# MorphIQ-Labs/VectorWave

Hardware: AMD Instinct MI355X
Metric: Msamples/sec MODWT fwd+inv db4 L=6, batch 4096×4096 fp64 @ 1/2/4/8 GPU (higher is better)
Workload: dtype f64

## Files before the change

include/vectorwave_amd.h:

```cpp
#ifndef VECTORWAVE_AMD_H
#define VECTORWAVE_AMD_H

#include <stdint.h>

#ifdef __cplusplus
extern "C" {
#endif

#define VW_API __attribute__((visibility("default")))

typedef struct vw_ctx vw_ctx;
typedef struct vw_stream vw_stream;
typedef int vw_status;

enum {
    VW_OK = 0,
    VW_ERR_NULL = 1,
    VW_ERR_EMPTY = 2,
    VW_ERR_NONFINITE = 3,
    VW_ERR_LEVEL = 4,
    VW_ERR_TOO_LARGE = 5,
    VW_ERR_BOUNDARY = 6,
    VW_ERR_ARG = 7,
    VW_ERR_DEVICE = 8,
// ... 27 lines not shown
VW_API vw_status vw_ctx_set_stream(vw_ctx *ctx, void *hip_stream);
VW_API vw_status vw_ctx_use_null_stream(vw_ctx *ctx);
VW_API void *vw_ctx_get_stream(vw_ctx *ctx);
VW_API vw_status vw_ctx_set_option(vw_ctx *ctx, const char *key, int value);
VW_API vw_status vw_ctx_synchronize(vw_ctx *ctx);
VW_API int vw_ctx_device(vw_ctx *ctx);

VW_API const char *vw_last_error(void);
VW_API int64_t vw_last_error_index(void);
VW_API const char *vw_version(void);
VW_API void vw_set_signal_base(int64_t base);

VW_API int vw_max_levels(int64_t N, int L);
VW_API int64_t vw_upsampled_length(int L, int level);

VW_API vw_status vw_modwt_forward_f64(vw_ctx *ctx, const double *x, int64_t B, int64_t N, int64_t ldx,
                                      const double *lo, const double *hi, int L, int wavelet_id,
                                      int boundary, int J, unsigned flags,
                                      double *details, double *approx);
VW_API vw_status vw_modwt_forward_f32(vw_ctx *ctx, const float *x, int64_t B, int64_t N, int64_t ldx,
                                      const double *lo, const double *hi, int L, int wavelet_id,
                                      int boundary, int J, unsigned flags,
                                      float *details, float *approx);

VW_API vw_status vw_modwt_inverse_f64(vw_ctx *ctx, const double *details, const double *approx,
                                      int64_t B, int64_t N, const double *lo, const double *hi, int L,
                                      int wavelet_id, int boundary, int J, unsigned detail_mask,
                                      int approx_zero, unsigned flags, double *y);
VW_API vw_status vw_modwt_inverse_f32(vw_ctx *ctx, const float *details, const float *approx,
                                      int64_t B, int64_t N, const double *lo, const double *hi, int L,
                                      int wavelet_id, int boundary, int J, unsigned detail_mask,
                                      int approx_zero, unsigned flags, float *y);

VW_API vw_status vw_modwt_forward_bi_f64(vw_ctx *ctx, const double *x, int64_t B, int64_t N, int64_t ldx,
                                         const double *lo, int Llo, const double *hi, int Lhi, int wavelet_id,
                                         int boundary, int J, unsigned flags, double *details, double *approx);
VW_API vw_status vw_modwt_forward_bi_f32(vw_ctx *ctx, const float *x, int64_t B, int64_t N, int64_t ldx,
                                         const double *lo, int Llo, const double *hi, int Lhi, int wavelet_id,
                                         int boundary, int J, unsigned flags, float *details, float *approx);
VW_API vw_status vw_modwt_inverse_bi_f64(vw_ctx *ctx, const double *details, const double *approx, int64_t B,
                                         int64_t N, const double *lo, int Llo, const double *hi, int Lhi,
                                         int wavelet_id, int boundary, int J, unsigned detail_mask,
                                         int approx_zero, unsigned flags, double *y);
VW_API vw_status vw_modwt_inverse_bi_f32(vw_ctx *ctx, const float *details, const float *approx, int64_t B,
                                         int64_t N, const double *lo, int Llo, const double *hi, int Lhi,
                                         int wavelet_id, int boundary, int J, unsigned detail_mask,
                                         int approx_zero, unsigned flags, float *y);
VW_API vw_status vw_modwt1_forward_bi_f64(vw_ctx *ctx, const double *x, int64_t B, int64_t N, int64_t ldx,
                                          const double *lo, int Llo, const double *hi, int Lhi, int boundary,
                                          unsigned flags, double *approx, double *detail);
VW_API vw_status vw_modwt1_inverse_bi_f64(vw_ctx *ctx, const double *approx, const double *detail, int64_t B,
                                          int64_t N, const double *lo, int Llo, const double *hi, int Lhi,
                                          int boundary, unsigned flags, double *y);

VW_API vw_status vw_modwt_energy_f64(vw_ctx *ctx, const double *x, int64_t B, int64_t N, int64_t ldx,
                                     const double *lo, const double *hi, int L, int wavelet_id,
                                     int boundary, int J, unsigned flags, double *out);
VW_API vw_status vw_energy_planes_f64(vw_ctx *ctx, const double *details, const double *approx, int64_t B,
                                      int64_t N, int J, unsigned flags, double *out);

VW_API vw_status vw_mra_planes_f64(vw_ctx *ctx, const double *details, const double *approx, int64_t B, int64_t N,
                                   const double *lo, const double *hi, int L, int wavelet_id, int boundary, int J,
                                   unsigned flags, double *out);
VW_API vw_status vw_mra_planes_f32(vw_ctx *ctx, const float *details, const float *approx, int64_t B, int64_t N,
                                   const double *lo, const double *hi, int L, int wavelet_id, int boundary, int J,
                                   unsigned flags, float *out);
VW_API vw_status vw_modwt_mra_f64(vw_ctx *ctx, const double *x, int64_t B, int64_t N, int64_t ldx,
                                  const double *lo, const double *hi, int L, int wavelet_id, int boundary, int J,
                                  unsigned flags, double *out);
VW_API vw_status vw_modwt_mra_f32(vw_ctx *ctx, const float *x, int64_t B, int64_t N, int64_t ldx,
                                  const double *lo, const double *hi, int L, int wavelet_id, int boundary, int J,
                                  unsigned flags, float *out);

VW_API vw_status vw_modwt_forward_multi_f64(vw_ctx *const *ctxs, int nctx, const double *x, int64_t B, int64_t N,
                                            int64_t ldx, const double *lo, const double *hi, int L, int wavelet_id,
                                            int boundary, int J, unsigned flags, double *details, double *approx);
VW_API vw_status vw_modwt_inverse_multi_f64(vw_ctx *const *ctxs, int nctx, const double *details,
                                            const double *approx, int64_t B, int64_t N, const double *lo,
                                            const double *hi, int L, int wavelet_id, int boundary, int J,
                                            unsigned detail_mask, int approx_zero, unsigned flags, double *y);

VW_API vw_status vw_modwt_forward_multi_dev_f64(vw_ctx *const *ctxs, int nctx, const double *const *x,
                                                const int64_t *rows, int64_t N, int64_t ldx, const double *lo,
                                                const double *hi, int L, int wavelet_id, int boundary, int J,
                                                unsigned flags, double *const *details, double *const *approx);
VW_API vw_status vw_modwt_inverse_multi_dev_f64(vw_ctx *const *ctxs, int nctx, const double *const *details,
                                                const double *const *approx, const int64_t *rows, int64_t N,
                                                const double *lo, const double *hi, int L, int wavelet_id,
                                                int boundary, int J, unsigned detail_mask, int approx_zero,
                                                unsigned flags, double *const *y);

VW_API vw_status vw_modwt1_forward_f64(vw_ctx *ctx, const double *x, int64_t B, int64_t N, int64_t ldx,
                                       const double *lo, const double *hi, int L, int boundary,
                                       unsigned flags, double *approx, double *detail);
VW_API vw_status vw_modwt1_inverse_f64(vw_ctx *ctx, const double *approx, const double *detail,
                                       int64_t B, int64_t N, const double *lo, const double *hi, int L,
                                       int boundary, unsigned flags, double *y);


VW_API vw_status vw_fin_analyze_f64(vw_ctx *ctx, const double *prices, int64_t B, int64_t N, int64_t ld,
                                    const double *lo, const double *hi, int L, double anomaly_k,
                                    unsigned flags, double *out);
VW_API vw_status vw_fin_sharpe_f64(vw_ctx *ctx, const double *returns, int64_t B, int64_t N, int64_t ld,
                                   double risk_free, unsigned flags, double *out);
VW_API vw_status vw_fin_wavelet_sharpe_f64(vw_ctx *ctx, const double *returns, int64_t B, int64_t N, int64_t ld,
                                           const double *lo, const double *hi, int L, int boundary,
                                           double risk_free, unsigned flags, double *out);

VW_API vw_status vw_swt_denoise_f64(vw_ctx *ctx, const double *x, int64_t B, int64_t N, int64_t ldx,
                                    const double *lo, const double *hi, int L, int wavelet_id,
                                    int boundary, int J, double threshold, int soft, unsigned flags,
                                    double *y, double *thresholds_out);
VW_API vw_status vw_transpose_f64(vw_ctx *ctx, const double *in, int64_t rows, int64_t cols, unsigned flags,
                                  double *out);
VW_API vw_status vw_transpose_f32(vw_ctx *ctx, const float *in, int64_t rows, int64_t cols, unsigned flags,
                                  float *out);

#define VW_THR_UNIVERSAL 0
#define VW_THR_SURE 1
#define VW_THR_MINIMAX 2
#define VW_THR_BAYES 3
#define VW_THR_FIXED 4
VW_API vw_status vw_wavelet_denoise_f64(vw_ctx *ctx, const double *x, int64_t B, int64_t N, int64_t ldx,
                                        const double *lo, const double *hi, int L, int wavelet_id,
                                        int boundary, int levels, int method, double fixed_threshold, int soft,
                                        unsigned flags, double *y, double *thresholds_out);

VW_API vw_status vw_noise_sigma_f64(vw_ctx *ctx, const double *coeffs, int64_t B, int64_t N,
                                    unsigned flags, double *sigma);
VW_API vw_status vw_threshold_f64(vw_ctx *ctx, double *c, int64_t B, int64_t N, const double *thr,
                                  int soft, unsigned flags);

VW_API vw_status vw_median_f64(vw_ctx *ctx, const double *x, int64_t B, int64_t N, const double *center,
                               unsigned flags, double *median_out);
VW_API vw_status vw_stddev_f64(vw_ctx *ctx, const double *x, int64_t N, unsigned flags, double *out);
VW_API vw_status vw_window_gather_abs_f64(vw_ctx *ctx, const double *src, const int32_t *idx, int64_t count,
                                          double *window, int64_t wsize, int64_t start);

VW_API vw_status vw_stream_create(vw_ctx *ctx, const double *lo, const double *hi, int L,
                                  int boundary, int levels, vw_stream **out);
VW_API vw_status vw_stream_destroy(vw_stream *s);
VW_API vw_status vw_stream_process_f64(vw_stream *s, const double *block, int64_t B, int64_t n,
                                       unsigned flags, double *details, double *approx);
VW_API vw_status vw_stream_flush_f64(vw_stream *s, int64_t tail_len, unsigned flags,
                                     double *details, double *approx);
VW_API int64_t vw_stream_history_length(vw_stream *s, int level);
VW_API int64_t vw_stream_batch(vw_stream *s);

typedef struct vw_graph vw_graph;
VW_API vw_status vw_capture_begin(vw_ctx *ctx);
VW_API vw_status vw_capture_end(vw_ctx *ctx, vw_graph **out);
VW_API vw_status vw_graph_launch(vw_graph *graph, int64_t count);
VW_API vw_status vw_graph_destroy(vw_graph *graph);

typedef struct vw_pipeline vw_pipeline;
VW_API vw_status vw_pipeline_create(vw_ctx *fwd_ctx, vw_ctx *inv_ctx, int elem_bytes, int sets, void *const *x,
                                    void *const *details, void *const *approx, void *const *y, int64_t B,
                                    int64_t N, const double *lo, const double *hi, int L, int wavelet_id,
                                    int boundary, int J, unsigned flags, vw_pipeline **out);
VW_API vw_status vw_pipeline_run(vw_pipeline *p, int64_t steps);
VW_API vw_status vw_pipeline_join(vw_pipeline *p);
VW_API int64_t vw_pipeline_last_set(vw_pipeline *p);
VW_API vw_status vw_pipeline_destroy(vw_pipeline *p);

VW_API vw_status vw_fill_uniform_f64(vw_ctx *ctx, double *x, int64_t count, uint64_t seed, int64_t offset);
VW_API vw_status vw_fill_uniform_f32(vw_ctx *ctx, float *x, int64_t count, uint64_t seed, int64_t offset);
VW_API vw_status vw_device_alloc(vw_ctx *ctx, int64_t bytes, void **out);
VW_API vw_status vw_device_free(vw_ctx *ctx, void *p);
VW_API vw_status vw_memcpy(vw_ctx *ctx, void *dst, const void *src, int64_t bytes, int kind );

VW_API vw_status vw_ctx_enable_timing(vw_ctx *ctx, int enable);
VW_API vw_status vw_ctx_kernel_time(vw_ctx *ctx, const char *family, double *total_ms, int64_t *launches);
VW_API vw_status vw_ctx_reset_timing(vw_ctx *ctx);
VW_API vw_status vw_ctx_kernel_spans(vw_ctx *ctx, const char *family, void *ref_event, int64_t max,
                                     double *start_ms, double *end_ms, int64_t *count);

#ifdef __cplusplus
}
#endif
#endif
```

vectorwave_amd/_native.py:

```python
from __future__ import annotations

import ctypes
import os
from ctypes import POINTER, c_char_p, c_double, c_float, c_int, c_int64, c_uint, c_uint64, c_void_p

_HERE = os.path.dirname(os.path.abspath(__file__))
LIB_PATH = os.environ.get("VW_LIB_PATH", os.path.join(_HERE, "libvectorwave_amd.so"))

FLAG_CORE_LEVELS = 1 << 0
FLAG_VALIDATE = 1 << 1
FLAG_FFT_SWITCH = 1 << 2
FLAG_FMA = 1 << 3
FLAG_HOST_MEMORY = 1 << 4
FLAG_SYNC = 1 << 5
FLAG_BATCH_SYM_INVERSE = 1 << 6
FLAG_BATCH_HAAR = 1 << 7
FLAG_REF_NONFINITE = 1 << 8
FLAG_TREE_SUMS = 1 << 9

PERIODIC, SYMMETRIC, ZERO_PADDING = 0, 1, 2

_dp = POINTER(c_double)
_fp = POINTER(c_float)
SIGNATURES = {
    "vw_ctx_create": (c_int, [c_int, POINTER(c_void_p)]),
    "vw_ctx_destroy": (c_int, [c_void_p]),
    "vw_ctx_use_null_stream": (c_int, [c_void_p]),
    "vw_ctx_set_stream": (c_int, [c_void_p, c_void_p]),
    "vw_ctx_get_stream": (c_void_p, [c_void_p]),
    "vw_ctx_set_option": (c_int, [c_void_p, c_char_p, c_int]),
    "vw_ctx_synchronize": (c_int, [c_void_p]),
    "vw_ctx_device": (c_int, [c_void_p]),
    "vw_last_error": (c_char_p, []),
    "vw_last_error_index": (c_int64, []),
    "vw_version": (c_char_p, []),
    "vw_set_signal_base": (None, [c_int64]),
    "vw_max_levels": (c_int, [c_int64, c_int]),
    "vw_upsampled_length": (c_int64, [c_int, c_int]),
    "vw_modwt_forward_f64": (c_int, [c_void_p, c_void_p, c_int64, c_int64, c_int64, _dp, _dp, c_int, c_int, c_int,
                                     c_int, c_uint, c_void_p, c_void_p]),
    "vw_modwt_forward_f32": (c_int, [c_void_p, c_void_p, c_int64, c_int64, c_int64, _dp, _dp, c_int, c_int, c_int,
                                     c_int, c_uint, c_void_p, c_void_p]),
    "vw_modwt_inverse_f64": (c_int, [c_void_p, c_void_p, c_void_p, c_int64, c_int64, _dp, _dp, c_int, c_int, c_int,
                                     c_int, c_uint, c_int, c_uint, c_void_p]),
    "vw_modwt_inverse_f32": (c_int, [c_void_p, c_void_p, c_void_p, c_int64, c_int64, _dp, _dp, c_int, c_int, c_int,
                                     c_int, c_uint, c_int, c_uint, c_void_p]),
    "vw_modwt_forward_multi_f64": (c_int, [c_void_p, c_int, c_void_p, c_int64, c_int64, c_int64, _dp, _dp, c_int,
                                           c_int, c_int, c_int, c_uint, c_void_p, c_void_p]),
    "vw_modwt_inverse_multi_f64": (c_int, [c_void_p, c_int, c_void_p, c_void_p, c_int64, c_int64, _dp, _dp, c_int,
                                           c_int, c_int, c_int, c_uint, c_int, c_uint, c_void_p]),
    "vw_modwt_forward_multi_dev_f64": (c_int, [c_void_p, c_int, c_void_p, c_void_p, c_int64, c_int64, _dp, _dp,
                                               c_int, c_int, c_int, c_int, c_uint, c_void_p, c_void_p]),
    "vw_modwt_inverse_multi_dev_f64": (c_int, [c_void_p, c_int, c_void_p, c_void_p, c_void_p, c_int64, _dp, _dp,
                                               c_int, c_int, c_int, c_int, c_uint, c_int, c_uint, c_void_p]),
    "vw_modwt1_forward_f64": (c_int, [c_void_p, c_void_p, c_int64, c_int64, c_int64, _dp, _dp, c_int, c_int, c_uint,
                                      c_void_p, c_void_p]),
    "vw_modwt1_inverse_f64": (c_int, [c_void_p, c_void_p, c_void_p, c_int64, c_int64, _dp, _dp, c_int, c_int, c_uint,
                                      c_void_p]),
    "vw_modwt_forward_bi_f64": (c_int, [c_void_p, c_void_p, c_int64, c_int64, c_int64, _dp, c_int, _dp, c_int, c_int,
                                        c_int, c_int, c_uint, c_void_p, c_void_p]),
    "vw_modwt_forward_bi_f32": (c_int, [c_void_p, c_void_p, c_int64, c_int64, c_int64, _dp, c_int, _dp, c_int, c_int,
                                        c_int, c_int, c_uint, c_void_p, c_void_p]),
    "vw_modwt_inverse_bi_f64": (c_int, [c_void_p, c_void_p, c_void_p, c_int64, c_int64, _dp, c_int, _dp, c_int, c_int,
                                        c_int, c_int, c_uint, c_int, c_uint, c_void_p]),
    "vw_modwt_inverse_bi_f32": (c_int, [c_void_p, c_void_p, c_void_p, c_int64, c_int64, _dp, c_int, _dp, c_int, c_int,
                                        c_int, c_int, c_uint, c_int, c_uint, c_void_p]),
    "vw_modwt1_forward_bi_f64": (c_int, [c_void_p, c_void_p, c_int64, c_int64, c_int64, _dp, c_int, _dp, c_int, c_int,
                                         c_uint, c_void_p, c_void_p]),
    "vw_modwt1_inverse_bi_f64": (c_int, [c_void_p, c_void_p, c_void_p, c_int64, c_int64, _dp, c_int, _dp, c_int, c_int,
                                         c_uint, c_void_p]),
    "vw_modwt_energy_f64": (c_int, [c_void_p, c_void_p, c_int64, c_int64, c_int64, _dp, _dp, c_int, c_int, c_int,
                                    c_int, c_uint, c_void_p]),
    "vw_energy_planes_f64": (c_int, [c_void_p, c_void_p, c_void_p, c_int64, c_int64, c_int, c_uint, c_void_p]),
    "vw_mra_planes_f64": (c_int, [c_void_p, c_void_p, c_void_p, c_int64, c_int64, _dp, _dp, c_int, c_int, c_int,
                                  c_int, c_uint, c_void_p]),
    "vw_mra_planes_f32": (c_int, [c_void_p, c_void_p, c_void_p, c_int64, c_int64, _dp, _dp, c_int, c_int, c_int,
                                  c_int, c_uint, c_void_p]),
    "vw_modwt_mra_f64": (c_int, [c_void_p, c_void_p, c_int64, c_int64, c_int64, _dp, _dp, c_int, c_int, c_int,
                                 c_int, c_uint, c_void_p]),
    "vw_modwt_mra_f32": (c_int, [c_void_p, c_void_p, c_int64, c_int64, c_int64, _dp, _dp, c_int, c_int, c_int,
                                 c_int, c_uint, c_void_p]),
    "vw_fin_analyze_f64": (c_int, [c_void_p, c_void_p, c_int64, c_int64, c_int64, _dp, _dp, c_int, c_double, c_uint,
                                   c_void_p]),
    "vw_fin_sharpe_f64": (c_int, [c_void_p, c_void_p, c_int64, c_int64, c_int64, c_double, c_uint, c_void_p]),
    "vw_fin_wavelet_sharpe_f64": (c_int, [c_void_p, c_void_p, c_int64, c_int64, c_int64, _dp, _dp, c_int, c_int,
                                          c_double, c_uint, c_void_p]),
    "vw_swt_denoise_f64": (c_int, [c_void_p, c_void_p, c_int64, c_int64, c_int64, _dp, _dp, c_int, c_int, c_int,
                                   c_int, c_double, c_int, c_uint, c_void_p, c_void_p]),
    "vw_wavelet_denoise_f64": (c_int, [c_void_p, c_void_p, c_int64, c_int64, c_int64, _dp, _dp, c_int, c_int, c_int,
                                       c_int, c_int, c_double, c_int, c_uint, c_void_p, c_void_p]),
    "vw_transpose_f64": (c_int, [c_void_p, c_void_p, c_int64, c_int64, c_uint, c_void_p]),
    "vw_transpose_f32": (c_int, [c_void_p, c_void_p, c_int64, c_int64, c_uint, c_void_p]),
    "vw_noise_sigma_f64": (c_int, [c_void_p, c_void_p, c_int64, c_int64, c_uint, c_void_p]),
    "vw_threshold_f64": (c_int, [c_void_p, c_void_p, c_int64, c_int64, c_void_p, c_int, c_uint]),
    "vw_stream_create": (c_int, [c_void_p, _dp, _dp, c_int, c_int, c_int, POINTER(c_void_p)]),
    "vw_stream_destroy": (c_int, [c_void_p]),
    "vw_stream_process_f64": (c_int, [c_void_p, c_void_p, c_int64, c_int64, c_uint, c_void_p, c_void_p]),
    "vw_stream_flush_f64": (c_int, [c_void_p, c_int64, c_uint, c_void_p, c_void_p]),
    "vw_stream_history_length": (c_int64, [c_void_p, c_int]),
    "vw_stream_batch": (c_int64, [c_void_p]),
    "vw_fill_uniform_f64": (c_int, [c_void_p, c_void_p, c_int64, c_uint64, c_int64]),
    "vw_fill_uniform_f32": (c_int, [c_void_p, c_void_p, c_int64, c_uint64, c_int64]),
    "vw_device_alloc": (c_int, [c_void_p, c_int64, POINTER(c_void_p)]),
    "vw_device_free": (c_int, [c_void_p, c_void_p]),
    "vw_memcpy": (c_int, [c_void_p, c_void_p, c_void_p, c_int64, c_int]),
    "vw_ctx_enable_timing": (c_int, [c_void_p, c_int]),
    "vw_ctx_kernel_time": (c_int, [c_void_p, c_char_p, POINTER(c_double), POINTER(c_int64)]),
    "vw_ctx_reset_timing": (c_int, [c_void_p]),
    "vw_ctx_kernel_spans": (c_int, [c_void_p, c_char_p, c_void_p, c_int64, POINTER(c_double), POINTER(c_double),
                                    POINTER(c_int64)]),
    "vw_median_f64": (c_int, [c_void_p, c_void_p, c_int64, c_int64, c_void_p, c_uint, c_void_p]),
    "vw_stddev_f64": (c_int, [c_void_p, c_void_p, c_int64, c_uint, c_void_p]),
    "vw_window_gather_abs_f64": (c_int, [c_void_p, c_void_p, c_void_p, c_int64, c_void_p, c_int64, c_int64]),
    "vw_capture_begin": (c_int, [c_void_p]),
    "vw_capture_end": (c_int, [c_void_p, POINTER(c_void_p)]),
    "vw_graph_launch": (c_int, [c_void_p, c_int64]),
    "vw_graph_destroy": (c_int, [c_void_p]),
    "vw_pipeline_create": (c_int, [c_void_p, c_void_p, c_int, c_int, c_void_p, c_void_p, c_void_p, c_void_p, c_int64,
                                   c_int64, _dp, _dp, c_int, c_int, c_int, c_int, c_uint, POINTER(c_void_p)]),
    "vw_pipeline_run": (c_int, [c_void_p, c_int64]),
    "vw_pipeline_join": (c_int, [c_void_p]),
    "vw_pipeline_last_set": (c_int64, [c_void_p]),
    "vw_pipeline_destroy": (c_int, [c_void_p]),
}

_lib = None


def load() -> ctypes.CDLL:
    global _lib
    if _lib is not None:
        return _lib
    if not os.path.exists(LIB_PATH):
        raise ImportError(
            f"vectorwave_amd native library not found at {LIB_PATH}; build it with "
            f"`python -c 'import __graft_entry__ as g; g.build()'` (make -C vectorwave_amd/csrc)")
    lib = ctypes.CDLL(LIB_PATH)
    for name, (res, args) in SIGNATURES.items():
        fn = getattr(lib, name)
        fn.restype = res
        fn.argtypes = args
    _lib = lib
    return lib


def last_error() -> str:
    msg = load().vw_last_error()
    return msg.decode() if msg else ""


def last_error_index() -> int:
    return int(load().vw_last_error_index())


def taps_array(values) -> ctypes.Array:
    arr = (c_double * len(values))(*[float(v) for v in values])
    return arr
```

vectorwave_amd/csrc/vw_capi.cpp:

```cpp
#include "../../include/vectorwave_amd.h"
#include "vw_internal.h"
#include "vw_deep.h"
#include "vw_plan.h"

#include <algorithm>
#include <cmath>
#include <cstdarg>
#include <cstdio>
#include <cstring>
#include <map>
#include <mutex>
#include <set>
#include <string>
#include <thread>
#include <vector>

using namespace vw;

static thread_local std::string t_err;
static thread_local int64_t t_err_index = -1;
static thread_local int64_t t_signal_base = 0;

static vw_status fail(vw_status code, const char* fmt, ...) {
  char buf[512];
  va_list ap;
  va_start(ap, fmt);
  vsnprintf(buf, sizeof(buf), fmt, ap);
  va_end(ap);
  t_err = buf;
  if (code != VW_ERR_NONFINITE) t_err_index = -1;
  return code;
}

static vw_status ok() {
  t_err.clear();
  t_err_index = -1;
  return VW_OK;
}

#define VW_HIP(call)                                                                         \
  do {                                                                                       \
    hipError_t e_ = (call);                                                                  \
    if (e_ != hipSuccess) return fail(VW_ERR_DEVICE, "%s: %s", #call, hipGetErrorString(e_)); \
  } while (0)

#define VW_TRY(expr)                      \
  do {                                    \
    vw_status s_ = (expr);                \
    if (s_ != VW_OK) return s_;           \
  } while (0)

struct TimedLaunch {
  std::string family;
  hipEvent_t start, stop;
  bool graph_owned = false;
};

struct vw_graph;
struct vw_ctx;
static void kill_pipelines_of(vw_ctx* c);

struct vw_ctx {
  int device = 0;
  hipStream_t stream = nullptr;
  bool own_stream = false;
  bool capturing = false;
  unsigned ws_gen = 0;
  Tuning tune;
  int cus = 256;
  std::recursive_mutex mu;
  void* ws = nullptr;
  size_t ws_bytes = 0;
  void* ws2 = nullptr;
  size_t ws2_bytes = 0;
  unsigned long long* bad = nullptr;
  bool timing = false;
  std::vector<TimedLaunch> pending;
  std::vector<TimedLaunch> captured;
  std::vector<hipEvent_t> event_pool;
  std::map<std::string, std::pair<double, int64_t>> totals;
  std::set<vw_graph*> graphs;
  std::vector<std::pair<void*, size_t>> stage;
  void* med = nullptr;
  size_t med_bytes = 0;
  int* nf = nullptr;
  int64_t nf_rows = 0;
};

struct vw_graph {
  vw_ctx* ctx = nullptr;
  int device = 0;
  unsigned ws_gen = 0;
  std::vector<TimedLaunch> timed;
  hipGraph_t graph = nullptr;
  hipGraphExec_t exec = nullptr;
};

static void release_graph(vw_graph* gr) {
  for (auto& t : gr->timed) { hipEventDestroy(t.start); hipEventDestroy(t.stop); }
  gr->timed.clear();
  if (gr->exec) hipGraphExecDestroy(gr->exec);
  if (gr->graph) hipGraphDestroy(gr->graph);
  gr->exec = nullptr;
  gr->graph = nullptr;
}

struct vw_stream {
  vw_ctx* ctx = nullptr;
  std::vector<double> lo, hi;
  int L = 0;
  int boundary = 0;
  int levels = 0;
  int64_t last_batch = -1;
  bool hist_init = false;
  std::vector<double*> hist;
  std::vector<double*> snap;
  std::vector<int> hist_len;
};

static hipEvent_t pool_event(vw_ctx* c) {
  if (!c->event_pool.empty()) {
    hipEvent_t e = c->event_pool.back();
    c->event_pool.pop_back();
    return e;
  }
  hipEvent_t e = nullptr;
  if (hipEventCreate(&e) != hipSuccess) return nullptr;
  return e;
}

static bool capture_event(hipStream_t st, hipEvent_t ev) {
  hipStreamCaptureStatus status;
  unsigned long long id = 0;
  hipGraph_t g = nullptr;
  const hipGraphNode_t* deps = nullptr;
  size_t ndeps = 0;
  if (hipStreamGetCaptureInfo_v2(st, &status, &id, &g, &deps, &ndeps) == hipSuccess &&
      status == hipStreamCaptureStatusActive && g) {
    hipGraphNode_t node = nullptr;
    if (hipGraphAddEventRecordNode(&node, g, deps, ndeps, ev) == hipSuccess &&
        hipStreamUpdateCaptureDependencies(st, &node, 1, hipStreamSetCaptureDependencies) == hipSuccess)
      return true;
  }
  (void)hipGetLastError();
  if (hipEventRecordWithFlags(ev, st, hipEventRecordExternal) == hipSuccess) return true;
  (void)hipGetLastError();
  return false;
}

struct LaunchTimer {
  vw_ctx* c;
  TimedLaunch tl;
  bool on;
  LaunchTimer(vw_ctx* ctx, const char* family) : c(ctx), on(ctx->timing) {
    if (!on) return;
    tl.family = family;
    if (c->capturing) {
      tl.graph_owned = true;
      tl.start = tl.stop = nullptr;
      if (hipEventCreate(&tl.start) != hipSuccess || hipEventCreate(&tl.stop) != hipSuccess ||
          !capture_event(c->stream, tl.start)) {
        if (tl.start) hipEventDestroy(tl.start);
        if (tl.stop) hipEventDestroy(tl.stop);
        on = false;
      }
      return;
    }
    tl.start = pool_event(c);
    tl.stop = pool_event(c);
    if (!tl.start || !tl.stop) { on = false; return; }
    hipEventRecord(tl.start, c->stream);
  }
  ~LaunchTimer() {
    if (!on) return;
    if (tl.graph_owned) {
      if (capture_event(c->stream, tl.stop)) {
        c->captured.push_back(tl);
      } else {
        hipEventDestroy(tl.start);
        hipEventDestroy(tl.stop);
      }
      return;
    }
    hipEventRecord(tl.stop, c->stream);
    c->pending.push_back(tl);
  }
};

static void collect_timing(vw_ctx* c) {
  for (auto& tl : c->pending) {
    float ms = 0.f;
    if (hipEventSynchronize(tl.stop) == hipSuccess && hipEventElapsedTime(&ms, tl.start, tl.stop) == hipSuccess) {
      auto& t = c->totals[tl.family];
      t.first += ms;
      t.second += 1;
    }
    if (!tl.graph_owned) {
      c->event_pool.push_back(tl.start);
      c->event_pool.push_back(tl.stop);
    }
  }
  c->pending.clear();
}

static vw_status ensure_ws(vw_ctx* c, size_t bytes) {
  if (bytes <= c->ws_bytes) return VW_OK;
  if (c->capturing) return fail(VW_ERR_STATE, "workspace growth during capture: run the call once before capturing it");
  if (c->ws) {
    hipDeviceSynchronize();
    ++c->ws_gen;
    hipFree(c->ws);
    c->ws = nullptr;
    c->ws_bytes = 0;
  }
  size_t want = std::max(bytes, (size_t)1 << 20);
  VW_HIP(hipMalloc(&c->ws, want));
  c->ws_bytes = want;
  return VW_OK;
}

static vw_status ensure_nf(vw_ctx* c, int64_t B) {
  if (B <= c->nf_rows) return VW_OK;
  if (c->capturing) return fail(VW_ERR_STATE, "row-flag growth during capture: run the call once before capturing it");
  if (c->nf) {
    hipDeviceSynchronize();
    ++c->ws_gen;
    hipFree(c->nf);
    c->nf = nullptr;
    c->nf_rows = 0;
  }
  const int64_t rows = std::max<int64_t>(B, 4096);
  VW_HIP(hipMalloc(&c->nf, (size_t)rows * sizeof(int)));
  VW_HIP(hipMemset(c->nf, 0, (size_t)rows * sizeof(int)));
  VW_HIP(hipDeviceSynchronize());
  c->nf_rows = rows;
  return VW_OK;
}

static inline size_t align_up(size_t v, size_t a) { return (v + a - 1) / a * a; }

extern "C" int vw_max_levels(int64_t N, int L) { return max_levels(N, L); }
extern "C" int64_t vw_upsampled_length(int L, int level) { return upsampled_length(L, level); }

extern "C" vw_status vw_ctx_create(int device, vw_ctx** out) {
  if (!out) return fail(VW_ERR_NULL, "out is null");
  int n = 0;
  VW_HIP(hipGetDeviceCount(&n));
  if (device < 0 || device >= n) return fail(VW_ERR_ARG, "device %d out of range (%d devices)", device, n);
  VW_HIP(hipSetDevice(device));
  vw_ctx* c = new vw_ctx();
  c->device = device;
  c->tune = read_tuning();
  { int n = 0; if (hipDeviceGetAttribute(&n, hipDeviceAttributeMultiprocessorCount, device) == hipSuccess && n > 0) c->cus = n; }
  if (hipStreamCreateWithFlags(&c->stream, hipStreamNonBlocking) != hipSuccess) {
    delete c;
    return fail(VW_ERR_DEVICE, "hipStreamCreate failed");
  }
  c->own_stream = true;
  if (hipMalloc(&c->bad, sizeof(unsigned long long)) != hipSuccess) {
    hipStreamDestroy(c->stream);
    delete c;
    return fail(VW_ERR_DEVICE, "hipMalloc failed");
  }
  *out = c;
  return ok();
}

extern "C" vw_status vw_ctx_destroy(vw_ctx* c) {
  if (!c) return fail(VW_ERR_NULL, "ctx is null");
  hipSetDevice(c->device);
  if (c->capturing) {
    hipGraph_t gph = nullptr;
    if (hipStreamEndCapture(c->stream, &gph) == hipSuccess && gph) hipGraphDestroy(gph);
    (void)hipGetLastError();
    for (auto& t : c->captured) { hipEventDestroy(t.start); hipEventDestroy(t.stop); }
    c->captured.clear();
    c->capturing = false;
  }
  hipStreamSynchronize(c->stream);
  kill_pipelines_of(c);
  hipSetDevice(c->device);
  collect_timing(c);
  for (vw_graph* gr : c->graphs) {
    release_graph(gr);
    gr->ctx = nullptr;
  }
  c->graphs.clear();
  for (auto e : c->event_pool) hipEventDestroy(e);
  if (c->ws) hipFree(c->ws);
  if (c->ws2) hipFree(c->ws2);
  if (c->med) hipFree(c->med);
  if (c->nf) hipFree(c->nf);
  for (auto& b : c->stage) hipFree(b.first);
  if (c->bad) hipFree(c->bad);
  if (c->own_stream) hipStreamDestroy(c->stream);
  delete c;
  return ok();
}

static vw_status rebind_stream(vw_ctx* c, hipStream_t next, bool own_next) {
  if (c->capturing) return fail(VW_ERR_STATE, "stream change during capture");
  hipStream_t prev = c->stream;
  if (c->own_stream) {
    VW_HIP(hipStreamSynchronize(prev));
    VW_HIP(hipStreamDestroy(prev));
    c->own_stream = false;
  } else if (prev != next) {
    hipEvent_t ev = nullptr;
    VW_HIP(hipEventCreateWithFlags(&ev, hipEventDisableTiming));
    hipError_t e = hipEventRecord(ev, prev);
    if (e == hipSuccess && next) e = hipStreamWaitEvent(next, ev, 0);
    if (e == hipSuccess && !next) e = hipEventSynchronize(ev);
    hipEventDestroy(ev);
    if (e != hipSuccess) return fail(VW_ERR_DEVICE, "stream ordering failed: %s", hipGetErrorString(e));
  }
  c->stream = next;
  c->own_stream = own_next;
  return VW_OK;
}

extern "C" vw_status vw_ctx_use_null_stream(vw_ctx* c) {
  if (!c) return fail(VW_ERR_NULL, "ctx is null");
  std::lock_guard<std::recursive_mutex> g(c->mu);
  hipSetDevice(c->device);
  VW_TRY(rebind_stream(c, nullptr, false));
  return ok();
}

extern "C" vw_status vw_ctx_set_stream(vw_ctx* c, void* s) {
  if (!c) return fail(VW_ERR_NULL, "ctx is null");
  std::lock_guard<std::recursive_mutex> g(c->mu);
  hipSetDevice(c->device);
  if (s) {
    VW_TRY(rebind_stream(c, (hipStream_t)s, false));
  } else {
    hipStream_t ns = nullptr;
    VW_HIP(hipStreamCreateWithFlags(&ns, hipStreamNonBlocking));
    VW_TRY(rebind_stream(c, ns, true));
  }
  return ok();
}


extern "C" vw_status vw_capture_begin(vw_ctx* c) {
  if (!c) return fail(VW_ERR_NULL, "ctx is null");
  std::lock_guard<std::recursive_mutex> g(c->mu);
  if (c->capturing) return fail(VW_ERR_STATE, "already capturing");
  if (!c->stream) return fail(VW_ERR_STATE, "the null stream cannot be captured; bind a stream first");
  hipSetDevice(c->device);
  VW_HIP(hipStreamBeginCapture(c->stream, hipStreamCaptureModeThreadLocal));
  c->capturing = true;
  c->captured.clear();
  return ok();
}

extern "C" vw_status vw_capture_end(vw_ctx* c, vw_graph** out) {
  if (!c || !out) return fail(VW_ERR_NULL, "null argument");
  std::lock_guard<std::recursive_mutex> g(c->mu);
  if (!c->capturing) return fail(VW_ERR_STATE, "not capturing");
  hipSetDevice(c->device);
  c->capturing = false;
  std::vector<TimedLaunch> timed;
  timed.swap(c->captured);
  auto drop = [&] { for (auto& t : timed) { hipEventDestroy(t.start); hipEventDestroy(t.stop); } };
  hipGraph_t graph = nullptr;
  hipError_t ec = hipStreamEndCapture(c->stream, &graph);
  if (ec != hipSuccess) {
    drop();
    return fail(VW_ERR_DEVICE, "hipStreamEndCapture: %s", hipGetErrorString(ec));
  }
  hipGraphExec_t exec = nullptr;
  hipError_t e = hipGraphInstantiate(&exec, graph, nullptr, nullptr, 0);
  if (e != hipSuccess) {
    hipGraphDestroy(graph);
    drop();
    return fail(VW_ERR_DEVICE, "graph instantiate failed: %s", hipGetErrorString(e));
  }
  vw_graph* gr = new vw_graph();
  gr->timed.swap(timed);
  gr->ctx = c;
  gr->device = c->device;
  gr->ws_gen = c->ws_gen;
  gr->graph = graph;
  gr->exec = exec;
  c->graphs.insert(gr);
  *out = gr;
  return ok();
}


extern "C" vw_status vw_graph_launch(vw_graph* gr, int64_t count) {
  if (!gr) return fail(VW_ERR_NULL, "graph is null");
  vw_ctx* c = gr->ctx;
  if (!c) return fail(VW_ERR_STATE, "the context of this graph was destroyed");
  std::lock_guard<std::recursive_mutex> g(c->mu);
  if (gr->ws_gen != c->ws_gen)
    return fail(VW_ERR_STATE, "the context workspace moved since this graph was recorded; record it again");
  hipSetDevice(c->device);
  for (int64_t i = 0; i < count; ++i) VW_HIP(hipGraphLaunch(gr->exec, c->stream));
  if (c->timing && count > 0 && !gr->timed.empty()) {
    std::set<hipEvent_t> mine;
    for (const auto& t : gr->timed) mine.insert(t.start);
    c->pending.erase(std::remove_if(c->pending.begin(), c->pending.end(),
                                    [&](const TimedLaunch& t) { return t.graph_owned && mine.count(t.start); }),
                     c->pending.end());
    for (const auto& t : gr->timed) c->pending.push_back(t);
  }
  return ok();
}

extern "C" vw_status vw_graph_destroy(vw_graph* gr) {
  if (!gr) return fail(VW_ERR_NULL, "graph is null");
  vw_ctx* c = gr->ctx;
  if (!c) {
    delete gr;
    return ok();
  }
  std::lock_guard<std::recursive_mutex> g(c->mu);
  hipSetDevice(c->device);
  hipStreamSynchronize(c->stream);
  collect_timing(c);
  release_graph(gr);
  c->graphs.erase(gr);
  delete gr;
  return ok();
}

struct vw_pipeline {
  vw_ctx* cf = nullptr;
  vw_ctx* ci = nullptr;
  int device = 0;
  int esz = 8;
  int R = 0;
  std::vector<void*> x, det, app, y;
  int64_t B = 0, N = 0;
  std::vector<double> lo, hi;
  int L = 0, wavelet_id = 0, boundary = 0, J = 0;
  unsigned flags = 0;
  std::vector<hipEvent_t> ev_f, ev_i;
  std::vector<char> live;
  hipEvent_t join_ev = nullptr;
  int64_t next = 0;
  bool dead = false;
  std::mutex mu;
};

static std::mutex g_pipe_mu;
static std::set<vw_pipeline*> g_pipes;

static void release_pipeline(vw_pipeline* p) {
  for (auto e : p->ev_f) if (e) hipEventDestroy(e);
  for (auto e : p->ev_i) if (e) hipEventDestroy(e);
  if (p->join_ev) hipEventDestroy(p->join_ev);
  p->ev_f.clear();
  p->ev_i.clear();
  p->join_ev = nullptr;
}

static void kill_pipelines_of(vw_ctx* c) {
  std::lock_guard<std::mutex> g(g_pipe_mu);
  for (vw_pipeline* p : g_pipes)
    if (!p->dead && (p->cf == c || p->ci == c)) {
      std::lock_guard<std::mutex> pg(p->mu);
      hipSetDevice(p->device);
      hipStreamSynchronize(p->cf->stream);
      hipStreamSynchronize(p->ci->stream);
      release_pipeline(p);
      p->dead = true;
    }
}

extern "C" vw_status vw_pipeline_create(vw_ctx* cf, vw_ctx* ci, int elem_bytes, int sets, void* const* x,
                                        void* const* details, void* const* approx, void* const* y, int64_t B,
                                        int64_t N, const double* lo, const double* hi, int L, int wavelet_id,
                                        int boundary, int J, unsigned flags, vw_pipeline** out) {
  if (!cf || !ci || !x || !details || !approx || !y || !lo || !hi || !out) return fail(VW_ERR_NULL, "null argument");
  if (elem_bytes != 8 && elem_bytes != 4) return fail(VW_ERR_ARG, "elem_bytes must be 8 (f64) or 4 (f32)");
  if (sets < 1 || sets > 1024) return fail(VW_ERR_ARG, "sets must be in [1, 1024]");
  if (B <= 0 || N <= 0) return fail(VW_ERR_EMPTY, "Signals cannot be null or empty");
  if (L <= 0 || L > kMaxTaps) return fail(VW_ERR_ARG, "filter length %d out of range", L);
  if (J < 1) return fail(VW_ERR_ARG, "levels must be >= 1");
  if (cf->device != ci->device) return fail(VW_ERR_ARG, "both contexts must be on one device");
  if (flags & (VW_FLAG_HOST_MEMORY | VW_FLAG_SYNC | VW_FLAG_VALIDATE))
    return fail(VW_ERR_ARG, "pipeline steps take device buffers, no SYNC / VALIDATE / HOST_MEMORY");
  for (int r = 0; r < sets; ++r)
    if (!x[r] || !details[r] || !approx[r] || !y[r]) return fail(VW_ERR_NULL, "buffer set %d has a null pointer", r);
  if (cf->capturing || ci->capturing) return fail(VW_ERR_STATE, "a context is capturing");
  vw_pipeline* p = new vw_pipeline();
  p->cf = cf;
  p->ci = ci;
  p->device = cf->device;
  p->esz = elem_bytes;
  p->R = sets;
  p->x.assign(x, x + sets);
  p->det.assign(details, details + sets);
  p->app.assign(approx, approx + sets);
  p->y.assign(y, y + sets);
  p->B = B;
  p->N = N;
  p->lo.assign(lo, lo + L);
  p->hi.assign(hi, hi + L);
  p->L = L;
  p->wavelet_id = wavelet_id;
  p->boundary = boundary;
  p->J = J;
  p->flags = flags;
  hipSetDevice(p->device);
  p->ev_f.assign(sets, nullptr);
  p->ev_i.assign(sets, nullptr);
  p->live.assign(sets, 0);
  hipError_t e = hipEventCreateWithFlags(&p->join_ev, hipEventDisableTiming);
  for (int r = 0; r < sets && e == hipSuccess; ++r) {
    e = hipEventCreateWithFlags(&p->ev_f[r], hipEventDisableTiming);
    if (e == hipSuccess) e = hipEventCreateWithFlags(&p->ev_i[r], hipEventDisableTiming);
  }
  if (e != hipSuccess) {
    release_pipeline(p);
    delete p;
    return fail(VW_ERR_DEVICE, "event creation failed: %s", hipGetErrorString(e));
  }
  {
    std::lock_guard<std::mutex> g(g_pipe_mu);
    g_pipes.insert(p);
  }
  *out = p;
  return ok();
}

extern "C" vw_status vw_pipeline_run(vw_pipeline* p, int64_t steps) {
  if (!p) return fail(VW_ERR_NULL, "pipeline is null");
  std::lock_guard<std::mutex> pg(p->mu);
  if (p->dead) return fail(VW_ERR_STATE, "a context of this pipeline was destroyed");
  if (steps < 0) return fail(VW_ERR_ARG, "steps must be >= 0");
  if (p->cf->capturing || p->ci->capturing) return fail(VW_ERR_STATE, "a context of this pipeline is capturing");
  hipSetDevice(p->device);
  const bool f32 = p->esz == 4;
  for (int64_t k = 0; k < steps; ++k) {
    const int r = (int)(p->next % p->R);
    hipStream_t sf = p->cf->stream, si = p->ci->stream;
    if (p->live[r]) VW_HIP(hipStreamWaitEvent(sf, p->ev_i[r], 0));
    vw_status st = f32 ? vw_modwt_forward_f32(p->cf, (const float*)p->x[r], p->B, p->N, p->N, p->lo.data(),
                                              p->hi.data(), p->L, p->wavelet_id, p->boundary, p->J, p->flags,
                                              (float*)p->det[r], (float*)p->app[r])
                       : vw_modwt_forward_f64(p->cf, (const double*)p->x[r], p->B, p->N, p->N, p->lo.data(),
                                              p->hi.data(), p->L, p->wavelet_id, p->boundary, p->J, p->flags,
                                              (double*)p->det[r], (double*)p->app[r]);
    if (st != VW_OK) return st;
    VW_HIP(hipEventRecord(p->ev_f[r], sf));
    VW_HIP(hipStreamWaitEvent(si, p->ev_f[r], 0));
    st = f32 ? vw_modwt_inverse_f32(p->ci, (const float*)p->det[r], (const float*)p->app[r], p->B, p->N,
                                    p->lo.data(), p->hi.data(), p->L, p->wavelet_id, p->boundary, p->J, 0xFFFFFFFFu,
                                    0, p->flags, (float*)p->y[r])
             : vw_modwt_inverse_f64(p->ci, (const double*)p->det[r], (const double*)p->app[r], p->B, p->N,
                                    p->lo.data(), p->hi.data(), p->L, p->wavelet_id, p->boundary, p->J, 0xFFFFFFFFu,
                                    0, p->flags, (double*)p->y[r]);
    if (st != VW_OK) return st;
    VW_HIP(hipEventRecord(p->ev_i[r], si));
    p->live[r] = 1;
    ++p->next;
  }
// ... 123 lines not shown
    if (J < 1 || J > maxl)
      return fail(VW_ERR_LEVEL, "Invalid number of decomposition levels: %d (valid 1..%d for N=%lld, L=%d)", J, maxl,
                  (long long)N, L);
  } else {
    if (J < 1) return fail(VW_ERR_LEVEL, "levels must be >= 1");
    if (J > kMaxLevels) return fail(VW_ERR_LEVEL, "levels %d exceeds engine limit %d", J, kMaxLevels);
    if (vw_upsampled_length(L, J) > (int64_t)1 << 30) return fail(VW_ERR_TOO_LARGE, "upsampled filter too long");
  }
  return VW_OK;
}

static vw_status check_bank(int64_t N, int L, int Lhi, int J, unsigned flags, bool forward) {
  if (Lhi == 0) return VW_OK;
  if (Lhi < 1 || Lhi > kMaxTaps) return fail(VW_ERR_ARG, "filter length %d unsupported (1..%d)", Lhi, kMaxTaps);
  if (flags & VW_FLAG_CORE_LEVELS) {
    if (vw_upsampled_length(std::max(L, Lhi), J) > N)
      return fail(VW_ERR_TOO_LARGE, "Upsampled %s filter length exceeds signal length", forward ? "analysis" : "reconstruction");
  } else if (forward && Lhi > L) {
    if (vw_upsampled_length(Lhi, J) > (int64_t)1 << 30) return fail(VW_ERR_TOO_LARGE, "upsampled filter too long");
  }
  return VW_OK;
}

template <typename T>
static void copy_taps(T* dst, const double* src, int L) {
  const double s = 1.0 / std::sqrt(2.0);
  for (int i = 0; i < L; ++i) dst[i] = (T)(src[i] * s);
  for (int i = L; i < kMaxTaps; ++i) dst[i] = T(0);
}

template <typename T, typename Call>
static void copy_bank(T* lo, T* hi, const Call& k, int taps, int taps_hi = 0) {
  copy_taps(lo, k.lo, std::min(k.L, taps));
  copy_taps(hi, k.hi, std::min(k.Lhi > 0 ? k.Lhi : k.L, taps_hi > 0 ? taps_hi : taps));
}

static vw_status capture_guard(vw_ctx* c, unsigned flags) {
  if (c->capturing && (flags & (VW_FLAG_VALIDATE | VW_FLAG_HOST_MEMORY | VW_FLAG_SYNC)))
    return fail(VW_ERR_STATE, "validation, host memory and SYNC cannot be captured");
  return VW_OK;
}

static vw_status read_bad(vw_ctx* c, unsigned long long* out) {
  VW_HIP(hipMemcpyAsync(out, c->bad, sizeof(unsigned long long), hipMemcpyDeviceToHost, c->stream));
  VW_HIP(hipStreamSynchronize(c->stream));
  return VW_OK;
}

static vw_status report_bad(unsigned long long bad, int64_t N) {
  if (bad == ~0ull) return VW_OK;
  const bool out = (bad >> 62) & 1ull;
  const unsigned long long flat = bad & ((1ull << 62) - 1);
  t_err_index = (int64_t)(flat % (unsigned long long)N);
  return fail(VW_ERR_NONFINITE, "%s contains non-finite value at index %lld (signal %lld)",
              out ? "coefficients" : "signal", (long long)(flat % (unsigned long long)N),
              (long long)(flat / (unsigned long long)N) + (long long)t_signal_base);
}

template <typename T>
struct ScanPlane {
  const T* p;
  int64_t ld;
  int len;
};

template <typename T>
static vw_status ref_nonfinite(vw_ctx* c, const std::vector<ScanPlane<T>>& planes, RefArgs<T>& r,
                               bool inverse, bool flagged, int grid) {
  const int64_t B = r.B, N = r.N;
  if ((int)planes.size() > kRefPlanes) return fail(VW_ERR_ARG, "too many planes for the non-finite scan");
  LaunchTimer lt(c, flagged ? "ref_nonfinite" : "ref_nonfinite_scan");
  hipError_t e;
  if (!flagged) {
    RefScan<T> s;
    memset(&s, 0, sizeof(s));
    for (const auto& p : planes) {
      s.p[s.np] = p.p;
      s.ld[s.np] = p.ld;
      s.len[s.np] = p.len;
      ++s.np;
    }
    s.B = B; s.N = (int)N; s.chunks = ref_scan_chunks((int)N); s.flag = c->nf;
    e = launch_flag_nonfinite<T>(s, c->stream);
    if (e != hipSuccess) return fail(VW_ERR_DEVICE, "non-finite scan launch failed: %s", hipGetErrorString(e));
  }
  r.flag = c->nf;
  r.scratch = reinterpret_cast<T*>(c->ws);
  e = launch_ref_cascade<T>(r, (int)grid, inverse, c->stream);
  if (e != hipSuccess) return fail(VW_ERR_DEVICE, "reference-arithmetic launch failed: %s", hipGetErrorString(e));
  return VW_OK;
}

static hipError_t mfma_forward(const FwdArgs<float>& a, int lds, hipStream_t st) { return launch_forward_mfma(a, lds, st); }
static hipError_t mfma_forward(const FwdArgs<double>&, int, hipStream_t) { return hipErrorNotSupported; }
static hipError_t mfma_inverse(const InvArgs<float>& a, int lds, hipStream_t st) { return launch_inverse_mfma(a, lds, st); }
static hipError_t mfma_inverse(const InvArgs<double>&, int, hipStream_t) { return hipErrorNotSupported; }


static vw_status reserve(vw_ctx* c, const PlanReserve& r) {
  if (r.ws_bytes) VW_TRY(ensure_ws(c, r.ws_bytes));
  if (r.nf_rows) VW_TRY(ensure_nf(c, r.nf_rows));
  return VW_OK;
}

static const char* const kStepNames[] = {"deep", "multi-level", "level-group", "level", "level"};
static vw_status step_failed(const char* dir, int kind, hipError_t e) {
  return fail(VW_ERR_DEVICE, "%s %s launch failed: %s", dir, kStepNames[kind - kStepDeep], hipGetErrorString(e));
}

template <typename T>
static vw_status forward_steps(vw_ctx* c, const FwdCall<T>& k, const FwdPlan<T>& p) {
  const size_t plane = (size_t)k.B * (size_t)k.N;
  T* const ws[2] = {reinterpret_cast<T*>(c->ws), reinterpret_cast<T*>(c->ws) + plane};
  for (const PlanStep<T>& s : p.steps) {
    const T* const src = s.src == kBufIn ? k.x : ws[s.src - kBufWs0];
    T* const dst = s.dst == kBufOut ? k.approx : ws[s.dst - kBufWs0];
    T* const det = k.details + (size_t)(s.jlo - 1) * plane;
    hipError_t e;
    if (s.kind == kStepDeep) {
      DeepArgs<T> d = s.deep;
      d.src = src; d.out = dst;
      d.nf_flag = s.probe ? c->nf : nullptr;
      for (int g = 0; g < d.g; ++g) d.out_d[g] = det + (size_t)g * plane;
      copy_bank(d.lo, d.hi, k, d.taps);
      LaunchTimer lt(c, "forward_level");
      e = launch_deep<T>(d, s.lds, p.fma, false, c->stream);
    } else if (s.kind == kStepMulti) {
      MultiArgs<T> m = s.multi;
      m.src_a = src; m.out_a = dst;
      for (int g = 0; g < m.nlev; ++g) m.out_d[g] = det + (size_t)g * plane;
      copy_bank(m.lo, m.hi, k, m.taps);
      LaunchTimer lt(c, "forward_level");
      e = launch_forward_multi<T>(m, s.lds, p.fma, c->stream);
    } else {
      LevelArgs<T> a = s.lvl;
      a.src_a = src; a.out_a = dst; a.out_d = det;
      a.hist = k.hist ? k.hist[s.jlo - 1] : nullptr;
      a.bad = c->bad;
      copy_bank(a.lo, a.hi, k, a.taps);
      LaunchTimer lt(c, "forward_level");
      e = s.kind == kStepSweep ? launch_forward_sweep<T>(a, p.fma, c->stream)
                               : launch_forward_level<T>(a, s.lds, p.fma, c->stream);
    }
    if (e != hipSuccess) return step_failed("forward", s.kind, e);
    if (s.hist_update) {
      e = launch_history_update<T>(src, s.lvl.lda, k.hist[s.jlo - 1], k.hist[s.jlo - 1], k.B, (int)k.N,
                                   s.lvl.lv.hist_len, c->stream);
      if (e != hipSuccess) return fail(VW_ERR_DEVICE, "history update failed: %s", hipGetErrorString(e));
    }
  }
  return VW_OK;
}

template <typename T>
static vw_status forward_impl(vw_ctx* c, FwdCall<T> k) {
  VW_TRY(capture_guard(c, k.flags));
  k.cus = c->cus;
  FwdPlan<T> p;
  plan_forward(c->tune, k, &p);
  if (p.error != VW_OK) return fail((vw_status)p.error, "%s", p.msg);
  VW_TRY(reserve(c, p.res));
  const LevelDesc* const lv = p.args.lv;
  if (p.snapshot)
    for (int j = 0; j < k.J; ++j)
      if (lv[j].hist_len > 0)
        VW_HIP(hipMemcpyAsync(k.hist_snap[j], k.hist[j], (size_t)k.B * lv[j].hist_len * sizeof(T),
                              hipMemcpyDeviceToDevice, c->stream));
  if (p.validate) VW_HIP(hipMemsetAsync(c->bad, 0xFF, sizeof(unsigned long long), c->stream));
  if (p.fused) {
    FwdArgs<T> a = p.args;
    a.x = k.x; a.details = k.details; a.approx = k.approx;
    a.bad = c->bad;
    a.nf_flag = p.nf_probed ? c->nf : nullptr;
    for (int j = 0; j < k.J; ++j) a.hist[j] = k.hist ? k.hist[j] : nullptr;
    copy_bank(a.lo, a.hi, k, a.taps, a.taps_hi);
    LaunchTimer lt(c, "forward");
    hipError_t e = p.kernel == kFwdMfma    ? mfma_forward(a, p.lds, c->stream)
                 : p.kernel == kFwdBlk     ? launch_forward_blk<T>(a, p.threads, p.lds, p.fma, p.nv, c->stream)
                 : p.kernel == kFwdPersist ? launch_forward_persist<T>(a, p.threads, p.lds, p.fma, p.nv, c->stream)
                                           : launch_forward_fused<T>(a, p.threads, p.lds, p.fma, p.nv, c->stream);
    if (e != hipSuccess) return fail(VW_ERR_DEVICE, "forward launch failed: %s", hipGetErrorString(e));
  } else {
    VW_TRY(forward_steps(c, k, p));
  }
  if (p.ref_nf) {
    std::vector<ScanPlane<T>> planes{{k.approx, k.N, 0}};
    RefArgs<T> r;
    memset(&r, 0, sizeof(r));
    r.x = k.x; r.ldx = k.ldx; r.details = k.details; r.approx = k.approx;
    r.B = k.B; r.N = (int)k.N; r.J = k.J; r.L = k.L; r.mode = ref_mode(k.boundary);
    if (k.hist) {
      r.hist_mode = 1;
      r.hist_first = k.hist_first ? 1 : 0;
      for (int j = 0; j < k.J; ++j) {
        r.hist_len[j] = lv[j].hist_len;
        r.hist_old[j] = k.hist_first ? nullptr : (k.hist_update ? k.hist_snap[j] : k.hist[j]);
        r.hist_new[j] = k.hist_update ? k.hist[j] : nullptr;
      }
    }
    r.Lhi = k.Lhi;
    copy_bank(r.lo, r.hi, k, p.args.taps, p.args.taps_hi);
    VW_TRY(ref_nonfinite<T>(c, planes, r, false, p.nf_probed, p.res.ref_grid));
  }
  if (p.validate) {
    unsigned long long bad = 0;
    VW_TRY(read_bad(c, &bad));
    VW_TRY(report_bad(bad, k.N));
  }
  if (k.flags & VW_FLAG_SYNC) VW_HIP(hipStreamSynchronize(c->stream));
  return VW_OK;
}

template <typename T>
static vw_status inverse_steps(vw_ctx* c, const InvCall<T>& k, const InvPlan<T>& p) {
  const size_t plane = (size_t)k.B * (size_t)k.N;
  T* const ws[2] = {reinterpret_cast<T*>(c->ws), reinterpret_cast<T*>(c->ws) + plane};
  auto det = [&](int j, int use_d) { return use_d ? k.details + (size_t)(j - 1) * plane : nullptr; };
  auto thr = [&](int j) { return k.thr ? k.thr + (size_t)(j - 1) * (size_t)k.thr_ld : nullptr; };
  for (const PlanStep<T>& s : p.steps) {
    const T* const src = s.src == kBufNone ? nullptr : s.src == kBufIn ? k.approx : ws[s.src - kBufWs0];
    T* const dst = s.dst == kBufOut ? k.y : ws[s.dst - kBufWs0];
    hipError_t e;
    if (s.kind == kStepDeep) {
      DeepArgs<T> d = s.deep;
      d.src = src; d.out = dst;
      for (int g = 0; g < d.g; ++g) {
        d.src_d[g] = det(s.jlo + g, p.args.lv[s.jlo - 1 + g].use_d);
        d.thr[g] = thr(s.jlo + g);
      }
      copy_bank(d.lo, d.hi, k, d.taps);
      LaunchTimer lt(c, "inverse_level");
      e = launch_deep<T>(d, s.lds, p.fma, true, c->stream);
    } else if (s.kind == kStepMulti) {
      MultiArgs<T> m = s.multi;
      m.src_a = src; m.out_a = dst;
      m.nf_flag = s.probe ? c->nf : nullptr;
      for (int g = 0; g < m.nlev; ++g) {
        m.src_d[g] = det(s.jlo + g, p.args.lv[s.jlo - 1 + g].use_d);
        m.thr[g] = thr(s.jlo + g);
      }
      copy_bank(m.lo, m.hi, k, m.taps);
      LaunchTimer lt(c, "inverse_level");
      e = launch_inverse_multi<T>(m, s.lds, p.fma, c->stream);
    } else {
      LevelArgs<T> a = s.lvl;
      a.src_a = src; a.out_a = dst;
      a.src_d = det(s.jhi, a.use_d);
      a.thr = thr(s.jhi);
      if (s.kind == kStepSweepG) {
        a.src_d2 = det(s.jhi - 1, a.use_d2);
        a.thr2 = thr(s.jhi - 1);
        if (s.jhi - s.jlo == 2) {
          a.src_d3 = det(s.jhi - 2, a.use_d3);
          a.thr3 = thr(s.jhi - 2);
        }
      }
      copy_bank(a.lo, a.hi, k, a.taps);
      LaunchTimer lt(c, "inverse_level");
      e = s.kind == kStepSweepG ? launch_inverse_sweepg<T>(a, s.G, s.ka, s.R, p.fma, c->stream)
        : s.kind == kStepSweep  ? launch_inverse_sweep<T>(a, p.fma, c->stream)
                                : launch_inverse_level<T>(a, s.lds, p.fma, c->stream);
    }
    if (e != hipSuccess) return step_failed("inverse", s.kind, e);
  }
  return VW_OK;
}

template <typename T>
static vw_status inverse_impl(vw_ctx* c, InvCall<T> k) {
  VW_TRY(capture_guard(c, k.flags));
  k.cus = c->cus;
  InvPlan<T> p;
  plan_inverse(c->tune, k, &p);
  if (p.error != VW_OK) return fail((vw_status)p.error, "%s", p.msg);
  VW_TRY(reserve(c, p.res));
  if (p.fused) {
    InvArgs<T> a = p.args;
    a.details = k.details; a.approx = k.approx; a.y = k.y; a.thr = k.thr;
    a.nf_flag = p.nf_probed ? c->nf : nullptr;
    copy_bank(a.lo, a.hi, k, a.taps, a.taps_hi);
    LaunchTimer lt(c, "inverse");
    hipError_t e = p.kernel == kInvMfma ? mfma_inverse(a, p.lds, c->stream)
                                        : launch_inverse_fused<T>(a, p.threads, p.lds, p.fma, p.nv, c->stream);
    if (e != hipSuccess) return fail(VW_ERR_DEVICE, "inverse launch failed: %s", hipGetErrorString(e));
  } else {
    VW_TRY(inverse_steps(c, k, p));
  }
  if (p.ref_nf) {
    std::vector<ScanPlane<T>> planes{{k.y, k.N, 0}};
    RefArgs<T> r;
    memset(&r, 0, sizeof(r));
    r.x = k.approx_zero ? nullptr : k.approx; r.det_in = k.details; r.y = k.y;
    r.thr = k.thr; r.thr_ld = k.thr_ld; r.soft = k.soft;
    r.B = k.B; r.N = (int)k.N; r.J = k.J; r.L = k.L; r.mode = ref_mode(k.boundary);
    r.Lhi = k.Lhi;
    copy_bank(r.lo, r.hi, k, p.args.taps, p.args.taps_hi);
    for (int j = 0; j < k.J; ++j) r.lv[j] = p.args.lv[j];
    VW_TRY(ref_nonfinite<T>(c, planes, r, true, p.nf_probed, p.res.ref_grid));
  }
  if (k.flags & VW_FLAG_SYNC) VW_HIP(hipStreamSynchronize(c->stream));
  return VW_OK;
}

struct Staging {
  vw_ctx* c;
  size_t used_block = 0, used_off = 0;
  explicit Staging(vw_ctx* ctx) : c(ctx) {}
  ~Staging() {
    hipStreamSynchronize(c->stream);
    if (c->stage.size() > 1) {
      auto big = std::max_element(c->stage.begin(), c->stage.end(),
                                  [](const std::pair<void*, size_t>& a, const std::pair<void*, size_t>& b) {
                                    return a.second < b.second;
                                  });
      const auto keep = *big;
      for (auto& blk : c->stage)
        if (blk.first != keep.first) hipFree(blk.first);
      c->stage.assign(1, keep);
    }
  }
  vw_status carve(size_t bytes, void** out) {
    bytes = align_up(std::max<size_t>(bytes, 16), 256);
    for (; used_block < c->stage.size(); ++used_block, used_off = 0) {
      auto& blk = c->stage[used_block];
      if (used_off + bytes <= blk.second) {
        *out = static_cast<char*>(blk.first) + used_off;
        used_off += bytes;
        return VW_OK;
      }
    }
    size_t carved = bytes;
    for (size_t k = 0; k < used_block && k < c->stage.size(); ++k) carved += c->stage[k].second;
    if (used_block < c->stage.size()) carved += used_off;
    const size_t want = std::max({carved, (size_t)4 << 20});
    void* p = nullptr;
    VW_HIP(hipMalloc(&p, want));
    c->stage.push_back({p, want});
    used_block = c->stage.size() - 1;
    used_off = bytes;
    *out = p;
    return VW_OK;
  }
  template <typename T>
  vw_status in(const T* host, size_t count, T** dev) {
    void* p = nullptr;
    VW_TRY(carve(count * sizeof(T), &p));
    if (host && count) VW_HIP(hipMemcpyAsync(p, host, count * sizeof(T), hipMemcpyHostToDevice, c->stream));
    *dev = reinterpret_cast<T*>(p);
    return VW_OK;
  }
  template <typename T>
  vw_status in_planes(const T* host, size_t planes, size_t count, size_t host_stride, T** dev) {
    void* p = nullptr;
    VW_TRY(carve(planes * count * sizeof(T), &p));
    if (host && count && planes)
      VW_HIP(hipMemcpy2DAsync(p, count * sizeof(T), host, host_stride * sizeof(T), count * sizeof(T), planes,
                              hipMemcpyHostToDevice, c->stream));
    *dev = reinterpret_cast<T*>(p);
    return VW_OK;
  }
  template <typename T>
  vw_status out(T* host, const T* dev, size_t count) {
    if (host && count) VW_HIP(hipMemcpyAsync(host, dev, count * sizeof(T), hipMemcpyDeviceToHost, c->stream));
    return VW_OK;
  }
  template <typename T>
  vw_status out_planes(T* host, const T* dev, size_t planes, size_t count, size_t host_stride) {
    if (host && count && planes)
      VW_HIP(hipMemcpy2DAsync(host, host_stride * sizeof(T), dev, count * sizeof(T), count * sizeof(T), planes,
                              hipMemcpyDeviceToHost, c->stream));
    return VW_OK;
  }
};


template <typename T>
static vw_status forward_host(vw_ctx* c, const T* x, int64_t B, int64_t N, int64_t ldx, const double* lo,
                              const double* hi, int L, int boundary, int J, unsigned flags, T* details,
                              int64_t det_stride, T* approx, int Lhi = 0) {
  if (c->capturing) return fail(VW_ERR_STATE, "host-memory calls cannot be captured (they synchronize)");
  Staging s(c);
  T *dx, *dd, *da;
  VW_TRY(s.in(x, (size_t)(B - 1) * ldx + N, &dx));
  VW_TRY(s.in<T>(nullptr, (size_t)J * B * N, &dd));
  VW_TRY(s.in<T>(nullptr, (size_t)B * N, &da));
  FwdCall<T> fk;
  fk.x = dx; fk.B = B; fk.N = N; fk.ldx = ldx; fk.lo = lo; fk.hi = hi; fk.L = L; fk.boundary = boundary; fk.J = J;
  fk.flags = flags & ~(VW_FLAG_SYNC | VW_FLAG_HOST_MEMORY); fk.details = dd; fk.approx = da; fk.Lhi = Lhi;
  VW_TRY(forward_impl<T>(c, fk));
  VW_TRY(s.out_planes(details, dd, (size_t)J, (size_t)(B * N), (size_t)det_stride));
  VW_TRY(s.out(approx, da, (size_t)B * N));
  VW_HIP(hipStreamSynchronize(c->stream));
  return VW_OK;
}

template <typename T>
static vw_status inverse_host(vw_ctx* c, const T* details, int64_t det_stride, const T* approx, int64_t B, int64_t N,
                              const double* lo, const double* hi, int L, int wid, int boundary, int J,
                              unsigned detail_mask, int approx_zero, unsigned flags, T* y, int Lhi = 0) {
  if (c->capturing) return fail(VW_ERR_STATE, "host-memory calls cannot be captured (they synchronize)");
  Staging s(c);
  T *dd = nullptr, *da = nullptr, *dy;
  if (detail_mask) VW_TRY(s.in_planes(details, (size_t)J, (size_t)(B * N), (size_t)det_stride, &dd));
  if (!approx_zero) VW_TRY(s.in(approx, (size_t)B * N, &da));
  VW_TRY(s.in<T>(nullptr, (size_t)B * N, &dy));
  InvCall<T> ik;
  ik.details = dd; ik.approx = da; ik.B = B; ik.N = N; ik.lo = lo; ik.hi = hi; ik.L = L; ik.wid = wid;
  ik.boundary = boundary; ik.J = J; ik.detail_mask = detail_mask; ik.approx_zero = approx_zero;
  ik.flags = flags & ~(VW_FLAG_SYNC | VW_FLAG_HOST_MEMORY); ik.y = dy; ik.Lhi = Lhi;
  VW_TRY(inverse_impl<T>(c, ik));
  VW_TRY(s.out(y, dy, (size_t)B * N));
  VW_HIP(hipStreamSynchronize(c->stream));
  return VW_OK;
}

template <typename T>
static vw_status modwt_forward(vw_ctx* c, const T* x, int64_t B, int64_t N, int64_t ldx, const double* lo,
                               const double* hi, int L, int wid, int boundary, int J, unsigned flags, T* details,
                               T* approx, int Lhi = 0) {
  (void)wid;
  VW_TRY(check_common(c, x, details, lo, hi, B, N, L, boundary));
  if (!approx) return fail(VW_ERR_NULL, "approx is null");
  if (ldx < N) return fail(VW_ERR_ARG, "ldx (%lld) < N (%lld)", (long long)ldx, (long long)N);
  VW_TRY(check_levels(N, L, J, flags));
  VW_TRY(check_bank(N, L, Lhi, J, flags, true));
  std::lock_guard<std::recursive_mutex> g(c->mu);
  hipSetDevice(c->device);
  if (flags & VW_FLAG_HOST_MEMORY) {
    VW_TRY(forward_host<T>(c, x, B, N, ldx, lo, hi, L, boundary, J, flags, details, B * N, approx, Lhi));
    return ok();
  }
  FwdCall<T> fk;
  fk.x = x; fk.B = B; fk.N = N; fk.ldx = ldx; fk.lo = lo; fk.hi = hi; fk.L = L; fk.boundary = boundary; fk.J = J;
  fk.flags = flags; fk.details = details; fk.approx = approx; fk.Lhi = Lhi;
  VW_TRY(forward_impl<T>(c, fk));
  return ok();
}

static vw_status check_inverse(vw_ctx* c, const void* details, const void* approx, const void* y, const double* lo,
                               const double* hi, int64_t B, int64_t N, int L, int boundary, int J, unsigned detail_mask,
                               int approx_zero, unsigned flags) {
  if (!c) return fail(VW_ERR_NULL, "ctx is null");
  if (!y || !lo || !hi) return fail(VW_ERR_NULL, "null argument");
  if (!details && detail_mask) return fail(VW_ERR_NULL, "details is null");
  if (!approx && !approx_zero) return fail(VW_ERR_NULL, "approx is null");
  VW_TRY(check_common(c, y, y, lo, hi, B, N, L, boundary));
  if (J < 1 || J > kMaxLevels) return fail(VW_ERR_LEVEL, "levels must be in 1..%d", kMaxLevels);
  if ((flags & VW_FLAG_CORE_LEVELS) && vw_upsampled_length(L, J) > N)
    return fail(VW_ERR_TOO_LARGE, "Upsampled reconstruction filter length exceeds signal length");
  return VW_OK;
}

template <typename T>
static vw_status modwt_inverse(vw_ctx* c, const T* details, const T* approx, int64_t B, int64_t N, const double* lo,
                               const double* hi, int L, int wid, int boundary, int J, unsigned detail_mask,
                               int approx_zero, unsigned flags, T* y, int Lhi = 0) {
  VW_TRY(check_inverse(c, details, approx, y, lo, hi, B, N, L, boundary, J, detail_mask, approx_zero, flags));
  VW_TRY(check_bank(N, L, Lhi, J, flags, false));
  std::lock_guard<std::recursive_mutex> g(c->mu);
  hipSetDevice(c->device);
  if (flags & VW_FLAG_HOST_MEMORY) {
    VW_TRY(inverse_host<T>(c, details, B * N, approx, B, N, lo, hi, L, wid, boundary, J, detail_mask, approx_zero,
                           flags, y, Lhi));
    return ok();
  }
  InvCall<T> ik;
  ik.details = details; ik.approx = approx; ik.B = B; ik.N = N; ik.lo = lo; ik.hi = hi; ik.L = L; ik.wid = wid;
  ik.boundary = boundary; ik.J = J; ik.detail_mask = detail_mask; ik.approx_zero = approx_zero; ik.flags = flags;
  ik.y = y; ik.Lhi = Lhi;
  VW_TRY(inverse_impl<T>(c, ik));
  return ok();
}

extern "C" vw_status vw_modwt_forward_f64(vw_ctx* c, const double* x, int64_t B, int64_t N, int64_t ldx,
                                          const double* lo, const double* hi, int L, int wid, int boundary, int J,
                                          unsigned flags, double* details, double* approx) {
  return modwt_forward<double>(c, x, B, N, ldx, lo, hi, L, wid, boundary, J, flags, details, approx);
}
extern "C" vw_status vw_modwt_forward_f32(vw_ctx* c, const float* x, int64_t B, int64_t N, int64_t ldx,
                                          const double* lo, const double* hi, int L, int wid, int boundary, int J,
                                          unsigned flags, float* details, float* approx) {
  return modwt_forward<float>(c, x, B, N, ldx, lo, hi, L, wid, boundary, J, flags, details, approx);
}
extern "C" vw_status vw_modwt_inverse_f64(vw_ctx* c, const double* details, const double* approx, int64_t B,
                                          int64_t N, const double* lo, const double* hi, int L, int wid, int boundary,
                                          int J, unsigned detail_mask, int approx_zero, unsigned flags, double* y) {
  return modwt_inverse<double>(c, details, approx, B, N, lo, hi, L, wid, boundary, J, detail_mask, approx_zero,
                               flags, y);
}
extern "C" vw_status vw_modwt_inverse_f32(vw_ctx* c, const float* details, const float* approx, int64_t B,
                                          int64_t N, const double* lo, const double* hi, int L, int wid, int boundary,
                                          int J, unsigned detail_mask, int approx_zero, unsigned flags, float* y) {
  return modwt_inverse<float>(c, details, approx, B, N, lo, hi, L, wid, boundary, J, detail_mask, approx_zero, flags,
                              y);
}

static int bank_hi(int Llo, int Lhi) { return Lhi == Llo ? 0 : Lhi; }
static vw_status bank_arg(int Lhi) {
  if (Lhi < 1 || Lhi > kMaxTaps) return fail(VW_ERR_ARG, "filter length %d unsupported (1..%d)", Lhi, kMaxTaps);
  return VW_OK;
}
extern "C" vw_status vw_modwt_forward_bi_f64(vw_ctx* c, const double* x, int64_t B, int64_t N, int64_t ldx,
                                             const double* lo, int Llo, const double* hi, int Lhi, int wid,
                                             int boundary, int J, unsigned flags, double* details, double* approx) {
  VW_TRY(bank_arg(Lhi));
  return modwt_forward<double>(c, x, B, N, ldx, lo, hi, Llo, wid, boundary, J, flags, details, approx, bank_hi(Llo, Lhi));
}
extern "C" vw_status vw_modwt_forward_bi_f32(vw_ctx* c, const float* x, int64_t B, int64_t N, int64_t ldx,
                                             const double* lo, int Llo, const double* hi, int Lhi, int wid,
                                             int boundary, int J, unsigned flags, float* details, float* approx) {
  VW_TRY(bank_arg(Lhi));
  return modwt_forward<float>(c, x, B, N, ldx, lo, hi, Llo, wid, boundary, J, flags, details, approx, bank_hi(Llo, Lhi));
}
extern "C" vw_status vw_modwt_inverse_bi_f64(vw_ctx* c, const double* details, const double* approx, int64_t B,
                                             int64_t N, const double* lo, int Llo, const double* hi, int Lhi, int wid,
                                             int boundary, int J, unsigned detail_mask, int approx_zero,
                                             unsigned flags, double* y) {
  VW_TRY(bank_arg(Lhi));
  return modwt_inverse<double>(c, details, approx, B, N, lo, hi, Llo, wid, boundary, J, detail_mask, approx_zero,
                               flags, y, bank_hi(Llo, Lhi));
}
extern "C" vw_status vw_modwt_inverse_bi_f32(vw_ctx* c, const float* details, const float* approx, int64_t B,
                                             int64_t N, const double* lo, int Llo, const double* hi, int Lhi, int wid,
                                             int boundary, int J, unsigned detail_mask, int approx_zero,
                                             unsigned flags, float* y) {
  VW_TRY(bank_arg(Lhi));
  return modwt_inverse<float>(c, details, approx, B, N, lo, hi, Llo, wid, boundary, J, detail_mask, approx_zero,
                              flags, y, bank_hi(Llo, Lhi));
}

static void shard_block(int64_t B, int n, int k, int64_t* start, int64_t* rows) {
  const int64_t base = B / n, extra = B % n;
  *start = k * base + std::min<int64_t>(k, extra);
  *rows = base + (k < extra ? 1 : 0);
}

template <typename F>
static vw_status run_per_ctx(vw_ctx* const* ctxs, int nctx, const char* what, F&& fn) {
  if (!ctxs) return fail(VW_ERR_NULL, "ctxs is null");
  if (nctx < 1) return fail(VW_ERR_ARG, "need at least one context (got %d)", nctx);
  for (int k = 0; k < nctx; ++k)
    if (!ctxs[k]) return fail(VW_ERR_NULL, "ctxs[%d] is null", k);
  struct Res { vw_status st = VW_OK; std::string msg; int64_t idx = -1; };
  std::vector<Res> res(nctx);
  auto work = [&](int k) {
    const vw_status st = fn(k);
    res[k].st = st;
    if (st != VW_OK) { res[k].msg = t_err; res[k].idx = t_err_index; }
  };
  std::vector<std::thread> th;
  th.reserve(nctx);
  for (int k = 1; k < nctx; ++k) th.emplace_back(work, k);
  work(0);
  for (auto& t : th) t.join();
  for (int k = 0; k < nctx; ++k)
    if (res[k].st != VW_OK) {
      t_err = std::string(what) + " " + std::to_string(k) + ": " + res[k].msg;
      t_err_index = res[k].idx;
      return res[k].st;
    }
  return ok();
}

template <typename F>
static vw_status run_sharded(vw_ctx* const* ctxs, int nctx, int64_t B, F&& fn) {
  if (!ctxs) return fail(VW_ERR_NULL, "ctxs is null");
  if (nctx < 1) return fail(VW_ERR_ARG, "need at least one context (got %d)", nctx);
  for (int k = 0; k < nctx; ++k)
    if (!ctxs[k]) return fail(VW_ERR_NULL, "ctxs[%d] is null", k);
  if (B <= 0) return fail(VW_ERR_EMPTY, "batch must be non-empty (B=%lld)", (long long)B);
  const int used = (int)std::min<int64_t>(nctx, B);
  struct Res { vw_status st = VW_OK; std::string msg; int64_t idx = -1; };
  std::vector<Res> res(used);
  auto work = [&](int k) {
    int64_t start, rows;
    shard_block(B, used, k, &start, &rows);
    t_signal_base = start;
    const vw_status st = fn(ctxs[k], start, rows);
    t_signal_base = 0;
    res[k].st = st;
    if (st != VW_OK) { res[k].msg = t_err; res[k].idx = t_err_index; }
  };
  std::vector<std::thread> th;
  th.reserve(used);
  for (int k = 1; k < used; ++k) th.emplace_back(work, k);
  work(0);
  for (auto& t : th) t.join();
  for (int k = 0; k < used; ++k)
    if (res[k].st != VW_OK) {
      int64_t start, rows;
      shard_block(B, used, k, &start, &rows);
      t_err = "block " + std::to_string(k) + " (rows " + std::to_string(start) + ".." +
              std::to_string(start + rows - 1) + "): " + res[k].msg;
      t_err_index = res[k].idx;
      return res[k].st;
    }
  return ok();
}

extern "C" vw_status vw_modwt_forward_multi_f64(vw_ctx* const* ctxs, int nctx, const double* x, int64_t B, int64_t N,
                                                int64_t ldx, const double* lo, const double* hi, int L, int wid,
                                                int boundary, int J, unsigned flags, double* details,
                                                double* approx) {
  if (!(flags & VW_FLAG_HOST_MEMORY)) return fail(VW_ERR_ARG, "multi-context calls take host memory (VW_FLAG_HOST_MEMORY)");
  if (!x || !details || !approx || !lo || !hi) return fail(VW_ERR_NULL, "null array argument");
  if (ldx < N) return fail(VW_ERR_ARG, "ldx (%lld) < N (%lld)", (long long)ldx, (long long)N);
  return run_sharded(ctxs, nctx, B, [&](vw_ctx* c, int64_t start, int64_t rows) -> vw_status {
    (void)wid;
    VW_TRY(check_common(c, x, details, lo, hi, rows, N, L, boundary));
    VW_TRY(check_levels(N, L, J, flags));
    std::lock_guard<std::recursive_mutex> g(c->mu);
    hipSetDevice(c->device);
    return forward_host<double>(c, x + start * ldx, rows, N, ldx, lo, hi, L, boundary, J, flags,
                                details + start * N, B * N, approx + start * N);
  });
}

extern "C" vw_status vw_modwt_inverse_multi_f64(vw_ctx* const* ctxs, int nctx, const double* details,
                                                const double* approx, int64_t B, int64_t N, const double* lo,
                                                const double* hi, int L, int wid, int boundary, int J,
                                                unsigned detail_mask, int approx_zero, unsigned flags, double* y) {
  if (!(flags & VW_FLAG_HOST_MEMORY)) return fail(VW_ERR_ARG, "multi-context calls take host memory (VW_FLAG_HOST_MEMORY)");
  if (!y || !lo || !hi) return fail(VW_ERR_NULL, "null argument");
  if (!details && detail_mask) return fail(VW_ERR_NULL, "details is null");
  if (!approx && !approx_zero) return fail(VW_ERR_NULL, "approx is null");
  if (J < 1 || J > kMaxLevels) return fail(VW_ERR_LEVEL, "levels must be in 1..%d", kMaxLevels);
  if ((flags & VW_FLAG_CORE_LEVELS) && vw_upsampled_length(L, J) > N)
    return fail(VW_ERR_TOO_LARGE, "Upsampled reconstruction filter length exceeds signal length");
  return run_sharded(ctxs, nctx, B, [&](vw_ctx* c, int64_t start, int64_t rows) -> vw_status {
    VW_TRY(check_common(c, y, y, lo, hi, rows, N, L, boundary));
    std::lock_guard<std::recursive_mutex> g(c->mu);
    hipSetDevice(c->device);
    return inverse_host<double>(c, details ? details + start * N : nullptr, B * N,
                                approx ? approx + start * N : nullptr, rows, N, lo, hi, L, wid, boundary, J,
                                detail_mask, approx_zero, flags, y + start * N);
  });
}

extern "C" vw_status vw_modwt_forward_multi_dev_f64(vw_ctx* const* ctxs, int nctx, const double* const* x,
                                                    const int64_t* rows, int64_t N, int64_t ldx, const double* lo,
                                                    const double* hi, int L, int wid, int boundary, int J,
                                                    unsigned flags, double* const* details,
                                                    double* const* approx) {
  if (flags & VW_FLAG_HOST_MEMORY)
    return fail(VW_ERR_ARG, "device-resident multi-context calls take device memory (no VW_FLAG_HOST_MEMORY)");
  if (!x || !rows || !details || !approx) return fail(VW_ERR_NULL, "null array argument");
  return run_per_ctx(ctxs, nctx, "context", [&](int k) -> vw_status {
// ... 1089 lines not shown
```

vectorwave_amd/csrc/vw_device.h:

```cpp
#pragma once
#include <hip/hip_runtime.h>
#include <cstdint>
#include <type_traits>
#include "vw_internal.h"

#pragma clang fp contract(off)

namespace vw {

template <typename T> struct VT;
template <> struct VT<double> { typedef double v __attribute__((ext_vector_type(2))); static constexpr int V = 2; };
template <> struct VT<float>  { typedef float  v __attribute__((ext_vector_type(4))); static constexpr int V = 4; };

__device__ __forceinline__ double fma_t(double a, double b, double c) { return __builtin_fma(a, b, c); }
__device__ __forceinline__ float fma_t(float a, float b, float c) { return __builtin_fmaf(a, b, c); }

template <bool FMA, typename T>
__device__ __forceinline__ T madd(T acc, T x, T f) {
  if constexpr (FMA) return fma_t(x, f, acc);
  else return acc + x * f;
}

#ifndef VW_PK_F32
#define VW_PK_F32 0
// ... 523 lines not shown
      const vec v = lds_vec_at<vec>(a0 + (unsigned)((LM - 1 - i) * S * (int)sizeof(T)));
      if (i < L) vmadd<FMA, kPkFwd>(al, v, lo[i]);
      if (i < LH) vmadd<FMA, kPkFwd>(ah, v, hi[i]);
      if ((i & 3) == 3) __builtin_amdgcn_sched_barrier(0);
    }
    emit(k, w, al, ah);
  });
}

template <typename T, int L, bool FMA, int NV, bool FULL = false, int LH = L, typename Emit>
__device__ __forceinline__ void fwd_row(const T* buf, int nvec, int s, const T* lo, const T* hi, int taps, int ct,
                                        Emit&& emit, int taps_hi = -1) {
  constexpr int V = VT<T>::V;
  if constexpr (L > 0) {
    if (s == 1) return fwd_row_t<T, L, FMA, NV, 1, FULL, LH>(buf, nvec, s, lo, hi, taps, emit);
    if constexpr (V == 4) {
      if (s == 2) return fwd_row_t<T, L, FMA, NV, 2, FULL, LH>(buf, nvec, s, lo, hi, taps, emit);
    }
  }
  if constexpr (L > 0 && L <= 8 && LH <= 8) {
    if (ct) {
      switch (s) {
#define VW_CASE(n) \
        case n:    \
          if constexpr (n % V == 0) return fwd_row_ct<T, L, FMA, NV, n, FULL, LH>(buf, nvec, lo, hi, emit); \
          break;
        VW_CT_SPACINGS(VW_CASE)
#undef VW_CASE
        default: break;
      }
    }
  }
  fwd_row_t<T, L, FMA, NV, 0, FULL, LH>(buf, nvec, s, lo, hi, taps, emit, taps_hi);
}

template <typename T, int L, bool FMA, int NV, int SC, int DIR, bool FULL = false>
__device__ __forceinline__ void inv_row_t(const T* buf, int nvec, int s, int dir, int off, const T* f, int taps,
                                          T (&acc)[NV][VT<T>::V]) {
  constexpr int V = VT<T>::V;
  using vec = typename VT<T>::v;
  for_vecs<L, NV, FULL>(nvec, [&](int k, int w) {
    const int t0 = w * V;
    if constexpr (L > 0 && SC > 0) {
      inv_window<T, L, FMA, SC, DIR>(buf, t0 + off, f, acc[k]);
    } else if constexpr (L > 0 && SC == 0) {
#pragma unroll
      for (int i = 0; i < L; ++i) {
        const vec v = *reinterpret_cast<const vec*>(buf + t0 + off + DIR * i * s);
        vmadd<FMA>(acc[k], v, f[i]);
        if ((i & 3) == 3) __builtin_amdgcn_sched_barrier(0);
      }
    } else {
      inv_branch<T, L, FMA>(buf, t0, s, dir, off, f, taps, acc[k]);
    }
#pragma unroll
    for (int e = 0; e < V; ++e) asm volatile("" : "+v"(acc[k][e]));
  });
}

template <typename T, int L, bool FMA, int NV, int S, int DIR, bool FULL>
__device__ __forceinline__ void inv_row_ct(const T* buf, int nvec, int off, const T* f, T (&acc)[NV][VT<T>::V]) {
  constexpr int V = VT<T>::V;
  using vec = typename VT<T>::v;
  static_assert(S % V == 0 && (L - 1) * S * (int)sizeof(T) < 65536, "aligned reads, 16-bit offsets");
  const T* const low = buf + off - (DIR > 0 ? 0 : (L - 1) * S);
  for_vecs<L, NV, FULL>(nvec, [&](int k, int w) {
    const int t0 = w * V;
    const unsigned a0 = lds_base(low + t0);
#pragma unroll
    for (int i = 0; i < L; ++i) {
      const vec v = lds_vec_at<vec>(a0 + (unsigned)((DIR > 0 ? i : L - 1 - i) * S * (int)sizeof(T)));
      vmadd<FMA>(acc[k], v, f[i]);
      if ((i & 3) == 3) __builtin_amdgcn_sched_barrier(0);
    }
#pragma unroll
    for (int e = 0; e < V; ++e) asm volatile("" : "+v"(acc[k][e]));
  });
}

template <typename T, int L, bool FMA, int NV, bool FULL = false>
__device__ __forceinline__ void inv_row(const T* buf, int nvec, int s, int dir, int off, const T* f, int taps, int ct,
                                        T (&acc)[NV][VT<T>::V]) {
  constexpr int V = VT<T>::V;
  if constexpr (L > 0) {
    if ((off & (V - 1)) == 0) {
      if (s == 1) {
        if (dir > 0) return inv_row_t<T, L, FMA, NV, 1, 1, FULL>(buf, nvec, s, dir, off, f, taps, acc);
        return inv_row_t<T, L, FMA, NV, 1, -1, FULL>(buf, nvec, s, dir, off, f, taps, acc);
      }
      if constexpr (V == 4) {
        if (s == 2) {
          if (dir > 0) return inv_row_t<T, L, FMA, NV, 2, 1, FULL>(buf, nvec, s, dir, off, f, taps, acc);
          return inv_row_t<T, L, FMA, NV, 2, -1, FULL>(buf, nvec, s, dir, off, f, taps, acc);
        }
      }
      if constexpr (L <= 8) {
        if (ct) {
          switch (s) {
#define VW_CASE(n)                                                                                  \
            case n:                                                                                 \
              if constexpr (n % V == 0) {                                                           \
                if (dir > 0) return inv_row_ct<T, L, FMA, NV, n, 1, FULL>(buf, nvec, off, f, acc);  \
                return inv_row_ct<T, L, FMA, NV, n, -1, FULL>(buf, nvec, off, f, acc);              \
              }                                                                                     \
              break;
            VW_CT_SPACINGS(VW_CASE)
#undef VW_CASE
            default: break;
          }
        }
      }
      if (dir > 0) return inv_row_t<T, L, FMA, NV, 0, 1, FULL>(buf, nvec, s, dir, off, f, taps, acc);
      return inv_row_t<T, L, FMA, NV, 0, -1, FULL>(buf, nvec, s, dir, off, f, taps, acc);
    }
  }
  inv_row_t<T, L, FMA, NV, -1, 1, FULL>(buf, nvec, s, dir, off, f, taps, acc);
}

template <typename T, int NV>
__device__ __forceinline__ void zero_regs(T (&r)[NV][VT<T>::V]) {
#pragma unroll
  for (int k = 0; k < NV; ++k)
#pragma unroll
    for (int e = 0; e < VT<T>::V; ++e) r[k][e] = T(0);
}

#ifndef VW_LONG_WAVES
#define VW_LONG_WAVES 4
#endif
#define VW_FUSED_W(L, W) ((L) <= 8 ? (W) : VW_LONG_WAVES)
#define VW_FUSED_BOUNDS(NV, W)                                                        \
  __attribute__((amdgpu_flat_work_group_size(1, ((NV) <= 4 && (NV) != 2) ? 512 : 1024), \
                 amdgpu_waves_per_eu((NV) == 2 ? 8 : (NV) <= 4 ? (W) : 4)))

template <typename T>
__device__ __forceinline__ T nf_step(T v, T z) {
  if constexpr (sizeof(T) == 8) return __builtin_fma(v, T(0), z);
  else return __builtin_fmaf(v, T(0), z);
}
template <typename T, int V>
__device__ __forceinline__ void nf_probe(T& z, const T (&v)[V]) {
#pragma unroll
  for (int e = 0; e < V; ++e) z = nf_step<T>(v[e], z);
}
template <typename T, int L, int NV, int V, bool FULL = false>
__device__ __forceinline__ void nf_probe_rows(T& z, const T (&v)[NV][V], int nvec) {
  for_vecs<L, NV, FULL>(nvec, [&](int k, int) { nf_probe<T, V>(z, v[k]); });
}
template <typename T>
__device__ __forceinline__ void nf_flag_row(int* flag, long long b, T z) {
  if (__any(z != z) && (threadIdx.x & 63) == 0) flag[b] = 1;
}

template <typename T, int L, bool FMA, int NV, bool VALIDATE, bool NFP = false, bool FULL = false, int LH = L>
__device__ __forceinline__ void fwd_level(const FwdArgs<T>& p, const T* X, int nvec, const LevelDesc& lv, T* dout,
                                          T* aout, bool vec_ok, unsigned long long flat0, T (&areg)[NV][VT<T>::V],
                                          T* nf = nullptr) {
  constexpr int V = VT<T>::V;
  const int N = p.N;
  const int ct = VALIDATE ? 0 : p.level_ct;
  fwd_row<T, L, FMA, NV, FULL, LH>(X, nvec, lv.s, p.lo, p.hi, p.taps, ct, [&](int k, int w, const T (&al)[V], const T (&ah)[V]) {
    const int t0 = w * V;
    store_vec<VW_FWD_STORE_AUX, FULL>(dout, t0, N, vec_ok, ah);
    if (aout) store_vec<VW_FWD_STORE_AUX, FULL>(aout, t0, N, vec_ok, al);
    if constexpr (VALIDATE) {
      check_out<T>(1, p.bad, flat0, t0, N, ah);
      check_out<T>(1, p.bad, flat0, t0, N, al);
    }
    if constexpr (NFP) {
      if (aout) nf_probe<T, V>(*nf, al);
    }
#pragma unroll
    for (int e = 0; e < V; ++e) areg[k][e] = al[e];
  }, p.taps_hi);
}

template <typename T, int L, bool FMA, int NV, bool HIST, int LH = L>
__global__ void VW_FUSED_BOUNDS(NV, VW_FUSED_W((L > LH ? L : LH), 8)) k_forward_fused(const FwdArgs<T> p) {
  constexpr int V = VT<T>::V;
  extern __shared__ __attribute__((aligned(16))) unsigned char smem[];
  T* X = reinterpret_cast<T*>(smem) + p.hlpad;
  T* Y = p.region1 ? reinterpret_cast<T*>(smem) + p.region1 + p.hlpad : X;
  const bool dbl = p.region1 != 0;
  const long long b = p.rev ? p.B - 1 - (long long)blockIdx.x : (long long)blockIdx.x;
  const int N = p.N;
  const int nvec = (N + V - 1) / V;
  const int NT = blockDim.x;
  const int tid = threadIdx.x;
  const bool vec_ok = (L > 0) || p.vec_io != 0;
  const unsigned long long flat0 = (unsigned long long)b * (unsigned long long)N;
  auto hist_of = [&](int j) -> const T* {
    if constexpr (!HIST) return nullptr;
    const LevelDesc& d = p.lv[j - 1];
    return d.mode == kHaloHistory ? p.hist[j - 1] + b * d.hist_len : nullptr;
  };

  T areg[NV][V];
  load_row_regs<T, NV>(areg, p.x + b * p.ldx, N, nvec, vec_ok, false);
  wait_vmem();
  if (p.validate) {
    for_vecs<L, NV>(nvec, [&](int k, int w) {
#pragma unroll
      for (int e = 0; e < V; ++e)
        if (w * V + e < N && !finite_t(areg[k][e])) atomicMin(p.bad, flat0 + (unsigned long long)(w * V + e));
    });
  }
  regs_to_level<T, L, NV>(X, areg, nvec, N, p.lv[0], p.npow2, hist_of(1));

  for (int j = 1; j <= p.J; ++j) {
    const LevelDesc lv = p.lv[j - 1];
    lds_barrier();
    T* dout = p.details + ((size_t)(j - 1) * (size_t)p.B + (size_t)b) * (size_t)N;
    T* aout = (j == p.J) ? p.approx + b * (size_t)N : nullptr;
    if (p.validate) fwd_level<T, L, FMA, NV, true, false, false, LH>(p, X, nvec, lv, dout, aout, vec_ok, flat0, areg);
    else fwd_level<T, L, FMA, NV, false, false, false, LH>(p, X, nvec, lv, dout, aout, vec_ok, flat0, areg);
    if (HIST && p.hist_update && lv.hist_len > 0) {
      T* hnew = p.hist[j - 1] + b * lv.hist_len;
      for (int q = tid; q < lv.hist_len; q += NT) hnew[q] = X[q + N - lv.hist_len];
    }
    if (j < p.J) {
      if (!dbl) lds_barrier();
      regs_to_level<T, L, NV>(Y, areg, nvec, N, p.lv[j], p.npow2, hist_of(j + 1));
      T* t = X; X = Y; Y = t;
    }
  }
}

__device__ __forceinline__ void lds_dma16(unsigned lds, const void* g, bool nt) {
  unsigned keep;
  if (nt) {
    asm volatile(
        "s_mov_b32 %0, m0\n\t"
        "s_mov_b32 m0, %2\n\t"
        "s_nop 0\n\t"
        "global_load_lds_dwordx4 %1, off nt\n\t"
        "s_mov_b32 m0, %0"
        : "=&s"(keep)
        : "v"(g), "s"(__builtin_amdgcn_readfirstlane(lds))
        : "memory");
  } else {
    asm volatile(
        "s_mov_b32 %0, m0\n\t"
        "s_mov_b32 m0, %2\n\t"
        "s_nop 0\n\t"
        "global_load_lds_dwordx4 %1, off\n\t"
        "s_mov_b32 m0, %0"
        : "=&s"(keep)
        : "v"(g), "s"(__builtin_amdgcn_readfirstlane(lds))
        : "memory");
  }
}

template <typename T>
__device__ __forceinline__ void dma_row(T* buf, const T* __restrict__ src, int nvec, bool nt) {
  constexpr int V = VT<T>::V;
  const int lane = threadIdx.x & 63, wv = __builtin_amdgcn_readfirstlane(threadIdx.x >> 6), nw = blockDim.x >> 6;
  for (int c = wv; c * 64 < nvec; c += nw)
    lds_dma16((unsigned)(uintptr_t)(buf + c * 64 * V), src + (size_t)(c * 64 + lane) * V, nt);
}

template <int N>
__device__ __forceinline__ void wait_vmcnt() {
  static_assert(N >= 0 && N < 64, "vmcnt range");
  __builtin_amdgcn_s_waitcnt((N & 0xF) | ((N >> 4) << 14) | (0x7 << 4) | (0xF << 8));
}

__device__ __forceinline__ void wait_vmcnt_rt(int n) {
  switch (__builtin_amdgcn_readfirstlane(n)) {
    case 0: wait_vmcnt<0>(); break;
    case 1: wait_vmcnt<1>(); break;
    case 2: wait_vmcnt<2>(); break;
    case 3: wait_vmcnt<3>(); break;
    case 4: wait_vmcnt<4>(); break;
    case 5: wait_vmcnt<5>(); break;
    case 6: wait_vmcnt<6>(); break;
    case 7: wait_vmcnt<7>(); break;
    case 8: wait_vmcnt<8>(); break;
    case 9: wait_vmcnt<9>(); break;
    case 10: wait_vmcnt<10>(); break;
    case 11: wait_vmcnt<11>(); break;
    case 12: wait_vmcnt<12>(); break;
    case 13: wait_vmcnt<13>(); break;
    case 14: wait_vmcnt<14>(); break;
    case 15: wait_vmcnt<15>(); break;
    case 16: wait_vmcnt<16>(); break;
    case 17: wait_vmcnt<17>(); break;
    case 18: wait_vmcnt<18>(); break;
    case 19: wait_vmcnt<19>(); break;
    case 20: wait_vmcnt<20>(); break;
    case 21: wait_vmcnt<21>(); break;
    case 22: wait_vmcnt<22>(); break;
    case 23: wait_vmcnt<23>(); break;
    case 24: wait_vmcnt<24>(); break;
    case 25: wait_vmcnt<25>(); break;
    case 26: wait_vmcnt<26>(); break;
    case 27: wait_vmcnt<27>(); break;
    case 28: wait_vmcnt<28>(); break;
    case 29: wait_vmcnt<29>(); break;
    case 30: wait_vmcnt<30>(); break;
    case 31: wait_vmcnt<31>(); break;
    case 32: wait_vmcnt<32>(); break;
    case 33: wait_vmcnt<33>(); break;
    case 34: wait_vmcnt<34>(); break;
    case 35: wait_vmcnt<35>(); break;
    case 36: wait_vmcnt<36>(); break;
    case 37: wait_vmcnt<37>(); break;
    case 38: wait_vmcnt<38>(); break;
    case 39: wait_vmcnt<39>(); break;
    case 40: wait_vmcnt<40>(); break;
    case 41: wait_vmcnt<41>(); break;
    case 42: wait_vmcnt<42>(); break;
    case 43: wait_vmcnt<43>(); break;
    case 44: wait_vmcnt<44>(); break;
    case 45: wait_vmcnt<45>(); break;
    case 46: wait_vmcnt<46>(); break;
    case 47: wait_vmcnt<47>(); break;
    case 48: wait_vmcnt<48>(); break;
    case 49: wait_vmcnt<49>(); break;
    case 50: wait_vmcnt<50>(); break;
    case 51: wait_vmcnt<51>(); break;
    case 52: wait_vmcnt<52>(); break;
    case 53: wait_vmcnt<53>(); break;
    case 54: wait_vmcnt<54>(); break;
    case 55: wait_vmcnt<55>(); break;
    case 56: wait_vmcnt<56>(); break;
    case 57: wait_vmcnt<57>(); break;
// ... 1150 lines not shown
```

vectorwave_amd/csrc/vw_internal.h:

```cpp
#pragma once
#include <hip/hip_runtime.h>
#include <atomic>
#include <cstdint>
#include "vw_taps.h"

namespace vw {

constexpr int kMaxTaps = 64;
constexpr int kMaxLevels = 24;
constexpr int kNV = 8;
constexpr int kMaxThreads = 1024;
constexpr int kLdsBytes = 160 * 1024;
constexpr int kSweepMinS = 16;
constexpr int kSweepChunk = 128;

enum HaloMode : int {
  kHaloPeriodic = 0,
  kHaloZero = 1,
  kHaloSymmetric = 2,
  kHaloFftPad = 3,
  kHaloHistory = 4
};

struct LevelDesc {
  int s;
  int hl, hr;
  int mode;
  int dir_a;
  int off_a;
  int dir_d;
  int off_d;
  int use_d;
  int hist_len;
  int own;
  int il_a, il_b;
  int ir_a, ir_b;
  int vs, ve;
};

template <typename T>
struct FwdArgs {
  const T* x;
  long long ldx;
  T* details;
  T* approx;
  long long B;
  int N;
  int J;
  int npow2;
  int hlpad;
  int region1;
  int vec_io;
  int unrolled;
  int dma_nt;
  int level_ct;
  int validate;
  int rev;
  unsigned long long* bad;
  T* hist[kMaxLevels];
  int hist_update;
  int taps;
  int taps_hi;
  int tap_lds;
  int blk_tight;
  int* nf_flag;
  T lo[kMaxTaps];
  T hi[kMaxTaps];
  LevelDesc lv[kMaxLevels];
};

template <typename T>
struct InvArgs {
  const T* details;
  const T* approx;
  T* y;
  long long B;
  int N;
  int J;
  int hlpad_a, hlpad_d;
  int region_d;
  int vec_io;
  int pair;
  int unrolled;
  int level_ct;
  int full;
  int plain;
  int waves;
  int db;
  int blk;
  int approx_zero;
  int rev;
  const T* thr;
  long long thr_ld;
  int soft;
  int taps;
  int taps_hi;
  int tap_lds;
  int blk_tight;
  int* nf_flag;
  T lo[kMaxTaps];
  T hi[kMaxTaps];
  LevelDesc lv[kMaxLevels];
};

template <typename T>
struct LevelArgs {
  const T* src_a;
  long long lda;
  const T* src_d;
  const T* src_d2;
  const T* thr2;
  int use_d2;
  const T* src_d3;
  const T* thr3;
  int use_d3;
  T* out_a;
  T* out_d;
  const T* hist;
  long long B;
  int N;
  int tile;
  int hlpad;
  int region_d, hlpad_d;
  int pair;
  const T* thr;
  int soft;
  int use_d;
  int vec_io;
  int validate;
  unsigned long long* bad;
  int npow2;
  int taps;
  T lo[kMaxTaps];
  T hi[kMaxTaps];
  LevelDesc lv;
};

constexpr int kMaxGroup = 8;
constexpr int kMultiInvNI = 8;
constexpr int kMultiPF = 6;
template <typename T>
struct MultiArgs {
  const T* src_a;
  long long lda;
  const T* src_d[kMaxGroup];
  T* out_d[kMaxGroup];
  T* out_a;
  const T* thr[kMaxGroup];
  long long B;
  int N;
  int tile;
  int nlev;
  int s0;
  int ext[kMaxGroup + 1];
  int region;
  int vec_io;
  int soft;
  int taps;
  int rblk;
  int pf;
  int pad;
  int* nf_flag;
  int slack;
  int ni;
  T lo[kMaxTaps];
  T hi[kMaxTaps];
};

enum ThrMethod { kThrUniversal = 0, kThrSure = 1, kThrMinimax = 2, kThrBayes = 3, kThrFixed = 4 };
constexpr int kSigmaRegN = 16384;
constexpr int kSureMaxN = 16384;
struct DenoiseConsts {
  double level_scale[kMaxLevels];
  double univ_c;
  double log_n;
  int method;
  int n;
};

constexpr int kRefPlanes = 2 * kMaxLevels + 3;
template <typename T>
struct RefScan {
  const T* p[kRefPlanes];
  long long ld[kRefPlanes];
  int len[kRefPlanes];
  int np;
  long long B;
  int N;
  int chunks;
  int* flag;
};
template <typename T>
struct RefArgs {
  const T* x;
  long long ldx;
  const T* det_in;
  T* details;
  T* approx;
  T* y;
  const T* thr;
  long long thr_ld;
  int soft;
  long long B;
  int N;
  int J;
  int L;
  int Lhi;
  int mode;
  int hist_mode;
  int hist_first;
  const T* hist_old[kMaxLevels];
  T* hist_new[kMaxLevels];
  int hist_len[kMaxLevels];
  int* flag;
  T* scratch;
  T lo[kMaxTaps];
  T hi[kMaxTaps];
  LevelDesc lv[kMaxLevels];
};
template <typename T>
hipError_t launch_flag_nonfinite(const RefScan<T>& a, hipStream_t st);
template <typename T>
hipError_t launch_ref_cascade(const RefArgs<T>& a, int grid, bool inverse, hipStream_t st);
int ref_scan_chunks(int N);

hipError_t launch_forward_mfma(const FwdArgs<float>& a, int lds, hipStream_t st);
hipError_t launch_inverse_mfma(const InvArgs<float>& a, int lds, hipStream_t st);

constexpr int kFinMaxN = 16384;
constexpr int kFinMaxTaps = 30;
constexpr int kFinPerThread = 16;
struct FinArgs {
  const double* x;
  long long ld;
  long long B;
  int N;
  int L;
  int tree;
  int validate;
  int wavelet;
  double k;
  double* out;
  unsigned long long* bad;
  double lo[kFinMaxTaps];
  double hi[kFinMaxTaps];
};
hipError_t launch_fin_analyze(const FinArgs& a, hipStream_t st);
hipError_t launch_fin_sharpe(const FinArgs& a, hipStream_t st);

constexpr int kEnergyWaves = kMaxThreads / 64;
constexpr int kEnergyRed = (kMaxLevels + 1) * kEnergyWaves;
constexpr int kEnergyUnrollMax = 8;
struct EnergyArgs {
  const double* x;
  long long ldx;
  double* out;
  long long B;
  int N;
  int J;
  int npow2;
  int hlpad;
  int region1;
  int red_off;
  int vec_io;
  int unrolled;
  int level_ct;
  int taps;
  double lo[kMaxTaps];
  double hi[kMaxTaps];
  LevelDesc lv[kMaxLevels];
};
struct EnergyPlanesArgs {
  const double* approx;
  const double* details;
  long long B;
  int N;
  int J;
  int vec_io;
  double* out;
};
hipError_t launch_energy_fused(const EnergyArgs& a, int threads, int lds_bytes, bool fma, int nv, int grid,
                               hipStream_t st);
hipError_t launch_energy_planes(const EnergyPlanesArgs& a, bool tree, int cus, hipStream_t st);

constexpr int kMraUnrollMax = 14;
template <typename T>
struct MraArgs {
  const T* details;
  const T* approx;
  T* out;
  long long B;
  int N;
  int J;
  int hlpad;
  int region1;
  int vec_io;
  int unrolled;
  int level_ct;
  int taps;
  T lo[kMaxTaps];
  T hi[kMaxTaps];
  LevelDesc lv[kMaxLevels];
};
template <typename T>
hipError_t launch_mra(const MraArgs<T>& a, int threads, int lds_bytes, bool fma, int nv, int grid, hipStream_t st);

constexpr int kMaxDevices = 64;
struct LdsOnce {
  std::atomic<int> limit[kMaxDevices];
};
template <typename Kern>
static hipError_t set_lds(Kern k, int lds_bytes, LdsOnce* once, int want = kLdsBytes) {
  if (lds_bytes <= 64 * 1024) return hipSuccess;
  int dev = 0;
  if (hipGetDevice(&dev) != hipSuccess || dev < 0) dev = 0;
  std::atomic<int>* f = dev < kMaxDevices ? &once->limit[dev] : nullptr;
  if (f && f->load(std::memory_order_acquire) >= lds_bytes) return hipSuccess;
  if (want < lds_bytes) want = lds_bytes;
  hipError_t e = hipFuncSetAttribute(reinterpret_cast<const void*>(k), hipFuncAttributeMaxDynamicSharedMemorySize, want);
  if (e != hipSuccess) return e;
  if (f) f->store(want, std::memory_order_release);
  return hipSuccess;
}

template <typename T>
hipError_t launch_forward_fused(const FwdArgs<T>& a, int threads, int lds_bytes, bool fma, int nv, hipStream_t st);
template <typename T>
hipError_t launch_forward_persist(const FwdArgs<T>& a, int threads, int lds_bytes, bool fma, int nv, hipStream_t st);
template <typename T>
hipError_t launch_forward_blk(const FwdArgs<T>& a, int threads, int lds_bytes, bool fma, int nv, hipStream_t st);
template <typename T>
hipError_t launch_inverse_fused(const InvArgs<T>& a, int threads, int lds_bytes, bool fma, int nv, hipStream_t st);
template <typename T>
hipError_t launch_forward_level(const LevelArgs<T>& a, int lds_bytes, bool fma, hipStream_t st);
template <typename T>
hipError_t launch_inverse_level(const LevelArgs<T>& a, int lds_bytes, bool fma, hipStream_t st);
template <typename T>
hipError_t launch_forward_sweep(const LevelArgs<T>& a, bool fma, hipStream_t st);
template <typename T>
hipError_t launch_inverse_sweep(const LevelArgs<T>& a, bool fma, hipStream_t st);
template <typename T>
hipError_t launch_inverse_sweepg(const LevelArgs<T>& a, int levels, int ka, int R, bool fma, hipStream_t st);
template <typename T>
hipError_t launch_forward_multi(const MultiArgs<T>& a, int lds_bytes, bool fma, hipStream_t st);

template <typename T>
hipError_t launch_inverse_multi(const MultiArgs<T>& a, int lds_bytes, bool fma, hipStream_t st);
template <typename T>
hipError_t launch_history_update(const T* level_in, long long ld_in, const T* old_hist, T* new_hist,
                                 long long B, int n, int hist_len, hipStream_t st);

hipError_t launch_level_threshold(const double* coeffs, long long level_stride, const double* sigma,
                                  const DenoiseConsts& k, long long B, int levels, double* thr, hipStream_t st);
hipError_t launch_noise_sigma(const double* coeffs, long long ld, long long B, int N, double scale_c,
                              double* sigma_out, double* thr_out, hipStream_t st);
hipError_t launch_median(const double* x, long long ld, long long B, int N, const double* center, double* median_out,
                         hipStream_t st);
hipError_t launch_abs_center(const double* x, long long ld, long long B, int N, const double* center, double* out,
                             hipStream_t st);
hipError_t launch_seq_std(const double* x, int n, double* out, hipStream_t st);
hipError_t launch_gather_abs(const double* src, const int* idx, int count, double* window, int wsize, int start,
                             hipStream_t st);
template <typename T>
hipError_t launch_transpose(const T* in, long long rows, long long cols, T* out, hipStream_t st);
template <typename T>
hipError_t launch_threshold(T* c, long long B, long long N, const T* thr, int soft, hipStream_t st);
template <typename T>
hipError_t launch_fill_uniform(T* x, long long count, unsigned long long seed, long long offset, hipStream_t st);
template <typename T>
hipError_t launch_single_haar_batch(const T* x, long long ldx, long long B, int N, T* approx, T* detail,
                                    hipStream_t st);

struct BlkLayout {
  int sh, pad;
};
constexpr BlkLayout blk_pad(int m, int nv, int tight = 0) {
  if (m <= 0 || m >= 16) return BlkLayout{30, 0};
  if (nv >= 8) return tight ? BlkLayout{4, 1} : BlkLayout{3, 1};
  if (m == 8) return BlkLayout{3, 2};
  return BlkLayout{2, 1};
}

int fused_max_threads();

}
```

vectorwave_amd/csrc/vw_plan.cpp:

```cpp
#include "vw_plan.h"

#include <algorithm>
#include <cstdio>
#include <cstdlib>
#include <cstring>
#include <type_traits>

namespace vw {

struct TuningKey {
  const char* name;
  void (*set)(Tuning& t, const Tuning& d, int v);
};
#define VW_KEY(name, stmt) {name, [](Tuning& t, const Tuning& d, int v) { (void)d; stmt; }}
static const TuningKey kTuningTable[] = {
    VW_KEY("VW_NV", t.nv = v < 0 ? d.nv : v <= 4 ? 4 : 8),
    VW_KEY("VW_FWD_PERSIST", t.fwd_persist = v < 0 ? d.fwd_persist : v != 0),
    VW_KEY("VW_FWD_BUF", t.fwd_buf = v < 0 ? d.fwd_buf : v),
    VW_KEY("VW_FORCE_TILED", t.force_tiled = v > 0),
    VW_KEY("VW_FWD_REV", t.fwd_rev = v < 0 ? 0 : v),
    VW_KEY("VW_INV_REV", t.inv_rev = v < 0 ? 0 : v),
    VW_KEY("VW_FWD_TILE", t.fwd_tile = v < 0 ? 0 : v),
    VW_KEY("VW_MULTI", t.multi = v < 0 ? d.multi : v != 0),
    VW_KEY("VW_MULTI_DIV", t.multi_div = v <= 0 ? d.multi_div : v),
    VW_KEY("VW_MULTI_TILE", t.multi_tile = v < 0 ? 0 : v),
    VW_KEY("VW_INV_BUF", t.inv_buf = v < 0 ? 0 : v),
    VW_KEY("VW_INV_TILE", t.inv_tile = v < 0 ? 0 : v),
    VW_KEY("VW_MULTI_RBLK", t.multi_rblk = v < 0 ? d.multi_rblk : v),
    VW_KEY("VW_MULTI_PF", t.multi_pf = v < 0 ? d.multi_pf : v),
    VW_KEY("VW_MULTI_PAD", t.multi_pad = v < 0 ? d.multi_pad : v),
    VW_KEY("VW_MULTI_INV_TILE", t.multi_inv_tile = v < 0 ? 0 : v),
    VW_KEY("VW_NO_SWEEP", t.no_sweep = v > 0),
    VW_KEY("VW_SWEEP_QC", t.sweep_qc = v >= 16 ? v : d.sweep_qc),
    VW_KEY("VW_UNROLL_MAX", t.unroll_max = v < 0 ? d.unroll_max : v),
    VW_KEY("VW_BLK", t.blk = v < 0 ? d.blk : v),
    VW_KEY("VW_FWD_NV", t.fwd_nv = v < 0 ? d.fwd_nv : v),
    VW_KEY("VW_INV_NV", t.inv_nv = v < 0 ? d.inv_nv : v),
    VW_KEY("VW_DEEP", t.deep = v < 0 ? d.deep : v != 0; t.deep_inv = v < 0 ? d.deep_inv : v != 0),
    VW_KEY("VW_DEEP_INV", t.deep_inv = v < 0 ? d.deep_inv : v != 0),
    VW_KEY("VW_DEEP_LDS", t.deep_lds = v <= 0 ? d.deep_lds : v),
    VW_KEY("VW_DEEP_WAVES", t.deep_waves = v <= 0 ? d.deep_waves : v),
    VW_KEY("VW_DEEP_PF_FWD", t.deep_pf_fwd = v <= 0 ? d.deep_pf_fwd : std::min(v, 16)),
    VW_KEY("VW_DEEP_PF_INV", t.deep_pf_inv = v <= 0 ? d.deep_pf_inv : std::min(v, 16)),
    VW_KEY("VW_SWEEP2", t.sweep2 = v < 0 ? d.sweep2 : v),
    VW_KEY("VW_SWEEP2_KA", t.sweep2_ka = v == 16 ? 16 : v == 8 ? 8 : d.sweep2_ka),
    VW_KEY("VW_SWEEP2_UC", t.sweep2_uc = v >= 32 ? v : d.sweep2_uc),
    VW_KEY("VW_SWEEP2_R", t.sweep2_r = v == 32 ? 32 : 0),
    VW_KEY("VW_SWEEP2_MINB", t.sweep2_minb = v < 0 ? d.sweep2_minb : v),
    VW_KEY("VW_BLK_FWD8", t.blk_fwd8 = v < 0 ? d.blk_fwd8 : v),
    VW_KEY("VW_DMA_NT", t.dma_nt = v < 0 ? d.dma_nt : v),
    VW_KEY("VW_MULTI_NI", t.multi_ni = v < 0 ? d.multi_ni : v == 4 ? 4 : 8),
    VW_KEY("VW_MFMA", t.mfma = v < 0 ? d.mfma : v),
    VW_KEY("VW_REF_GRID", t.ref_grid = v < 0 ? d.ref_grid : v),
    VW_KEY("VW_LEVEL_CT", t.level_ct = v < 0 ? d.level_ct : v != 0),
    VW_KEY("VW_ENERGY_FUSED", t.energy_fused = v < 0 ? d.energy_fused : v),
    VW_KEY("VW_MRA_FUSED", t.mra_fused = v < 0 ? d.mra_fused : v >= 2 ? 2 : v),
    VW_KEY("VW_BI", t.bi = v < 0 ? d.bi : v & 7),
    VW_KEY("VW_BI_LISTED", t.bi_listed = v < 0 ? d.bi_listed : v != 0),
    VW_KEY("VW_INV_WAVES", t.inv_waves = v == 6 || v == 8 ? v : d.inv_waves),
};
#undef VW_KEY

bool set_tuning(Tuning& t, const char* key, int v) {
  const Tuning d;
  for (const TuningKey& k : kTuningTable)
    if (!strcmp(k.name, key)) { k.set(t, d, v); return true; }
  return false;
}

Tuning read_tuning() {
  Tuning t;
  const Tuning d;
  for (const TuningKey& k : kTuningTable) {
    const char* e = getenv(k.name);
    if (e) k.set(t, d, *e == '\0' ? 1 : atoi(e));
  }
  return t;
}


int max_levels(int64_t N, int L) {
  if (L <= 0 || N <= L) return 0;
  int max_level = 1;
  const long long lm1 = L - 1;
  while (max_level < 10) {
    const long long scaled = lm1 * (1LL << (max_level - 1)) + 1LL;
    if (scaled > N) break;
    max_level++;
  }
  return max_level - 1;
}

int64_t upsampled_length(int L, int level) {
  const int64_t up = (level <= 1) ? 1 : ((int64_t)1 << (level - 1));
  return (int64_t)(L - 1) * up + 1;
}

int ref_mode(int boundary) {
  return boundary == VW_PERIODIC ? kHaloPeriodic : boundary == VW_ZERO_PADDING ? kHaloZero : kHaloSymmetric;
}

static void sym_decide(int wid, int L, int level, int* ap, int* dh, int* dp, int* dg) {
  int detailPlus = 1, deltaG = 0, deltaH = 0;
  const bool isHaar = L <= 2;
  int approxPlus = isHaar ? 1 : 0;
  if (isHaar) {
    deltaG = 0;
    deltaH = (level <= 1) ? 0 : -1;
  } else if (wid == VW_WID_DB6) {
    deltaH = (level <= 1) ? 0 : -1;
    deltaG = (level >= 3) ? 1 : 0;
  } else if (wid == VW_WID_DB8) {
    deltaH = (level <= 1) ? 0 : 1;
    deltaG = (level >= 2) ? 1 : 0;
  } else if (wid == VW_WID_SYM4) {
    approxPlus = 1; detailPlus = 0; deltaH = 0; deltaG = 0;
  } else if (wid == VW_WID_SYM8) {
    if (level <= 1) { deltaH = 0; deltaG = 0; }
    else if (level == 2) { deltaH = 1; deltaG = 0; }
    else { deltaH = 1; deltaG = 1; }
  } else if (wid == VW_WID_COIF2) {
    approxPlus = 1; deltaH = (level <= 1) ? 0 : 1; detailPlus = 0; deltaG = 0;
  } else if (wid == VW_WID_COIF3) {
    detailPlus = 0;
    if (level <= 1) { deltaH = 0; deltaG = 0; } else { deltaH = -1; deltaG = 1; }
  } else if (L >= 12) {
    if (level <= 1) { deltaH = 0; deltaG = 0; }
    else { const bool even = level % 2 == 0; deltaH = even ? 0 : -1; deltaG = even ? 0 : -1; }
  } else {
    if (level <= 1) { deltaH = 0; deltaG = 0; } else { deltaH = -1; deltaG = 0; }
  }
  *ap = approxPlus; *dh = deltaH; *dp = detailPlus; *dg = deltaG;
}

static int compute_tau(int base_len, int level) {
  const int lm1 = base_len - 1;
  if (level <= 1) return std::max(0, lm1 / 2);
  const long long up = 1LL << (level - 1);
  const long long Lj = (long long)lm1 * up + 1LL;
  const long long tau = (Lj - 1LL) / 2LL;
  if (tau < 0) return 0;
  if (tau > 2147483647LL) return 2147483647;
  return (int)tau;
}

static int next_pow2(int64_t n) {
  int64_t p = 1;
  while (p < n) p <<= 1;
  return (int)p;
}

static bool is_pow2(int64_t n) { return n > 0 && (n & (n - 1)) == 0; }

static void branch_extent(int N, int tmax, int L, int s, int dir, int off, int* hl, int* hr) {
  const long long reach = (long long)(L - 1) * s;
  long long mn, mx;
  if (dir > 0) { mn = off; mx = (long long)tmax + reach + off; }
  else { mn = (long long)off - reach; mx = (long long)tmax + off; }
  *hl = (int)std::max<long long>(*hl, -mn);
  *hr = (int)std::max<long long>(*hr, mx - (N - 1));
}

static inline int64_t round_up(int64_t v, int64_t a) { return (v + a - 1) / a * a; }
template <typename T> static constexpr int vec_width() { return 16 / (int)sizeof(T); }
static bool aligned16(const void* p) { return ((uintptr_t)p & 15u) == 0; }
static bool plus_zero(const LevelDesc& d) { return d.dir_a == 1 && d.dir_d == 1 && d.off_a == 0 && d.off_d == 0; }

struct StepAlign {
  const void* in;
  const void* out;
  const void* planes;
  size_t plane_bytes;
  bool buf(int b) const {
    return b == kBufIn ? aligned16(in) : b == kBufOut ? aligned16(out) : b == kBufWs1 ? plane_bytes % 16 == 0 : true;
  }
  bool plane(int k) const { return (((uintptr_t)planes + (uintptr_t)k * plane_bytes) & 15u) == 0; }
};

template <typename P>
static void plan_error(P* p, int code, const char* fmt, int a = 0, int b = 0) {
  p->error = code;
  snprintf(p->msg, sizeof(p->msg), fmt, a, b);
}

static bool fused_plan(const Tuning& tu, int64_t N, int V, int elem, int64_t lds_elems_extra, int* threads, int* nv,
                       int* lds, bool* fit, int nv_req = 0) {
  const int64_t nvec = (N + V - 1) / V;
  int want = tu.nv;
  if ((nvec + want - 1) / want > 512) want = 8;
  if (nv_req == 2 && nvec % 2 == 0 && nvec / 2 <= kMaxThreads) want = 2;
  const int64_t th = (nvec + want - 1) / want;
  if (th > kMaxThreads) return false;
  const int64_t bytes = lds_elems_extra * elem;
  if (bytes > kLdsBytes) return false;
  *nv = want;
  *threads = (int)th;
  *lds = (int)bytes;
  *fit = (int64_t)(want - 1) * th <= nvec;
  return true;
}

static void set_halo_images(LevelDesc& d, int64_t N, int64_t npow2, int V, int threads, int nv) {
  int64_t s_el = 0, e_el = N;
  d.il_a = 0; d.il_b = 1; d.ir_a = 0; d.ir_b = -1;
  switch (d.mode) {
    case kHaloPeriodic:
      d.il_a = 1; d.il_b = (int)-N; d.ir_a = 1; d.ir_b = (int)N;
      s_el = d.hr; e_el = N - d.hl;
      break;
    case kHaloSymmetric:
      d.il_a = -1; d.il_b = -1; d.ir_a = -1; d.ir_b = (int)(2 * N - 1);
      s_el = d.hl; e_el = N - d.hr;
// ... 321 lines not shown
      MultiArgs<T>& m = s.multi;
      m.lda = lda;
      bool io = al.buf(src) && al.buf(s.dst);
      for (int k = 0; k < g; ++k) io = io && al.plane(j - 1 + k);
      m.ext[g] = 0;
      for (int k = g - 1; k >= 0; --k)
        m.ext[k] = m.ext[k + 1] + (int)round_up((int64_t)(L - 1) * lv[j - 1 + k].s, V);
      m.B = c.B; m.N = (int)N; m.tile = mtile; m.nlev = g; m.s0 = lv[j - 1].s;
      m.region = (int)round_up(m.ext[0] + mtile + V, V);
      m.vec_io = (N % V == 0) && (lda % V == 0) && io;
      m.taps = L;
      s.lds = (int)(2 * m.region * sizeof(T));
      src = s.dst;
      lda = N;
      j = je;
      continue;
    }
    const bool sweep = lv[j - 1].s >= kSweepMinS && has_unrolled_taps(L) && !tu.no_sweep;
    PlanStep<T>& s = add_step(p->steps, sweep ? kStepSweep : kStepTile, j, j, src, j == J ? kBufOut : nxt);
    LevelArgs<T>& a = s.lvl;
    a.lv = lv[j - 1];
    const int hp = (int)round_up(a.lv.hl, V);
    const int64_t fit = ((int64_t)kLdsBytes / (int64_t)sizeof(T) - hp - 2 * V) / V * V;
    const int tile = (int)std::min<int64_t>(tile_max, fit);
    if (tile < 64 * V) return plan_error(p, VW_ERR_UNSUPPORTED, "level %d halo (%d samples) exceeds LDS", j, a.lv.hl);
    a.lda = lda;
    a.B = c.B; a.N = (int)N; a.tile = sweep ? tu.sweep_qc : tile; a.hlpad = hp;
    a.vec_io = (N % V == 0) && (lda % V == 0) && al.buf(src) && al.buf(s.dst) && al.plane(j - 1);
    a.validate = validate; a.npow2 = p->args.npow2; a.taps = L;
    s.lds = sweep ? 0 : (int)((hp + tile + V) * sizeof(T));
    s.hist_update = hist && c.hist_update;
    src = s.dst;
    lda = N;
  }
  p->nf_probed = !p->steps.empty() && p->steps.back().probe;
}

template <typename C>
static int hi_taps(const C& c) { return c.Lhi > 0 ? c.Lhi : c.L; }

static int listed_taps(const Tuning& tu, int L, bool two_lengths) {
  return (two_lengths && tu.bi_listed && !has_unrolled_taps(L) && L < kMaxTaps && has_unrolled_taps(L + 1)) ? L + 1 : L;
}

template <typename T>
static void plan_forward_taps(const Tuning& tu, const FwdCall<T>& call, int taps, FwdPlan<T>* p, bool bi = false) {
  FwdCall<T> c = call;
  const int Llo = call.L, Lhi = hi_taps(call);
  c.L = taps;
  c.Lhi = 0;
  const bool hist = c.hist != nullptr;
  p->fma = c.flags & VW_FLAG_FMA;
  p->validate = c.flags & VW_FLAG_VALIDATE;
  FwdArgs<T>& a = p->args;
  a.B = c.B; a.N = (int)c.N; a.J = c.J; a.ldx = c.ldx;
  a.npow2 = next_pow2(c.N);
  a.validate = p->validate;
  a.hist_update = c.hist_update ? 1 : 0;
  a.taps = c.L; a.taps_hi = c.L;
  int mixed = 0;
  const int max_hl = forward_levels(c, a.lv, Llo, Lhi, &mixed);
  if (mixed)
    return plan_error(p, VW_ERR_UNSUPPORTED, "FFT switch: one filter of level %d is in the FFT region, one is not (mixed level)",
                      mixed);
  p->snapshot = (c.flags & VW_FLAG_REF_NONFINITE) && hist && c.hist_update && c.hist_snap && !c.hist_first && c.J >= 2;
  const bool padded = taps != Llo || taps != Lhi;
  p->ref_nf = (c.flags & VW_FLAG_REF_NONFINITE) && !p->validate && (padded || (!c.single_level && c.J >= 2)) &&
              !(c.flags & VW_FLAG_FFT_SWITCH) && (!hist || !c.hist_update || c.hist_first || c.hist_snap);
  p->fused = plan_forward_fused(tu, c, max_hl, p, bi);
  if (bi && p->fused && !hist && p->nv != 2 && p->kernel == kFwdFused &&
      ((tu.bi & 4) || (a.unrolled && has_unrolled_pair(Llo, Lhi)))) {
    a.taps = Llo; a.taps_hi = Lhi;
    a.unrolled = a.unrolled && has_unrolled_pair(Llo, Lhi);
  }
  if (!p->fused) plan_forward_levels(tu, c, p);
  reserve_ref<T>(tu, c.cus, c.B, c.N, p);
}

void plan_energy(const Tuning& tu, const FwdCall<double>& c, EnergyPlan* p) {
  constexpr int V = vec_width<double>();
  const int64_t N = c.N, nvec = (N + V - 1) / V;
  const int L = c.L, J = c.J;
  EnergyArgs& a = p->args;
  p->fma = c.flags & VW_FLAG_FMA;
  p->fused = false;
  if (!(c.flags & VW_FLAG_TREE_SUMS) || tu.energy_fused == 0 || tu.force_tiled || J < 1 || J > kMaxLevels ||
      (c.flags & (VW_FLAG_VALIDATE | VW_FLAG_REF_NONFINITE)) || c.hist || c.single_level)
    return;
  const int max_hl = forward_levels(c, a.lv);
  for (int j = 0; j < J; ++j)
    if (a.lv[j].mode == kHaloFftPad) return;
  const int hlpad = (int)round_up(max_hl, V);
  const int64_t region = round_up(hlpad + nvec * V + V, V);
  int threads = 0, lds = 0, nv = 4;
  bool fit = false;
  bool dbl = p->fma && (2 * region + kEnergyRed) * (int64_t)sizeof(double) <= kLdsBytes / 2 &&
             fused_plan(tu, N, V, sizeof(double), 2 * region + kEnergyRed, &threads, &nv, &lds, &fit);
  if (!dbl && !fused_plan(tu, N, V, sizeof(double), region + kEnergyRed, &threads, &nv, &lds, &fit)) return;
  threads = (int)round_up(threads, 64);
  fit = (int64_t)(nv - 1) * threads <= nvec;
  const bool io_aligned = (c.ldx % V == 0) && (N % V == 0) && aligned16(c.x);
  a.B = c.B; a.N = (int)N; a.J = J; a.ldx = c.ldx;
  a.npow2 = next_pow2(N);
  a.taps = L;
  for (int j = 0; j < J; ++j) set_halo_images(a.lv[j], N, a.npow2, V, threads, nv);
  a.hlpad = hlpad;
  a.region1 = dbl ? (int)region : 0;
  a.red_off = (int)((dbl ? 2 : 1) * region);
  a.vec_io = io_aligned;
  a.unrolled = io_aligned && fit && L <= tu.unroll_max && L <= kEnergyUnrollMax && has_unrolled_taps(L);
  a.level_ct = tu.level_ct;
  const int wpe = (nv <= 4 && L <= 8) ? 6 : 4;
  const int by_waves = std::max(1, wpe * 4 / (threads / 64));
  const int by_lds = std::max(1, kLdsBytes / std::max(lds, 1));
  p->grid = (int)std::min<int64_t>(c.B, (int64_t)std::max(c.cus, 1) * std::min(by_waves, by_lds));
  p->threads = threads; p->nv = nv; p->lds = lds;
  p->fused = true;
}


template <typename T>
static void inverse_levels(const InvCall<T>& c, int Llo, int Lhi, LevelDesc* lv, int* max_hl, int* max_hr) {
  constexpr int V = vec_width<T>();
  const int tmax = (int)((c.N + V - 1) / V * V - 1);
  for (int j = 1; j <= c.J; ++j) {
    LevelDesc& d = lv[j - 1];
    memset(&d, 0, sizeof(d));
    d.s = 1 << (j - 1);
    d.use_d = (c.detail_mask >> (j - 1)) & 1u;
    d.mode = ref_mode(c.boundary);
    if (c.boundary == VW_SYMMETRIC && !c.single_level) {
      int ap, dh, dp, dg;
      sym_decide(c.wid, Llo, j, &ap, &dh, &dp, &dg);
      const int tauH = compute_tau(Llo, j) + dh;
      const int tauG = compute_tau(Lhi, j) + dg;
      d.dir_a = ap ? 1 : -1; d.off_a = ap ? -tauH : tauH;
      d.dir_d = dp ? 1 : -1; d.off_d = dp ? -tauG : tauG;
    } else if (c.boundary == VW_SYMMETRIC) {
      const int dir = (c.flags & VW_FLAG_BATCH_SYM_INVERSE) ? 1 : -1;
      d.dir_a = d.dir_d = dir; d.off_a = d.off_d = 0;
    } else {
      d.dir_a = d.dir_d = 1; d.off_a = d.off_d = 0;
    }
    int hl = 0, hr = 0;
    branch_extent((int)c.N, tmax, c.L, d.s, d.dir_a, d.off_a, &hl, &hr);
    branch_extent((int)c.N, tmax, c.L, d.s, d.dir_d, d.off_d, &hl, &hr);
    d.hl = hl; d.hr = hr;
    *max_hl = std::max(*max_hl, hl);
    *max_hr = std::max(*max_hr, hr);
  }
}

template <typename T>
static bool plan_inverse_fused(const Tuning& tu, const InvCall<T>& c, bool pair, int max_hl, int max_hr,
                               InvPlan<T>* p, bool bi = false) {
  constexpr int V = vec_width<T>();
  const int64_t N = c.N, nvec = (N + V - 1) / V;
  const int L = c.L, J = c.J;
  const bool periodic = c.boundary == VW_PERIODIC;
  InvArgs<T>& a = p->args;
  const int hlpad = (int)round_up(max_hl, V);
  const int64_t region = round_up(hlpad + nvec * V + max_hr + V, V);
  int threads = 0, lds = 0, nv = 4;
  const bool blk_pref = !bi && tu.blk > 0 && L >= tu.blk && has_unrolled_taps(L) && periodic;
  bool db = !pair && (tu.inv_buf ? tu.inv_buf == 2 : (c.B <= 2LL * c.cus && !blk_pref));
  bool fused = false, fit = false;
  const bool inv_io = (N % V == 0) && aligned16(c.details) && aligned16(c.approx) && aligned16(c.y);
  const int inv_nv2 = (tu.inv_nv == 2 && inv_io && L <= 8 && L <= tu.unroll_max && has_unrolled_taps(L)) ? 2 : 0;
  if (!tu.force_tiled) {
    if (pair || db) fused = fused_plan(tu, N, V, sizeof(T), 2 * region, &threads, &nv, &lds, &fit, inv_nv2);
    if (!fused && !pair) {
      db = false;
      fused = fused_plan(tu, N, V, sizeof(T), region, &threads, &nv, &lds, &fit, inv_nv2);
    }
  }
  if (!fused) return false;
  for (int j = 0; j < J; ++j) set_halo_images(a.lv[j], N, 0, V, threads, nv);
  a.db = db ? 1 : 0;
  a.hlpad_a = hlpad; a.hlpad_d = hlpad; a.region_d = (int)region;
  a.vec_io = inv_io;
  a.unrolled = a.vec_io && fit && L <= tu.unroll_max;
  a.pair = pair;
  a.rev = tu.inv_rev;
  a.level_ct = tu.level_ct;
  a.full = tu.level_ct && a.unrolled && (int64_t)threads * nv == nvec;
  p->kernel = pair ? kInvPair : db ? kInvDb : kInvSeq;
  if (!bi && tu.blk > 0 && L >= tu.blk && has_unrolled_taps(L) && nv != 2 && !pair && !db && periodic && a.unrolled &&
      (int64_t)threads * nv == nvec) {
    const BlkPlan b = blk_plan<T>(a.lv, J, L, nvec, nv, true);
    a.blk_tight = b.tight;
    if (b.ok) {
      a.blk = 1;
      a.tap_lds = (int)(b.buf * V);
      lds = (int)(b.buf * 16) + 2 * L * (int)sizeof(T);
      p->kernel = kInvBlk;
    }
  }
  if (std::is_same<T, float>::value) {
    bool ok = !bi && (tu.mfma & 2) && p->fma && !pair && periodic && a.vec_io;
    for (int j = 0; ok && j < J; ++j) ok = plus_zero(a.lv[j]);
    if (const int mfma_lds = mfma_layout(ok, L, J, N, 0, &a.hlpad_a, &a.tap_lds)) {
      lds = mfma_lds;
      p->kernel = kInvMfma;
    }
  }
  p->nf_probed = p->ref_nf && (p->kernel == kInvSeq || p->kernel == kInvBlk);
  bool plain = a.full && p->kernel == kInvSeq && sizeof(T) == 8 && nv == 4 && L <= 8 && periodic && !c.thr &&
               !c.approx_zero && !a.rev && !p->ref_nf;
  for (int j = 0; plain && j < J; ++j)
    plain = a.lv[j].use_d && plus_zero(a.lv[j]) && a.lv[j].hl == 0 && a.lv[j].hr <= N;
  a.plain = plain ? 1 : 0;
  a.waves = tu.inv_waves;
  p->threads = threads; p->nv = nv; p->lds = lds;
  return true;
}

template <typename T>
static void inverse_multi_layout(const Tuning& tu, const LevelDesc* lv, int j0, int g, int L, int mtile,
                                 MultiArgs<T>& m) {
  constexpr int V = vec_width<T>();
  m.region = (int)round_up(mtile + m.ext[g - 1] + V, V);
  m.rblk = tu.multi_rblk;
  m.pf = tu.multi_pf && m.vec_io && (int64_t)(mtile + m.ext[g - 1]) / V <= (int64_t)kMultiPF * 256;
  m.pad = tu.multi_pad && m.pf && m.rblk && has_unrolled_taps(L);
  if (m.pad) {
    const int nvmax = (mtile + m.ext[g - 1]) / V + 1;
    m.region = (nvmax + nvmax / 8 + 1) * V;
  }
  m.slack = 160;
  m.ni = kMultiInvNI;
  if (tu.multi_ni == 4 && sizeof(T) == 8 && m.pad) {
    auto fits = [&](int64_t t) {
      if ((t + m.ext[g - 1]) / V > (int64_t)kMultiPF * 256) return false;
      for (int k = 0; k < g; ++k) {
        const int64_t s = lv[j0 - 1 + k].s, M = s % V == 0 ? s / V : 0;
        const int64_t nv = (t + (k > 0 ? m.ext[k - 1] : 0)) / V;
        const bool blk = M == 1 || M == 2 || M == 4 || M == 8;
        if (blk ? (nv + 4 * M - 1) / (4 * M) * M > 256 : nv > 4 * 256) return false;
      }
      return true;
    };
    int64_t t = mtile;
    while (t >= 512 && !fits(t)) t -= 64 * V;
    if (t >= 512) {
      m.ni = 4;
      m.tile = (int)t;
      const int nvmax = (int)((t + m.ext[g - 1]) / V) + 1;
      m.region = (nvmax + nvmax / 4 + 1) * V;
    }
  }
}

template <typename T>
static void plan_inverse_levels(const Tuning& tu, const InvCall<T>& c, bool pair, InvPlan<T>* p) {
  constexpr int V = vec_width<T>();
  const int64_t N = c.N;
  const int L = c.L, J = c.J;
  const bool periodic = c.boundary == VW_PERIODIC;
  const LevelDesc* lv = p->args.lv;
  const int tile_max = tu.inv_tile ? tu.inv_tile / V * V : 1024;
  const size_t plane = (size_t)c.B * (size_t)N;
  p->res.ws_bytes = 2 * plane * sizeof(T) + 256;
  const StepAlign al{c.approx, c.y, c.details, plane * sizeof(T)};
  auto plane_al = [&](int j) { return !lv[j - 1].use_d || al.plane(j - 1); };
  const int mtile = tu.multi_inv_tile >= 64 * V ? tu.multi_inv_tile / V * V : multi_tile<T>(tu);
  int groups[kMaxLevels], start_of[kMaxLevels + 1] = {};
  level_groups(tu, lv, J, L, V, mtile, !pair && periodic, groups);
  for (int j = 1; j <= J; ++j) {
    if (groups[j - 1] < 2) continue;
    int64_t ext = 0;
    for (int k = 0; k < groups[j - 1]; ++k) ext += round_up((int64_t)(L - 1) * lv[j - 1 + k].s, V);
    if ((mtile + ext) / V <= (int64_t)kMultiInvNI * 256) start_of[j + groups[j - 1] - 1] = j;
  }
  char in_group[kMaxLevels + 1] = {};
  for (int e = 1; e <= J; ++e)
    for (int k = start_of[e]; start_of[e] > 0 && k <= e; ++k) in_group[k] = 1;
  int cur = c.approx_zero ? kBufNone : kBufIn;
  for (int j = J; j >= 1; --j) {
    const int nxt = cur == kBufWs0 ? kBufWs1 : kBufWs0;
    if (!pair && periodic && !in_group[j] && al.buf(cur) && aligned16(c.details) && aligned16(c.y) &&
        deep_plan<T>(tu, lv, j, j, L, N, true, nullptr)) {
      int jl = j;
      while (jl > 1 && !in_group[jl - 1] && deep_plan<T>(tu, lv, jl - 1, j, L, N, true, nullptr)) --jl;
      PlanStep<T>& s = add_step(p->steps, kStepDeep, jl, j, cur, jl == 1 ? kBufOut : nxt);
      s.lds = deep_plan<T>(tu, lv, jl, j, L, N, true, &s.deep);
      deep_segments<T>(tu, c.cus, c.B, &s.deep);
      s.deep.lda = N; s.deep.B = c.B; s.deep.taps = L; s.deep.soft = c.soft;
      cur = s.dst;
      j = jl;
      continue;
    }
    if (start_of[j] > 0) {
      const int j0 = start_of[j], g = j - j0 + 1;
      PlanStep<T>& s = add_step(p->steps, kStepMulti, j0, j, cur, j0 == 1 ? kBufOut : nxt);
      MultiArgs<T>& m = s.multi;
      s.probe = p->ref_nf && j0 == 1;
      bool io = al.buf(cur) && al.buf(s.dst);
      for (int k = 0; k < g; ++k) {
        io = io && plane_al(j0 + k);
        m.ext[k] = (k > 0 ? m.ext[k - 1] : 0) + (int)round_up((int64_t)(L - 1) * lv[j0 - 1 + k].s, V);
      }
      m.B = c.B; m.N = (int)N; m.tile = mtile; m.nlev = g; m.s0 = lv[j0 - 1].s;
      m.vec_io = (N % V == 0) && io;
      m.soft = c.soft; m.taps = L;
      inverse_multi_layout<T>(tu, lv, j0, g, L, mtile, m);
      s.lds = (int)((2 * m.region + m.slack * V) * sizeof(T));
      cur = s.dst;
      j = j0;
      continue;
    }
    if (tu.sweep2 && !tu.deep_inv && !tu.no_sweep && !pair && j >= 2 && has_unrolled_taps(L)) {
      int G = 0, ka = 0, R = 0;
      for (int levels = std::min(tu.sweep2 >= 3 ? 3 : 2, j); levels >= 2 && !G; --levels)
        if (sweepg_plan<T>(tu, lv, j, levels, L, N, in_group, start_of, &ka, &R)) G = levels;
      if (G) {
        PlanStep<T>& s = add_step(p->steps, kStepSweepG, j - G + 1, j, cur, j == G ? kBufOut : nxt);
        LevelArgs<T>& a = s.lvl;
        a.lv = lv[j - 1];
        a.use_d = lv[j - 1].use_d;
        a.use_d2 = lv[j - 2].use_d;
        if (G == 3) a.use_d3 = lv[j - 3].use_d;
        a.soft = c.soft;
        a.B = c.B; a.N = (int)N; a.taps = L;
        s.G = G == 2 ? 2 : 4; s.ka = ka; s.R = R;
        a.tile = (int)round_up(tu.sweep2_uc, s.G * ka);
        cur = s.dst;
        j -= G - 1;
        continue;
      }
    }
    const bool sweep = lv[j - 1].s >= kSweepMinS && has_unrolled_taps(L) && !tu.no_sweep;
    PlanStep<T>& s = add_step(p->steps, sweep ? kStepSweep : kStepTile, j, j, cur, j == 1 ? kBufOut : nxt);
    LevelArgs<T>& a = s.lvl;
    a.lv = lv[j - 1];
    const int hp = (int)round_up(a.lv.hl, V);
    const int64_t fit = ((int64_t)kLdsBytes / (int64_t)sizeof(T) / 2 - hp - a.lv.hr - 2 * V) / V * V;
    const int tile = (int)std::min<int64_t>(tile_max, fit);
    if (tile < 64 * V) return plan_error(p, VW_ERR_UNSUPPORTED, "level %d halo exceeds LDS", j);
    const int64_t reg = round_up(hp + tile + a.lv.hr + V, V);
    a.use_d = a.lv.use_d;
    a.B = c.B; a.N = (int)N; a.tile = sweep ? tu.sweep_qc : tile; a.hlpad = hp; a.hlpad_d = hp; a.region_d = (int)reg;
    a.pair = pair; a.soft = c.soft; a.taps = L;
    a.vec_io = (N % V == 0) && al.buf(s.dst) && al.buf(cur) && plane_al(j);
    s.lds = sweep ? 0 : (int)(2 * reg * sizeof(T));
    cur = s.dst;
  }
  p->nf_probed = !p->steps.empty() && p->steps.back().probe;
}

template <typename T>
static void plan_inverse_taps(const Tuning& tu, const InvCall<T>& call, int taps, InvPlan<T>* p, bool bi = false) {
  InvCall<T> c = call;
  const int Llo = call.L, Lhi = hi_taps(call);
  const bool pair = c.single_level || c.boundary == VW_ZERO_PADDING;
  if (pair && Lhi < Llo)
    return plan_error(p, VW_ERR_UNSUPPORTED, "pairwise inverse: the reference indexes past its high-pass array (%d < %d taps)",
                      Lhi, Llo);
  c.L = pair ? Llo : taps;
  c.Lhi = 0;
  p->fma = c.flags & VW_FLAG_FMA;
  const bool padded = !pair && (c.L != Llo || c.L != Lhi);
  p->ref_nf = (c.flags & VW_FLAG_REF_NONFINITE) && (padded || (!c.single_level && c.J >= 2));
  InvArgs<T>& a = p->args;
  a.B = c.B; a.N = (int)c.N; a.J = c.J;
  a.approx_zero = c.approx_zero; a.thr_ld = c.thr_ld; a.soft = c.soft; a.taps = c.L; a.taps_hi = c.L;
  int max_hl = 0, max_hr = 0;
  inverse_levels(c, Llo, Lhi, a.lv, &max_hl, &max_hr);
  p->fused = plan_inverse_fused(tu, c, pair, max_hl, max_hr, p, bi);
  if (bi && p->fused && !pair && p->nv != 2 && (p->kernel == kInvSeq || p->kernel == kInvDb) &&
      ((tu.bi & 4) || (a.unrolled && has_unrolled_pair(Llo, Lhi)))) {
    a.taps = Llo; a.taps_hi = Lhi;
    a.unrolled = a.unrolled && has_unrolled_pair(Llo, Lhi);
    a.full = 0;
    a.plain = 0;
  }
  if (!p->fused) plan_inverse_levels(tu, c, pair, p);
  reserve_ref<T>(tu, c.cus, c.B, c.N, p);
}

template <typename T>
void plan_mra(const Tuning& tu, const InvCall<T>& c, MraPlan<T>* p) {
  constexpr int V = vec_width<T>();
  const int64_t N = c.N, nvec = (N + V - 1) / V;
  const int L = c.L, J = c.J;
  MraArgs<T>& a = p->args;
  p->fma = c.flags & VW_FLAG_FMA;
  p->fused = false;
  if (tu.mra_fused == 0 || tu.force_tiled || c.single_level || J < 1 || J > kMaxLevels || L < 1 || L > kMaxTaps ||
      (c.flags & (VW_FLAG_VALIDATE | VW_FLAG_REF_NONFINITE)) || (c.Lhi != 0 && c.Lhi != L) || c.thr)
    return;
  InvCall<T> k = c;
  k.detail_mask = ~0u;
  k.approx_zero = 0;
  int max_hl = 0, max_hr = 0;
  inverse_levels(k, L, L, a.lv, &max_hl, &max_hr);
  const int64_t hlpad = round_up(max_hl, V);
  const int64_t region = round_up(hlpad + nvec * V + max_hr + V, V);
  int threads = 0, lds = 0, nv = 4;
  bool fit = false;
  if (!fused_plan(tu, N, V, sizeof(T), 2 * region, &threads, &nv, &lds, &fit)) return;
  threads = (int)round_up(threads, 64);
  fit = (int64_t)(nv - 1) * threads <= nvec;
  const bool io_aligned = (N % V == 0) && aligned16(c.details) && aligned16(c.approx) && aligned16(c.y);
  a.B = c.B; a.N = (int)N; a.J = J;
  a.taps = L;
  for (int j = 0; j < J; ++j) set_halo_images(a.lv[j], N, 0, V, threads, nv);
  a.hlpad = (int)hlpad;
  a.region1 = (int)region;
  a.vec_io = io_aligned;
  a.unrolled = io_aligned && fit && L <= tu.unroll_max && L <= kMraUnrollMax && has_unrolled_taps(L);
  a.level_ct = tu.level_ct;
  if (tu.mra_fused == 1 && !a.unrolled && io_aligned && fit && L <= tu.unroll_max && has_unrolled_taps(L)) return;
  const int wpe = (nv <= 4 && !(a.unrolled && L > 8)) ? 6 : 4;
  const int by_waves = std::max(1, wpe * 4 / (threads / 64));
  const int by_lds = std::max(1, kLdsBytes / std::max(lds, 1));
  p->grid = (int)std::min<int64_t>(c.B, (int64_t)std::max(c.cus, 1) * std::min(by_waves, by_lds));
  p->threads = threads; p->nv = nv; p->lds = lds;
  p->fused = true;
}
template void plan_mra<float>(const Tuning&, const InvCall<float>&, MraPlan<float>*);
template void plan_mra<double>(const Tuning&, const InvCall<double>&, MraPlan<double>*);

template <typename T>
void plan_forward(const Tuning& tu, const FwdCall<T>& c, FwdPlan<T>* p) {
  const int Lmax = std::max(c.L, hi_taps(c)), taps = listed_taps(tu, Lmax, c.L != hi_taps(c));
  if ((tu.bi & 1) && c.L != hi_taps(c) && !c.hist) {
    plan_forward_taps(tu, c, Lmax, p, true);
    if (p->error != VW_OK || p->args.taps_hi != p->args.taps) return;
    *p = FwdPlan<T>();
  }
  plan_forward_taps(tu, c, taps, p);
  if (p->error != VW_OK && taps != Lmax) {
    *p = FwdPlan<T>();
    plan_forward_taps(tu, c, Lmax, p);
  }
}

template <typename T>
void plan_inverse(const Tuning& tu, const InvCall<T>& c, InvPlan<T>* p) {
  const int Lmax = std::max(c.L, hi_taps(c)), taps = listed_taps(tu, Lmax, c.L != hi_taps(c));
  if ((tu.bi & 2) && c.L != hi_taps(c)) {
    plan_inverse_taps(tu, c, Lmax, p, true);
    if (p->error == VW_OK && p->args.taps_hi != p->args.taps) return;
    *p = InvPlan<T>();
  }
  plan_inverse_taps(tu, c, taps, p);
  if (p->error != VW_OK && taps != Lmax) {
    *p = InvPlan<T>();
    plan_inverse_taps(tu, c, Lmax, p);
  }
}

template void plan_forward<float>(const Tuning&, const FwdCall<float>&, FwdPlan<float>*);
template void plan_forward<double>(const Tuning&, const FwdCall<double>&, FwdPlan<double>*);
template void plan_inverse<float>(const Tuning&, const InvCall<float>&, InvPlan<float>*);
template void plan_inverse<double>(const Tuning&, const InvCall<double>&, InvPlan<double>*);

}
```

vectorwave_amd/csrc/vw_plan.h:

```cpp
#pragma once
#include "../../include/vectorwave_amd.h"
#include "vw_internal.h"
#include "vw_deep.h"

#include <vector>

namespace vw {

struct Tuning {
  int nv = 4;
  bool fwd_persist = true;
  int fwd_buf = 0;
  bool force_tiled = false;
  int fwd_rev = 0, inv_rev = 0;
  int dma_nt = -1;
  int fwd_tile = 0;
  bool multi = true;
  int multi_div = 4;
  int multi_tile = 0;
  int inv_buf = 0;
  int inv_tile = 0;
  int multi_rblk = 1;
  int multi_pf = 1;
  int multi_pad = 1;
  int multi_inv_tile = 0;
  int multi_ni = 4;
  bool no_sweep = false;
  int sweep_qc = kSweepChunk;
  int unroll_max = kMaxTaps;
  int blk = 10;
  bool deep = true;
  bool deep_inv = false;
  int deep_lds = 80;
  int deep_waves = 4;
  int deep_pf_fwd = 1;
  int deep_pf_inv = 1;
  int fwd_nv = 0;
  int inv_nv = 0;
  int sweep2 = 3;
  int sweep2_ka = 8;
  int sweep2_uc = 2048;
  int sweep2_r = 0;
  int sweep2_minb = 64;
  int blk_fwd8 = 1;
  int ref_grid = 0;
  int level_ct = 1;
  int mfma = 0;
  int energy_fused = 1;
  int bi = 3;
  int inv_waves = 6;
  int mra_fused = 1;
  int bi_listed = 1;
};

bool set_tuning(Tuning& t, const char* key, int v);
Tuning read_tuning();

int max_levels(int64_t N, int L);
int64_t upsampled_length(int L, int level);
int ref_mode(int boundary);

template <typename T>
struct FwdCall {
  const T* x = nullptr;
  int64_t B = 0, N = 0, ldx = 0;
  const double* lo = nullptr;
  const double* hi = nullptr;
  int L = 0, boundary = VW_PERIODIC, J = 1;
  unsigned flags = 0;
  T* details = nullptr;
  T* approx = nullptr;
  bool single_level = false;
  int mode_override = -1;
  T* const* hist = nullptr;
  bool hist_update = false;
  T* const* hist_snap = nullptr;
  bool hist_first = false;
  int cus = 256;
  int Lhi = 0;
};

template <typename T>
struct InvCall {
  const T* details = nullptr;
  const T* approx = nullptr;
  int64_t B = 0, N = 0;
  const double* lo = nullptr;
  const double* hi = nullptr;
  int L = 0, wid = VW_WID_OTHER, boundary = VW_PERIODIC, J = 1;
  unsigned detail_mask = ~0u;
  int approx_zero = 0;
  unsigned flags = 0;
  T* y = nullptr;
  bool single_level = false;
  const T* thr = nullptr;
  int soft = 0;
  int64_t thr_ld = 0;
  int cus = 256;
  int Lhi = 0;
};

enum PlanKernel : int {
  kFwdFused, kFwdPersist, kFwdBlk, kFwdMfma,
  kInvPair, kInvSeq, kInvDb, kInvBlk, kInvMfma,
  kStepDeep, kStepMulti, kStepSweepG, kStepSweep, kStepTile
};
enum PlanBuf : int { kBufNone, kBufIn, kBufWs0, kBufWs1, kBufOut };

template <typename T>
struct PlanStep {
  int kind;
  int jlo, jhi;
  int src, dst;
  int lds;
  int G, ka, R;
  int probe;
  int hist_update;
  union {
    LevelArgs<T> lvl;
    MultiArgs<T> multi;
    DeepArgs<T> deep;
  };
};

struct PlanReserve {
  size_t ws_bytes = 0;
  int64_t nf_rows = 0;
  int ref_grid = 0;
};

template <typename T, typename Args>
struct Plan {
  int error = VW_OK;
  char msg[96] = "";
  bool fused = false;
  int kernel = kFwdFused;
  int threads = 0, nv = 4, lds = 0;
  bool fma = false, validate = false;
  bool snapshot = false;
  bool ref_nf = false;
  bool nf_probed = false;
  PlanReserve res;
  Args args{};
  std::vector<PlanStep<T>> steps;
};
template <typename T> using FwdPlan = Plan<T, FwdArgs<T>>;
template <typename T> using InvPlan = Plan<T, InvArgs<T>>;

struct EnergyPlan {
  bool fused = false;
  bool fma = false;
  int threads = 0, nv = 4, lds = 0;
  int grid = 0;
  EnergyArgs args{};
};
void plan_energy(const Tuning& tu, const FwdCall<double>& c, EnergyPlan* p);

template <typename T>
struct MraPlan {
  bool fused = false;
  bool fma = false;
  int threads = 0, nv = 4, lds = 0;
  int grid = 0;
  MraArgs<T> args{};
};
template <typename T> void plan_mra(const Tuning& tu, const InvCall<T>& c, MraPlan<T>* p);

template <typename T> void plan_forward(const Tuning& tu, const FwdCall<T>& c, FwdPlan<T>* p);
template <typename T> void plan_inverse(const Tuning& tu, const InvCall<T>& c, InvPlan<T>* p);

}
```

vectorwave_amd/engine.py:

```python
from __future__ import annotations

import ctypes
import threading
from ctypes import byref, c_double, c_int64, c_void_p
from typing import Optional, Sequence, Tuple

import numpy as np

from . import _native as nat
from .errors import InvalidArgumentException, raise_for_status

try:
    import torch
except Exception:
    torch = None


def _is_device_tensor(a) -> bool:
    return torch is not None and isinstance(a, torch.Tensor) and a.is_cuda


def _one_length(lo, hi, what: str) -> int:
    if len(lo) != len(hi):
        raise InvalidArgumentException(f"{what} takes one filter length, got {len(lo)} low-pass and {len(hi)} "
# ... 21 lines not shown
        self._keep = None

    @classmethod
    def get(cls, device: Optional[int] = None) -> "Engine":
        if device is None:
            device = torch.cuda.current_device() if (torch is not None and torch.cuda.is_available()) else 0
        with cls._lock:
            eng = cls._instances.get(device)
            if eng is None:
                eng = cls(device)
                cls._instances[device] = eng
            return eng

    def close(self) -> None:
        if self.ctx:
            with Engine._lock:
                if Engine._instances.get(self.device) is self:
                    del Engine._instances[self.device]
            _check(self.lib.vw_ctx_destroy(self.ctx))
            self.ctx = None

    def bind_torch_stream(self) -> None:
        s = torch.cuda.current_stream(self.device).cuda_stream
        if s != self._ext_stream:
            _check(self.lib.vw_ctx_use_null_stream(self.ctx) if s == 0 else
                   self.lib.vw_ctx_set_stream(self.ctx, c_void_p(s)))
            self._ext_stream = s

    def set_option(self, key: str, value: int) -> None:
        _check(self.lib.vw_ctx_set_option(self.ctx, key.encode(), int(value)))

    def options(self, **kv):
        import contextlib

        @contextlib.contextmanager
        def cm():
            for k, v in kv.items():
                self.set_option(k, v)
            try:
                yield self
            finally:
                for k in kv:
                    self.set_option(k, -1)
        return cm()

    def synchronize(self) -> None:
        _check(self.lib.vw_ctx_synchronize(self.ctx))

    def enable_timing(self, on: bool = True) -> None:
        _check(self.lib.vw_ctx_enable_timing(self.ctx, 1 if on else 0))

    def reset_timing(self) -> None:
        _check(self.lib.vw_ctx_reset_timing(self.ctx))

    def kernel_time(self, family: str) -> Tuple[float, int]:
        ms = c_double()
        n = c_int64()
        _check(self.lib.vw_ctx_kernel_time(self.ctx, family.encode(), byref(ms), byref(n)))
        return ms.value, n.value

    def kernel_spans(self, family: str, ref_event, max_n: int = 4096):
        st = (c_double * max_n)()
        en = (c_double * max_n)()
        n = c_int64()
        _check(self.lib.vw_ctx_kernel_spans(self.ctx, family.encode(), c_void_p(ref_event.cuda_event), max_n, st, en,
                                            byref(n)))
        return [(st[i], en[i]) for i in range(min(n.value, max_n))]

    def _prep(self, x, dtype=None):
        if _is_device_tensor(x):
            if dtype is not None:
                want = torch.float32 if np.dtype(dtype) == np.float32 else torch.float64
                if x.dtype != want:
                    x = x.to(want)
            elif x.dtype not in (torch.float64, torch.float32):
                x = x.to(torch.float64)
            if not x.is_contiguous():
                x = x.contiguous()
            if x.device.index != self.device:
                raise ValueError(f"tensor on cuda:{x.device.index}, engine on cuda:{self.device}")
            self.bind_torch_stream()
            if self._keep is not None:
                self._keep.append(x)
            return x, True, c_void_p(x.data_ptr()), x.dtype == torch.float32
        if torch is not None and isinstance(x, torch.Tensor):
            x = x.detach().numpy()
        a = np.asarray(x)
        if dtype is None:
            dtype = np.float32 if a.dtype == np.float32 else np.float64
        a = np.ascontiguousarray(a, dtype=dtype)
        return a, False, a.ctypes.data_as(c_void_p), a.dtype == np.float32

    def _empty(self, like, is_dev, shape):
        if is_dev:
            t = torch.empty(shape, dtype=like.dtype, device=like.device)
            if self._keep is not None:
                self._keep.append(t)
            return t
        return np.empty(shape, dtype=like.dtype)

    @staticmethod
    def _ptr(a, is_dev):
        if a is None:
            return None
        return c_void_p(a.data_ptr()) if is_dev else a.ctypes.data_as(c_void_p)

    @staticmethod
    def _flags(flags: int, is_dev: bool) -> int:
        return flags if is_dev else flags | nat.FLAG_HOST_MEMORY

    def forward(self, x, lo: Sequence[float], hi: Sequence[float], wavelet_id: int, boundary: int, levels: int,
                flags: int):
        xa, dev, xp, f32 = self._prep(x)
        one = xa.ndim == 1
        B, N = (1, xa.shape[0]) if one else xa.shape
        det = self._empty(xa, dev, (levels, N) if one else (levels, B, N))
        app = self._empty(xa, dev, (N,) if one else (B, N))
        if len(lo) != len(hi):
            fn = self.lib.vw_modwt_forward_bi_f32 if f32 else self.lib.vw_modwt_forward_bi_f64
            _check(fn(self.ctx, xp, B, N, N, nat.taps_array(lo), len(lo), nat.taps_array(hi), len(hi), wavelet_id,
                      boundary, levels, self._flags(flags, dev), self._ptr(det, dev), self._ptr(app, dev)))
            return det, app
        fn = self.lib.vw_modwt_forward_f32 if f32 else self.lib.vw_modwt_forward_f64
        _check(fn(self.ctx, xp, B, N, N, nat.taps_array(lo), nat.taps_array(hi), len(lo), wavelet_id, boundary,
                  levels, self._flags(flags, dev), self._ptr(det, dev), self._ptr(app, dev)))
        return det, app

    def inverse(self, details, approx, lo, hi, wavelet_id: int, boundary: int, levels: int, flags: int,
                detail_mask: int = 0xFFFFFFFF, approx_zero: bool = False, shape=None):
        ref = approx if approx is not None else details
        ra, dev, _, f32 = self._prep(ref)
        da = dp = None
        if details is not None:
            da, _, dp, _ = self._prep(details, np.float32 if f32 else np.float64)
        aa = ap = None
        if approx is not None:
            aa, _, ap, _ = self._prep(approx, np.float32 if f32 else np.float64)
        if shape is None:
            shape = tuple(aa.shape if aa is not None else da.shape[1:])
        one = len(shape) == 1
        B, N = (1, shape[0]) if one else shape
        y = self._empty(ra, dev, shape)
        if len(lo) != len(hi):
            fn = self.lib.vw_modwt_inverse_bi_f32 if f32 else self.lib.vw_modwt_inverse_bi_f64
            _check(fn(self.ctx, dp, ap, B, N, nat.taps_array(lo), len(lo), nat.taps_array(hi), len(hi), wavelet_id,
                      boundary, levels, detail_mask & 0xFFFFFFFF, 1 if approx_zero else 0, self._flags(flags, dev),
                      self._ptr(y, dev)))
            return y
        fn = self.lib.vw_modwt_inverse_f32 if f32 else self.lib.vw_modwt_inverse_f64
        _check(fn(self.ctx, dp, ap, B, N, nat.taps_array(lo), nat.taps_array(hi), len(lo), wavelet_id, boundary, levels,
                  detail_mask & 0xFFFFFFFF, 1 if approx_zero else 0, self._flags(flags, dev), self._ptr(y, dev)))
        return y

    def forward1(self, x, lo, hi, boundary: int, flags: int):
        xa, dev, xp, f32 = self._prep(x, np.float64)
        one = xa.ndim == 1
        B, N = (1, xa.shape[0]) if one else xa.shape
        app = self._empty(xa, dev, xa.shape)
        det = self._empty(xa, dev, xa.shape)
        if len(lo) != len(hi):
            _check(self.lib.vw_modwt1_forward_bi_f64(self.ctx, xp, B, N, N, nat.taps_array(lo), len(lo),
                                                     nat.taps_array(hi), len(hi), boundary, self._flags(flags, dev),
                                                     self._ptr(app, dev), self._ptr(det, dev)))
            return app, det
        _check(self.lib.vw_modwt1_forward_f64(self.ctx, xp, B, N, N, nat.taps_array(lo), nat.taps_array(hi), len(lo),
                                              boundary, self._flags(flags, dev), self._ptr(app, dev),
                                              self._ptr(det, dev)))
        return app, det

    def inverse1(self, approx, detail, lo, hi, boundary: int, flags: int):
        aa, dev, ap, _ = self._prep(approx, np.float64)
        da, _, dp, _ = self._prep(detail, np.float64)
        one = aa.ndim == 1
        B, N = (1, aa.shape[0]) if one else aa.shape
        y = self._empty(aa, dev, aa.shape)
        if len(lo) != len(hi):
            _check(self.lib.vw_modwt1_inverse_bi_f64(self.ctx, ap, dp, B, N, nat.taps_array(lo), len(lo),
                                                     nat.taps_array(hi), len(hi), boundary, self._flags(flags, dev),
                                                     self._ptr(y, dev)))
            return y
        _check(self.lib.vw_modwt1_inverse_f64(self.ctx, ap, dp, B, N, nat.taps_array(lo), nat.taps_array(hi), len(lo),
                                              boundary, self._flags(flags, dev), self._ptr(y, dev)))
        return y

    def denoise(self, x, lo, hi, wavelet_id: int, boundary: int, levels: int, threshold: float, soft: bool,
                flags: int, want_thresholds: bool = False):
        xa, dev, xp, _ = self._prep(x, np.float64)
        one = xa.ndim == 1
        B, N = (1, xa.shape[0]) if one else xa.shape
        y = self._empty(xa, dev, xa.shape)
        thr = self._empty(xa, dev, (B,)) if want_thresholds else None
        _check(self.lib.vw_swt_denoise_f64(self.ctx, xp, B, N, N, nat.taps_array(lo), nat.taps_array(hi),
                                           _one_length(lo, hi, "denoise"),
                                           wavelet_id, boundary, levels, float(threshold), 1 if soft else 0,
                                           self._flags(flags, dev), self._ptr(y, dev), self._ptr(thr, dev)))
        return (y, thr) if want_thresholds else y

    def wavelet_denoise(self, x, lo, hi, wavelet_id: int, boundary: int, levels: int, method: int, fixed: float,
                        soft: bool, flags: int, want_thresholds: bool = False):
        xa, dev, xp, _ = self._prep(x, np.float64)
        one = xa.ndim == 1
        B, N = (1, xa.shape[0]) if one else xa.shape
        y = self._empty(xa, dev, xa.shape)
        thr = self._empty(xa, dev, (max(levels, 1), B)) if want_thresholds else None
        _check(self.lib.vw_wavelet_denoise_f64(self.ctx, xp, B, N, N, nat.taps_array(lo), nat.taps_array(hi),
                                               _one_length(lo, hi, "wavelet_denoise"),
                                               wavelet_id, boundary, levels, method, float(fixed), 1 if soft else 0,
                                               self._flags(flags, dev), self._ptr(y, dev), self._ptr(thr, dev)))
        return (y, thr) if want_thresholds else y

    def _rows(self, x, N):
        xa, dev, xp, _ = self._prep(x, np.float64)
        B, ld = (1, xa.shape[0]) if xa.ndim == 1 else xa.shape
        n = ld if N is None else int(N)
        if n > ld:
            raise ValueError(f"N={n} exceeds the row width {ld}")
        return xa, dev, xp, B, n, ld

    def fin_analyze(self, prices, lo, hi, anomaly_k: float, flags: int = 0, N: Optional[int] = None):
        xa, dev, xp, B, n, ld = self._rows(prices, N)
        out = self._empty(xa, dev, (5, B))
        _check(self.lib.vw_fin_analyze_f64(self.ctx, xp, B, n, ld, nat.taps_array(lo), nat.taps_array(hi),
                                           _one_length(lo, hi, "fin_analyze"),
                                           float(anomaly_k), self._flags(flags, dev), self._ptr(out, dev)))
        return out

    def fin_sharpe(self, returns, risk_free: float, flags: int = 0, N: Optional[int] = None):
        xa, dev, xp, B, n, ld = self._rows(returns, N)
        out = self._empty(xa, dev, (B,))
        _check(self.lib.vw_fin_sharpe_f64(self.ctx, xp, B, n, ld, float(risk_free), self._flags(flags, dev),
                                          self._ptr(out, dev)))
        return out

    def fin_wavelet_sharpe(self, returns, lo, hi, boundary: int, risk_free: float, flags: int = 0,
                           N: Optional[int] = None):
        xa, dev, xp, B, n, ld = self._rows(returns, N)
        out = self._empty(xa, dev, (B,))
        _check(self.lib.vw_fin_wavelet_sharpe_f64(self.ctx, xp, B, n, ld, nat.taps_array(lo), nat.taps_array(hi),
                                                  _one_length(lo, hi, "fin_wavelet_sharpe"), int(boundary),
                                                  float(risk_free), self._flags(flags, dev), self._ptr(out, dev)))
        return out

    def energy(self, x, lo: Sequence[float], hi: Sequence[float], wavelet_id: int, boundary: int, levels: int,
               flags: int = 0, N: Optional[int] = None):
        xa, dev, xp, B, n, ld = self._rows(x, N)
        out = self._empty(xa, dev, (levels + 1, B))
        _check(self.lib.vw_modwt_energy_f64(self.ctx, xp, B, n, ld, nat.taps_array(lo), nat.taps_array(hi),
                                            _one_length(lo, hi, "energy"),
                                            wavelet_id, boundary, levels, self._flags(flags, dev),
                                            self._ptr(out, dev)))
        return out

    def energy_planes(self, details, approx, flags: int = 0):
        aa, dev, ap, _ = self._prep(approx, np.float64)
        B, N = (1, aa.shape[0]) if aa.ndim == 1 else aa.shape
        J, dp = 0, None
        if details is not None and details.shape[0] > 0:
            da, ddev, dp, _ = self._prep(details, np.float64)
            J = int(da.shape[0])
            if ddev != dev or tuple(da.shape[1:]) != tuple(aa.shape):
                raise ValueError("details must be [J] + approx.shape, in the same memory as approx")
        out = self._empty(aa, dev, (J + 1, B))
        _check(self.lib.vw_energy_planes_f64(self.ctx, dp, ap, B, N, J, self._flags(flags, dev),
                                             self._ptr(out, dev)))
        return out

    def mra_planes(self, details, approx, lo: Sequence[float], hi: Sequence[float], wavelet_id: int, boundary: int,
                   flags: int = 0):
        aa, dev, ap, f32 = self._prep(approx)
        da, ddev, dp, _ = self._prep(details, np.float32 if f32 else np.float64)
        if ddev != dev or da.ndim != aa.ndim + 1 or tuple(da.shape[1:]) != tuple(aa.shape) or da.shape[0] < 1:
            raise ValueError("details must be [J] + approx.shape with J >= 1, in the same memory as approx")
        J = int(da.shape[0])
        B, N = (1, aa.shape[0]) if aa.ndim == 1 else aa.shape
        out = self._empty(aa, dev, (J + 1,) + tuple(aa.shape))
        fn = self.lib.vw_mra_planes_f32 if f32 else self.lib.vw_mra_planes_f64
        _check(fn(self.ctx, dp, ap, B, N, nat.taps_array(lo), nat.taps_array(hi), _one_length(lo, hi, "mra_planes"),
                  wavelet_id, boundary, J, self._flags(flags, dev), self._ptr(out, dev)))
        return out

    def mra(self, x, lo: Sequence[float], hi: Sequence[float], wavelet_id: int, boundary: int, levels: int,
            flags: int = 0):
        xa, dev, xp, f32 = self._prep(x)
        B, N = (1, xa.shape[0]) if xa.ndim == 1 else xa.shape
        out = self._empty(xa, dev, (levels + 1,) + tuple(xa.shape))
        fn = self.lib.vw_modwt_mra_f32 if f32 else self.lib.vw_modwt_mra_f64
        _check(fn(self.ctx, xp, B, N, N, nat.taps_array(lo), nat.taps_array(hi), _one_length(lo, hi, "mra"),
                  wavelet_id, boundary, levels, self._flags(flags, dev), self._ptr(out, dev)))
        return out

    def transpose(self, a, rows: int, cols: int):
        aa, dev, ap, f32 = self._prep(a)
        if (aa.numel() if dev else aa.size) != rows * cols:
            raise ValueError("transpose: size mismatch")
        out = self._empty(aa, dev, (rows * cols,))
        fn = self.lib.vw_transpose_f32 if f32 else self.lib.vw_transpose_f64
        _check(fn(self.ctx, ap, rows, cols, self._flags(0, dev), self._ptr(out, dev)))
        return out

    def noise_sigma(self, coeffs):
        ca, dev, cp, _ = self._prep(coeffs, np.float64)
        one = ca.ndim == 1
        B, N = (1, ca.shape[0]) if one else ca.shape
        sig = self._empty(ca, dev, (B,))
        _check(self.lib.vw_noise_sigma_f64(self.ctx, cp, B, N, self._flags(0, dev), self._ptr(sig, dev)))
        return sig

    def threshold_inplace(self, coeffs, thresholds, soft: bool):
        ca, dev, cp, _ = self._prep(coeffs, np.float64)
        one = ca.ndim == 1
        B, N = (1, ca.shape[0]) if one else ca.shape
        ta, _, tp, _ = self._prep(thresholds, np.float64)
        _check(self.lib.vw_threshold_f64(self.ctx, cp, B, N, tp, 1 if soft else 0, self._flags(0, dev)))
        if ca is not coeffs:
            if dev:
                coeffs.copy_(ca)
            else:
                np.copyto(coeffs, ca)
        return coeffs

    def capture(self, fn) -> "Graph":
        self.bind_torch_stream()
        _check(self.lib.vw_capture_begin(self.ctx))
        self._keep = []
        done = False
        result = None
        try:
            result = fn()
            done = True
        finally:
            keep, self._keep = self._keep, None
            g = c_void_p()
            st = self.lib.vw_capture_end(self.ctx, byref(g))
            if not done and st == 0:
                self.lib.vw_graph_destroy(g)
        _check(st)
        return Graph(self, g, keep=keep, result=result)

    def fill_uniform(self, x, seed: int, offset: int = 0):
        if not _is_device_tensor(x):
            raise TypeError("fill_uniform needs a CUDA tensor")
        self.bind_torch_stream()
        fn = self.lib.vw_fill_uniform_f32 if x.dtype == torch.float32 else self.lib.vw_fill_uniform_f64
        _check(fn(self.ctx, c_void_p(x.data_ptr()), x.numel(), ctypes.c_uint64(seed), offset))
        return x


class Graph:

    def __init__(self, engine: Engine, handle: c_void_p, keep=None, result=None):
        self.engine = engine
        self.handle = handle
        self._keep = keep or []
        self.result = result

    def launch(self, count: int = 1) -> None:
        _check(self.engine.lib.vw_graph_launch(self.handle, int(count)))

    def close(self) -> None:
        if self.handle:
            _check(self.engine.lib.vw_graph_destroy(self.handle))
            self.handle = None
        self._keep = []

    def __del__(self):
        try:
            self.close()
        except Exception:
            pass


def version() -> str:
    return nat.load().vw_version().decode()


def max_levels(N: int, L: int) -> int:
    return int(nat.load().vw_max_levels(N, L))
```

Measured before the change: 48520.

## Fuse MODWT forward and inverse into one round-trip kernel, including graph capture

Adds a fused round-trip kernel that runs the forward transform and the inverse reconstruction in one launch. Each block keeps its forward results in registers or LDS and reconstructs the row directly, so the inverse no longer re-reads details and approximation from global memory. During graph capture, a forward kernel followed by a matching inverse is patched into a single fused node, and a direct roundtrip API is exposed as well. Fusion only applies under strict conditions (periodic boundary, fp64, matching plans, non-overlapping buffers); otherwise the separate kernels run as before. The risks are higher register and LDS pressure, which lowers occupancy, and more complex capture logic.

```diff
diff --git a/include/vectorwave_amd.h b/include/vectorwave_amd.h
--- a/include/vectorwave_amd.h
+++ b/include/vectorwave_amd.h
@@ -203,6 +203,13 @@
 VW_API vw_status vw_capture_end(vw_ctx *ctx, vw_graph **out);
 VW_API vw_status vw_graph_launch(vw_graph *graph, int64_t count);
 VW_API vw_status vw_graph_destroy(vw_graph *graph);
+VW_API vw_status vw_graph_stats(vw_graph *graph, int *kernel_nodes, int *fused_pairs);
+
+VW_API vw_status vw_modwt_roundtrip_f64(vw_ctx *ctx, const double *x, int64_t B, int64_t N, int64_t ldx,
+                                        const double *lo, const double *hi, const double *rlo, const double *rhi,
+                                        int L, int wavelet_id, int boundary, int J, unsigned flags, double *details,
+                                        double *approx, double *y);
+VW_API vw_status vw_roundtrip_occupancy(vw_ctx *ctx, int64_t N, int L, int J, unsigned flags, int *per_cu);
 
 typedef struct vw_pipeline vw_pipeline;
 VW_API vw_status vw_pipeline_create(vw_ctx *fwd_ctx, vw_ctx *inv_ctx, int elem_bytes, int sets, void *const *x,
diff --git a/vectorwave_amd/_native.py b/vectorwave_amd/_native.py
--- a/vectorwave_amd/_native.py
+++ b/vectorwave_amd/_native.py
@@ -116,6 +116,10 @@
     "vw_capture_end": (c_int, [c_void_p, POINTER(c_void_p)]),
     "vw_graph_launch": (c_int, [c_void_p, c_int64]),
     "vw_graph_destroy": (c_int, [c_void_p]),
+    "vw_graph_stats": (c_int, [c_void_p, POINTER(c_int), POINTER(c_int)]),
+    "vw_modwt_roundtrip_f64": (c_int, [c_void_p, c_void_p, c_int64, c_int64, c_int64, _dp, _dp, _dp, _dp, c_int, c_int,
+                                       c_int, c_int, c_uint, c_void_p, c_void_p, c_void_p]),
+    "vw_roundtrip_occupancy": (c_int, [c_void_p, c_int64, c_int, c_int, c_uint, POINTER(c_int)]),
     "vw_pipeline_create": (c_int, [c_void_p, c_void_p, c_int, c_int, c_void_p, c_void_p, c_void_p, c_void_p, c_int64,
                                    c_int64, _dp, _dp, c_int, c_int, c_int, c_int, c_uint, POINTER(c_void_p)]),
     "vw_pipeline_run": (c_int, [c_void_p, c_int64]),
diff --git a/vectorwave_amd/csrc/vw_capi.cpp b/vectorwave_amd/csrc/vw_capi.cpp
--- a/vectorwave_amd/csrc/vw_capi.cpp
+++ b/vectorwave_amd/csrc/vw_capi.cpp
@@ -59,6 +59,14 @@
 struct vw_graph;
 struct vw_ctx;
 static void kill_pipelines_of(vw_ctx* c);
+
+struct PairPending {
+  bool valid = false;
+  hipGraphNode_t node = nullptr;
+  FwdCall<double> call;
+  FwdPlan<double> plan;
+  FwdArgs<double> args;
+};
 
 struct vw_ctx {
   int device = 0;
@@ -85,6 +93,8 @@
   size_t med_bytes = 0;
   int* nf = nullptr;
   int64_t nf_rows = 0;
+  PairPending pair;
+  int fused_pairs = 0;
 };
 
 struct vw_graph {
@@ -94,6 +104,7 @@
   std::vector<TimedLaunch> timed;
   hipGraph_t graph = nullptr;
   hipGraphExec_t exec = nullptr;
+  int fused_pairs = 0;
 };
 
 static void release_graph(vw_graph* gr) {
@@ -153,6 +164,7 @@
   TimedLaunch tl;
   bool on;
   LaunchTimer(vw_ctx* ctx, const char* family) : c(ctx), on(ctx->timing) {
+    c->pair.valid = false;
     if (!on) return;
     tl.family = family;
     if (c->capturing) {
@@ -351,6 +363,8 @@
   VW_HIP(hipStreamBeginCapture(c->stream, hipStreamCaptureModeThreadLocal));
   c->capturing = true;
   c->captured.clear();
+  c->pair.valid = false;
+  c->fused_pairs = 0;
   return ok();
 }
 
@@ -360,6 +374,7 @@
   if (!c->capturing) return fail(VW_ERR_STATE, "not capturing");
   hipSetDevice(c->device);
   c->capturing = false;
+  c->pair.valid = false;
   std::vector<TimedLaunch> timed;
   timed.swap(c->captured);
   auto drop = [&] { for (auto& t : timed) { hipEventDestroy(t.start); hipEventDestroy(t.stop); } };
@@ -383,6 +398,7 @@
   gr->ws_gen = c->ws_gen;
   gr->graph = graph;
   gr->exec = exec;
+  gr->fused_pairs = c->fused_pairs;
   c->graphs.insert(gr);
   *out = gr;
   return ok();
@@ -406,6 +422,29 @@
                      c->pending.end());
     for (const auto& t : gr->timed) c->pending.push_back(t);
   }
+  return ok();
+}
+
+extern "C" vw_status vw_graph_stats(vw_graph* gr, int* kernel_nodes, int* fused_pairs) {
+  if (!gr) return fail(VW_ERR_NULL, "graph is null");
+  vw_ctx* c = gr->ctx;
+  if (!c) return fail(VW_ERR_STATE, "the context of this graph was destroyed");
+  std::lock_guard<std::recursive_mutex> g(c->mu);
+  hipSetDevice(c->device);
+  if (kernel_nodes) {
+    size_t n = 0;
+    VW_HIP(hipGraphGetNodes(gr->graph, nullptr, &n));
+    std::vector<hipGraphNode_t> nodes(n);
+    if (n) VW_HIP(hipGraphGetNodes(gr->graph, nodes.data(), &n));
+    int kernels = 0;
+    for (size_t i = 0; i < n; ++i) {
+      hipGraphNodeType ty;
+      VW_HIP(hipGraphNodeGetType(nodes[i], &ty));
+      if (ty == hipGraphNodeTypeKernel) ++kernels;
+    }
+    *kernel_nodes = kernels;
+  }
+  if (fused_pairs) *fused_pairs = gr->fused_pairs;
   return ok();
 }
 
@@ -835,6 +874,93 @@
   return VW_OK;
 }
 
+
+static bool capture_tail(hipStream_t st, hipGraphNode_t* node) {
+  hipStreamCaptureStatus status;
+  unsigned long long id = 0;
+  hipGraph_t g = nullptr;
+  const hipGraphNode_t* deps = nullptr;
+  size_t ndeps = 0;
+  if (hipStreamGetCaptureInfo_v2(st, &status, &id, &g, &deps, &ndeps) != hipSuccess) {
+    (void)hipGetLastError();
+    return false;
+  }
+  if (status != hipStreamCaptureStatusActive || ndeps != 1 || !deps) return false;
+  *node = deps[0];
+  return true;
+}
+
+static bool pair_forward_shape(const FwdPlan<double>& p) {
+  return p.fused && p.kernel == kFwdPersist && p.args.level_ct && p.nv == 4 && p.args.taps <= kPairMaxTaps;
+}
+
+static void pair_after_forward(vw_ctx* c, const FwdCall<double>& k, const FwdPlan<double>& p, const FwdArgs<double>& a) {
+  c->pair.valid = false;
+  if (!c->tune.pair_fuse || !pair_forward_shape(p)) return;
+  if (!c->capturing) {
+    if (pair_prepare(a.taps, p.fma, p.threads, p.lds, nullptr) != hipSuccess) (void)hipGetLastError();
+    return;
+  }
+  if (c->timing || p.ref_nf || p.validate) return;
+  hipGraphNode_t node = nullptr;
+  hipGraphNodeType ty;
+  if (!capture_tail(c->stream, &node)) return;
+  if (hipGraphNodeGetType(node, &ty) != hipSuccess || ty != hipGraphNodeTypeKernel) {
+    (void)hipGetLastError();
+    return;
+  }
+  c->pair.node = node;
+  c->pair.call = k;
+  c->pair.call.lo = c->pair.call.hi = nullptr;
+  c->pair.plan = p;
+  c->pair.args = a;
+  c->pair.valid = true;
+}
+static void pair_after_forward(vw_ctx* c, const FwdCall<float>&, const FwdPlan<float>&, const FwdArgs<float>&) {
+  c->pair.valid = false;
+}
+
+static void pair_args(const FwdArgs<double>& f, const InvCall<double>& k, const InvPlan<double>& p, PairArgs<double>* a) {
+  a->f = f;
+  a->y = k.y;
+  double lo[kMaxTaps], hi[kMaxTaps];
+  copy_bank(lo, hi, k, p.args.taps, p.args.taps_hi);
+  for (int i = 0; i < kPairMaxTaps; ++i) { a->ilo[i] = lo[i]; a->ihi[i] = hi[i]; }
+  for (int j = 0; j < kMaxLevels; ++j) { a->hr[j] = p.args.lv[j].hr; a->own[j] = p.args.lv[j].own; }
+}
+
+static bool try_pair_fuse(vw_ctx* c, const InvCall<double>& k, const InvPlan<double>& p) {
+  const bool pending = c->pair.valid;
+  c->pair.valid = false;
+  if (!pending || !c->capturing || c->timing || !c->tune.pair_fuse) return false;
+  hipGraphNode_t tail = nullptr;
+  if (!capture_tail(c->stream, &tail) || tail != c->pair.node) return false;
+  if (!pair_fusable(c->pair.call, c->pair.plan, k, p)) return false;
+  const FwdPlan<double>& fp = c->pair.plan;
+  PairLaunch l;
+  if (!pair_launch_shape(fp.args.taps, fp.fma, fp.threads, fp.lds, k.B, c->cus, &l)) return false;
+  PairArgs<double> a;
+  pair_args(c->pair.args, k, p, &a);
+  void* params[] = {&a};
+  hipKernelNodeParams np;
+  memset(&np, 0, sizeof(np));
+  np.func = const_cast<void*>(l.func);
+  np.gridDim = dim3(l.grid);
+  np.blockDim = dim3(l.threads);
+  np.sharedMemBytes = l.lds;
+  np.kernelParams = params;
+  if (hipGraphKernelNodeSetParams(c->pair.node, &np) != hipSuccess) {
+    (void)hipGetLastError();
+    return false;
+  }
+  ++c->fused_pairs;
+  return true;
+}
+static bool try_pair_fuse(vw_ctx* c, const InvCall<float>&, const InvPlan<float>&) {
+  c->pair.valid = false;
+  return false;
+}
+
 template <typename T>
 static vw_status forward_impl(vw_ctx* c, FwdCall<T> k) {
   VW_TRY(capture_guard(c, k.flags));
@@ -857,12 +983,15 @@
     a.nf_flag = p.nf_probed ? c->nf : nullptr;
     for (int j = 0; j < k.J; ++j) a.hist[j] = k.hist ? k.hist[j] : nullptr;
     copy_bank(a.lo, a.hi, k, a.taps, a.taps_hi);
-    LaunchTimer lt(c, "forward");
-    hipError_t e = p.kernel == kFwdMfma    ? mfma_forward(a, p.lds, c->stream)
-                 : p.kernel == kFwdBlk     ? launch_forward_blk<T>(a, p.threads, p.lds, p.fma, p.nv, c->stream)
-                 : p.kernel == kFwdPersist ? launch_forward_persist<T>(a, p.threads, p.lds, p.fma, p.nv, c->stream)
-                                           : launch_forward_fused<T>(a, p.threads, p.lds, p.fma, p.nv, c->stream);
-    if (e != hipSuccess) return fail(VW_ERR_DEVICE, "forward launch failed: %s", hipGetErrorString(e));
+    {
+      LaunchTimer lt(c, "forward");
+      hipError_t e = p.kernel == kFwdMfma    ? mfma_forward(a, p.lds, c->stream)
+                   : p.kernel == kFwdBlk     ? launch_forward_blk<T>(a, p.threads, p.lds, p.fma, p.nv, c->stream)
+                   : p.kernel == kFwdPersist ? launch_forward_persist<T>(a, p.threads, p.lds, p.fma, p.nv, c->stream)
+                                             : launch_forward_fused<T>(a, p.threads, p.lds, p.fma, p.nv, c->stream);
+      if (e != hipSuccess) return fail(VW_ERR_DEVICE, "forward launch failed: %s", hipGetErrorString(e));
+    }
+    pair_after_forward(c, k, p, a);
   } else {
     VW_TRY(forward_steps(c, k, p));
   }
@@ -957,6 +1086,7 @@
   plan_inverse(c->tune, k, &p);
   if (p.error != VW_OK) return fail((vw_status)p.error, "%s", p.msg);
   VW_TRY(reserve(c, p.res));
+  if (try_pair_fuse(c, k, p)) return VW_OK;
   if (p.fused) {
     InvArgs<T> a = p.args;
     a.details = k.details; a.approx = k.approx; a.y = k.y; a.thr = k.thr;
@@ -1176,6 +1306,73 @@
                                           int J, unsigned detail_mask, int approx_zero, unsigned flags, float* y) {
   return modwt_inverse<float>(c, details, approx, B, N, lo, hi, L, wid, boundary, J, detail_mask, approx_zero, flags,
                               y);
+}
+
+extern "C" vw_status vw_modwt_roundtrip_f64(vw_ctx* c, const double* x, int64_t B, int64_t N, int64_t ldx,
+                                            const double* lo, const double* hi, const double* rlo, const double* rhi,
+                                            int L, int wid, int boundary, int J, unsigned flags, double* details,
+                                            double* approx, double* y) {
+  if (c && x && details && approx && y && lo && hi && rlo && rhi && !(flags & VW_FLAG_HOST_MEMORY) && B > 0 && N > 0 &&
+      ldx >= N && L >= 1 && L <= kPairMaxTaps && J >= 1 && J <= kMaxLevels && boundary == VW_PERIODIC) {
+    std::lock_guard<std::recursive_mutex> g(c->mu);
+    hipSetDevice(c->device);
+    FwdCall<double> fk;
+    fk.x = x; fk.B = B; fk.N = N; fk.ldx = ldx; fk.lo = lo; fk.hi = hi; fk.L = L; fk.boundary = boundary; fk.J = J;
+    fk.flags = flags; fk.details = details; fk.approx = approx; fk.cus = c->cus;
+    InvCall<double> ik;
+    ik.details = details; ik.approx = approx; ik.B = B; ik.N = N; ik.lo = rlo; ik.hi = rhi; ik.L = L; ik.wid = wid;
+    ik.boundary = boundary; ik.J = J; ik.flags = flags; ik.y = y; ik.cus = c->cus;
+    FwdPlan<double> fp;
+    InvPlan<double> ip;
+    if (c->tune.pair_fuse && check_levels(N, L, J, flags) == VW_OK && capture_guard(c, flags) == VW_OK) {
+      plan_forward(c->tune, fk, &fp);
+      plan_inverse(c->tune, ik, &ip);
+      PairLaunch l;
+      if (pair_fusable(fk, fp, ik, ip) &&
+          (c->capturing || pair_prepare(fp.args.taps, fp.fma, fp.threads, fp.lds, nullptr) == hipSuccess) &&
+          pair_launch_shape(fp.args.taps, fp.fma, fp.threads, fp.lds, B, c->cus, &l)) {
+        FwdArgs<double> f = fp.args;
+        f.x = x; f.details = details; f.approx = approx;
+        f.bad = c->bad;
+        copy_bank(f.lo, f.hi, fk, f.taps, f.taps_hi);
+        PairArgs<double> a;
+        pair_args(f, ik, ip, &a);
+        {
+          LaunchTimer lt(c, "roundtrip");
+          hipError_t e = launch_roundtrip(a, l, c->stream);
+          if (e != hipSuccess) return fail(VW_ERR_DEVICE, "round-trip launch failed: %s", hipGetErrorString(e));
+        }
+        if (flags & VW_FLAG_SYNC) VW_HIP(hipStreamSynchronize(c->stream));
+        return ok();
+      }
+      (void)hipGetLastError();
+    }
+  }
+  VW_TRY(modwt_forward<double>(c, x, B, N, ldx, lo, hi, L, wid, boundary, J, flags, details, approx));
+  return modwt_inverse<double>(c, details, approx, B, N, rlo, rhi, L, wid, boundary, J, ~0u, 0, flags, y);
+}
+
+extern "C" vw_status vw_roundtrip_occupancy(vw_ctx* c, int64_t N, int L, int J, unsigned flags, int* per_cu) {
+  if (!c || !per_cu) return fail(VW_ERR_NULL, "null argument");
+  *per_cu = 0;
+  if (N <= 0 || N > (1LL << 30) || L < 1 || L > kPairMaxTaps || J < 1 || J > kMaxLevels) return ok();
+  std::lock_guard<std::recursive_mutex> g(c->mu);
+  if (c->capturing) return fail(VW_ERR_STATE, "occupancy queries cannot be captured");
+  hipSetDevice(c->device);
+  double* const aligned = reinterpret_cast<double*>(uintptr_t(4096));
+  static const double taps[kPairMaxTaps] = {0};
+  FwdCall<double> fk;
+  fk.x = aligned; fk.details = aligned; fk.approx = aligned;
+  fk.B = 4LL * c->cus; fk.N = N; fk.ldx = N; fk.lo = taps; fk.hi = taps; fk.L = L; fk.J = J;
+  fk.flags = flags & VW_FLAG_FMA; fk.cus = c->cus;
+  FwdPlan<double> fp;
+  plan_forward(c->tune, fk, &fp);
+  if (fp.error != VW_OK || !pair_forward_shape(fp)) return ok();
+  if (pair_prepare(fp.args.taps, fp.fma, fp.threads, fp.lds, per_cu) != hipSuccess) {
+    (void)hipGetLastError();
+    *per_cu = 0;
+  }
+  return ok();
 }
 
 static int bank_hi(int Llo, int Lhi) { return Lhi == Llo ? 0 : Lhi; }
diff --git a/vectorwave_amd/csrc/vw_device.h b/vectorwave_amd/csrc/vw_device.h
--- a/vectorwave_amd/csrc/vw_device.h
+++ b/vectorwave_amd/csrc/vw_device.h
@@ -699,17 +699,18 @@
   if (__any(z != z) && (threadIdx.x & 63) == 0) flag[b] = 1;
 }
 
-template <typename T, int L, bool FMA, int NV, bool VALIDATE, bool NFP = false, bool FULL = false, int LH = L>
+template <typename T, int L, bool FMA, int NV, bool VALIDATE, bool NFP = false, bool FULL = false, int LH = L,
+          int AUX = VW_FWD_STORE_AUX>
 __device__ __forceinline__ void fwd_level(const FwdArgs<T>& p, const T* X, int nvec, const LevelDesc& lv, T* dout,
                                           T* aout, bool vec_ok, unsigned long long flat0, T (&areg)[NV][VT<T>::V],
-                                          T* nf = nullptr) {
+                                          T* nf = nullptr, T (*dkeep)[VT<T>::V] = nullptr) {
   constexpr int V = VT<T>::V;
   const int N = p.N;
   const int ct = VALIDATE ? 0 : p.level_ct;
   fwd_row<T, L, FMA, NV, FULL, LH>(X, nvec, lv.s, p.lo, p.hi, p.taps, ct, [&](int k, int w, const T (&al)[V], const T (&ah)[V]) {
     const int t0 = w * V;
-    store_vec<VW_FWD_STORE_AUX, FULL>(dout, t0, N, vec_ok, ah);
-    if (aout) store_vec<VW_FWD_STORE_AUX, FULL>(aout, t0, N, vec_ok, al);
+    store_vec<AUX, FULL>(dout, t0, N, vec_ok, ah);
+    if (aout) store_vec<AUX, FULL>(aout, t0, N, vec_ok, al);
     if constexpr (VALIDATE) {
       check_out<T>(1, p.bad, flat0, t0, N, ah);
       check_out<T>(1, p.bad, flat0, t0, N, al);
@@ -719,6 +720,10 @@
     }
 #pragma unroll
     for (int e = 0; e < V; ++e) areg[k][e] = al[e];
+    if (dkeep) {
+#pragma unroll
+      for (int e = 0; e < V; ++e) dkeep[k][e] = ah[e];
+    }
   }, p.taps_hi);
 }
 
diff --git a/vectorwave_amd/csrc/vw_internal.h b/vectorwave_amd/csrc/vw_internal.h
--- a/vectorwave_amd/csrc/vw_internal.h
+++ b/vectorwave_amd/csrc/vw_internal.h
@@ -103,6 +103,17 @@
   LevelDesc lv[kMaxLevels];
 };
 
+constexpr int kPairMaxTaps = 8;
+template <typename T>
+struct PairArgs {
+  FwdArgs<T> f;
+  T* y;
+  T ilo[kPairMaxTaps];
+  T ihi[kPairMaxTaps];
+  int hr[kMaxLevels];
+  int own[kMaxLevels];
+};
+
 template <typename T>
 struct LevelArgs {
   const T* src_a;
@@ -331,6 +342,13 @@
 hipError_t launch_forward_blk(const FwdArgs<T>& a, int threads, int lds_bytes, bool fma, int nv, hipStream_t st);
 template <typename T>
 hipError_t launch_inverse_fused(const InvArgs<T>& a, int threads, int lds_bytes, bool fma, int nv, hipStream_t st);
+struct PairLaunch {
+  const void* func;
+  unsigned grid, threads, lds;
+};
+hipError_t pair_prepare(int taps, bool fma, int threads, int lds_bytes, int* per_cu);
+bool pair_launch_shape(int taps, bool fma, int threads, int lds_bytes, long long B, int cus, PairLaunch* out);
+hipError_t launch_roundtrip(const PairArgs<double>& a, const PairLaunch& l, hipStream_t st);
 template <typename T>
 hipError_t launch_forward_level(const LevelArgs<T>& a, int lds_bytes, bool fma, hipStream_t st);
 template <typename T>
diff --git a/vectorwave_amd/csrc/vw_pair.hip b/vectorwave_amd/csrc/vw_pair.hip
--- /dev/null
+++ b/vectorwave_amd/csrc/vw_pair.hip
@@ -0,0 +1,181 @@
+#include "vw_device.h"
+
+#include <algorithm>
+#include <mutex>
+
+namespace vw {
+
+#ifndef VW_PAIR_STORE_AUX
+#define VW_PAIR_STORE_AUX 16
+#endif
+
+template <typename P>
+__device__ __forceinline__ const P* reread(const P* p) {
+  int z = 0;
+  asm volatile("" : "+s"(z));
+  return p + z;
+}
+
+template <typename T, int L, bool FMA>
+__global__ void __attribute__((amdgpu_flat_work_group_size(1, 512), amdgpu_waves_per_eu(4)))
+k_roundtrip(const PairArgs<T> q) {
+  constexpr int V = VT<T>::V;
+  constexpr int NV = 4;
+  const FwdArgs<T>& p = q.f;
+  extern __shared__ __attribute__((aligned(16))) unsigned char smem[];
+  const int N = p.N;
+  const int nvec = N / V;
+  const long long G = gridDim.x;
+  const size_t plane = (size_t)p.B * (size_t)(unsigned)p.N;
+  const unsigned slab = blockDim.x * 16u;
+  long long b = blockIdx.x;
+  if (b >= p.B) return;
+  int cur = 0;
+  dma_row<T>(reinterpret_cast<T*>(smem) + p.hlpad, p.x + b * p.ldx, nvec, p.dma_nt != 0);
+  wait_vmem();
+  for (;;) {
+    const FwdArgs<T>& p0 = *reread(&q.f);
+    T* X = reinterpret_cast<T*>(smem) + (cur ? p0.region1 : 0) + p0.hlpad;
+    T* Y = reinterpret_cast<T*>(smem) + (cur ? 0 : p0.region1) + p0.hlpad;
+    lds_barrier();
+    fill_halo(X, p0.N, p0.lv[0].hl, p0.lv[0].hr, p0.lv[0].mode, p0.npow2, (const T*)nullptr, 0);
+    const long long bn = b + G;
+    const size_t row = (size_t)b * (size_t)(unsigned)N;
+    const int J = p0.J;
+    T acc[NV][V];
+    T dlast[NV][V];
+    T dreg[NV][V];
+    for (int j = 1; j <= J; ++j) {
+      const FwdArgs<T>& pj = *reread(&q.f);
+      const LevelDesc lv = pj.lv[j - 1];
+      lds_barrier();
+      if (j == pj.J && bn < pj.B) dma_row<T>(Y, pj.x + bn * pj.ldx, nvec, pj.dma_nt != 0);
+      T* dout = pj.details + (size_t)(j - 1) * plane + row;
+      T* aout = (j == pj.J) ? pj.approx + row : nullptr;
+      fwd_level<T, L, FMA, NV, false, false, true, L, VW_PAIR_STORE_AUX>(p, X, nvec, lv, dout, aout, true, 0ull, acc,
+                                                                         nullptr, dlast);
+      if (j < pj.J) {
+        regs_to_level<T, L, NV, true>(Y, acc, nvec, pj.N, pj.lv[j], pj.npow2, (const T*)nullptr);
+        T* t = X; X = Y; Y = t;
+      }
+    }
+    const PairArgs<T>& qi = *reread(&q);
+    T* const R = X - qi.f.hlpad;
+    lds_barrier();
+    plain_to_level<T, NV>(R, acc, slab, qi.f.N, qi.hr[qi.f.J - 1], qi.own[qi.f.J - 1]);
+    for (int j = J; j >= 1; --j) {
+      const PairArgs<T>& qj = *reread(&q);
+      const int s = qj.f.lv[j - 1].s;
+      lds_barrier();
+      zero_regs<T, NV>(acc);
+      plain_row<T, L, FMA, NV, 4>(R, slab, s, qj.ilo, acc);
+      lds_barrier();
+      if (j < qj.f.J) {
+        wait_vmem();
+        plain_to_level<T, NV>(R, dreg, slab, qj.f.N, qj.hr[j - 1], qj.own[j - 1]);
+      } else {
+        plain_to_level<T, NV>(R, dlast, slab, qj.f.N, qj.hr[j - 1], qj.own[j - 1]);
+      }
+      if (j > 1) {
+        if (j == qj.f.J) {
+          if (bn < qj.f.B) wait_vmcnt<3 * NV>();
+          else wait_vmcnt<2 * NV>();
+        }
+        plain_load_row<T, NV>(dreg, qj.f.details + (size_t)(j - 2) * plane + row, slab);
+      }
+      lds_barrier();
+      plain_row<T, L, FMA, NV, 4>(R, slab, s, reread(q.ihi), acc);
+      if (j > 1) {
+        lds_barrier();
+        plain_to_level<T, NV>(R, acc, slab, qj.f.N, qj.hr[j - 2], qj.own[j - 2]);
+      }
+    }
+    plain_store_row<T, NV>(q.y + row, acc, slab);
+    if (bn >= p.B) break;
+    wait_vmcnt<3 * NV>();
+    cur = (cur + J) & 1;
+    b = bn;
+  }
+}
+
+struct PairKernel {
+  static constexpr int kShapes = 16;
+  const void* func = nullptr;
+  LdsOnce lds;
+  std::mutex mu;
+  struct Shape { int threads = -1, lds = -1, per_cu = 0; } shapes[kShapes];
+  int next = 0;
+  int find(int threads, int lds_bytes) {
+    for (const Shape& sh : shapes)
+      if (sh.threads == threads && sh.lds == lds_bytes) return sh.per_cu;
+    return 0;
+  }
+};
+
+template <int L, bool FMA>
+static PairKernel* pair_kernel_of() {
+  static PairKernel k;
+  k.func = reinterpret_cast<const void*>(&k_roundtrip<double, L, FMA>);
+  return &k;
+}
+
+static PairKernel* pair_kernel(int taps, bool fma) {
+  switch (taps) {
+#define VW_CASE(n) \
+    case n:        \
+      if constexpr (n <= kPairMaxTaps) return fma ? pair_kernel_of<n, true>() : pair_kernel_of<n, false>(); \
+      break;
+    VW_TAP_LIST(VW_CASE)
+#undef VW_CASE
+    default: break;
+  }
+  return nullptr;
+}
+
+static bool lds_ready(PairKernel* k, int lds) {
+  if (lds <= 64 * 1024) return true;
+  int dev = 0;
+  if (hipGetDevice(&dev) != hipSuccess || dev < 0 || dev >= kMaxDevices) return false;
+  return k->lds.limit[dev].load(std::memory_order_acquire) >= lds;
+}
+
+hipError_t pair_prepare(int taps, bool fma, int threads, int lds, int* per_cu) {
+  PairKernel* k = pair_kernel(taps, fma);
+  if (!k) return hipErrorNotSupported;
+  hipError_t e = set_lds(k->func, lds, &k->lds);
+  if (e != hipSuccess) return e;
+  std::lock_guard<std::mutex> g(k->mu);
+  int n = k->find(threads, lds);
+  if (!n) {
+    if ((e = hipOccupancyMaxActiveBlocksPerMultiprocessor(&n, k->func, threads, lds)) != hipSuccess) return e;
+    if (n < 1) return hipErrorInvalidConfiguration;
+    PairKernel::Shape& sh = k->shapes[k->next];
+    k->next = (k->next + 1) % PairKernel::kShapes;
+    sh.threads = threads; sh.lds = lds; sh.per_cu = n;
+  }
+  if (per_cu) *per_cu = n;
+  return hipSuccess;
+}
+
+bool pair_launch_shape(int taps, bool fma, int threads, int lds, long long B, int cus, PairLaunch* out) {
+  PairKernel* k = pair_kernel(taps, fma);
+  if (!k || !lds_ready(k, lds)) return false;
+  int n;
+  {
+    std::lock_guard<std::mutex> g(k->mu);
+    n = k->find(threads, lds);
+  }
+  if (n < 1) return false;
+  out->func = k->func;
+  out->grid = (unsigned)std::min<long long>(B, (long long)n * cus);
+  out->threads = (unsigned)threads;
+  out->lds = (unsigned)lds;
+  return true;
+}
+
+hipError_t launch_roundtrip(const PairArgs<double>& a, const PairLaunch& l, hipStream_t st) {
+  void* params[] = {const_cast<PairArgs<double>*>(&a)};
+  return hipLaunchKernel(l.func, dim3(l.grid), dim3(l.threads), params, l.lds, st);
+}
+
+}
diff --git a/vectorwave_amd/csrc/vw_plan.cpp b/vectorwave_amd/csrc/vw_plan.cpp
--- a/vectorwave_amd/csrc/vw_plan.cpp
+++ b/vectorwave_amd/csrc/vw_plan.cpp
@@ -58,6 +58,7 @@
     VW_KEY("VW_BI", t.bi = v < 0 ? d.bi : v & 7),
     VW_KEY("VW_BI_LISTED", t.bi_listed = v < 0 ? d.bi_listed : v != 0),
     VW_KEY("VW_INV_WAVES", t.inv_waves = v == 6 || v == 8 ? v : d.inv_waves),
+    VW_KEY("VW_PAIR_FUSE", t.pair_fuse = v < 0 ? d.pair_fuse : v != 0),
 };
 #undef VW_KEY
 
@@ -685,6 +686,17 @@
 }
 
 template <typename T>
+static bool plain_class(const InvCall<T>& c, const InvPlan<T>& p, int nv) {
+  const InvArgs<T>& a = p.args;
+  if (!(a.full && sizeof(T) == 8 && nv == 4 && c.L <= 8 && c.boundary == VW_PERIODIC && !c.thr && !c.approx_zero &&
+        !a.rev && !p.ref_nf))
+    return false;
+  for (int j = 0; j < c.J; ++j)
+    if (!(a.lv[j].use_d && plus_zero(a.lv[j]) && a.lv[j].hl == 0 && a.lv[j].hr <= c.N)) return false;
+  return true;
+}
+
+template <typename T>
 static bool plan_inverse_fused(const Tuning& tu, const InvCall<T>& c, bool pair, int max_hl, int max_hr,
                                InvPlan<T>* p, bool bi = false) {
   constexpr int V = vec_width<T>();
@@ -738,11 +750,7 @@
     }
   }
   p->nf_probed = p->ref_nf && (p->kernel == kInvSeq || p->kernel == kInvBlk);
-  bool plain = a.full && p->kernel == kInvSeq && sizeof(T) == 8 && nv == 4 && L <= 8 && periodic && !c.thr &&
-               !c.approx_zero && !a.rev && !p->ref_nf;
-  for (int j = 0; plain && j < J; ++j)
-    plain = a.lv[j].use_d && plus_zero(a.lv[j]) && a.lv[j].hl == 0 && a.lv[j].hr <= N;
-  a.plain = plain ? 1 : 0;
+  a.plain = p->kernel == kInvSeq && plain_class(c, *p, nv) ? 1 : 0;
   a.waves = tu.inv_waves;
   p->threads = threads; p->nv = nv; p->lds = lds;
   return true;
@@ -984,6 +992,46 @@
   }
 }
 
+static bool ranges_overlap(const void* a, size_t a_bytes, const void* b, size_t b_bytes) {
+  const uintptr_t a0 = (uintptr_t)a, b0 = (uintptr_t)b;
+  return a0 < b0 + b_bytes && b0 < a0 + a_bytes;
+}
+
+template <typename T>
+bool pair_fusable(const FwdCall<T>& fc, const FwdPlan<T>& fp, const InvCall<T>& ic, const InvPlan<T>& ip) {
+  if (sizeof(T) != 8) return false;
+  if (fp.error != VW_OK || ip.error != VW_OK || !fp.fused || !ip.fused) return false;
+  const int64_t B = fc.B, N = fc.N;
+  const int J = fc.J, L = fc.L;
+  if (ic.B != B || ic.N != N || ic.J != J || ic.L != L || hi_taps(fc) != L || hi_taps(ic) != L) return false;
+  if (fc.boundary != VW_PERIODIC || ic.boundary != VW_PERIODIC || fc.single_level || ic.single_level) return false;
+  if (fp.fma != ip.fma) return false;
+  if ((const T*)fc.details != ic.details || (const T*)fc.approx != ic.approx) return false;
+  const unsigned all = J >= 32 ? ~0u : (1u << J) - 1u;
+  if ((ic.detail_mask & all) != all || ic.approx_zero || ic.thr) return false;
+  const unsigned off = VW_FLAG_VALIDATE | VW_FLAG_REF_NONFINITE | VW_FLAG_HOST_MEMORY;
+  if ((fc.flags | ic.flags) & off) return false;
+  if (fc.hist || fp.validate || fp.ref_nf || ip.ref_nf || fp.snapshot) return false;
+  if (fp.kernel != kFwdPersist || !fp.args.level_ct || fp.nv != 4 || fp.args.region1 <= 0) return false;
+  if (L > kPairMaxTaps || !has_unrolled_taps(L) || fp.args.taps != L || fp.args.taps_hi != L) return false;
+  const InvArgs<T>& ia = ip.args;
+  if (ip.threads != fp.threads || ip.nv != 4 || ia.taps != L || ia.taps_hi != L) return false;
+  if (!ia.plain && !(ip.kernel == kInvDb && plain_class(ic, ip, ip.nv))) return false;
+  for (int j = 0; j < J; ++j)
+    if (ia.lv[j].s != fp.args.lv[j].s || N + ia.lv[j].hr > fp.args.region1) return false;
+  if (fp.lds < 2 * fp.args.region1 * (int)sizeof(T)) return false;
+  const size_t row = (size_t)N * sizeof(T), plane = (size_t)B * row;
+  const size_t x_bytes = ((size_t)(B - 1) * (size_t)fc.ldx + (size_t)N) * sizeof(T);
+  if (ranges_overlap(ic.y, plane, fc.x, x_bytes) || ranges_overlap(ic.y, plane, fc.details, (size_t)J * plane) ||
+      ranges_overlap(ic.y, plane, fc.approx, plane))
+    return false;
+  return true;
+}
+template bool pair_fusable<float>(const FwdCall<float>&, const FwdPlan<float>&, const InvCall<float>&,
+                                  const InvPlan<float>&);
+template bool pair_fusable<double>(const FwdCall<double>&, const FwdPlan<double>&, const InvCall<double>&,
+                                   const InvPlan<double>&);
+
 template void plan_forward<float>(const Tuning&, const FwdCall<float>&, FwdPlan<float>*);
 template void plan_forward<double>(const Tuning&, const FwdCall<double>&, FwdPlan<double>*);
 template void plan_inverse<float>(const Tuning&, const InvCall<float>&, InvPlan<float>*);
diff --git a/vectorwave_amd/csrc/vw_plan.h b/vectorwave_amd/csrc/vw_plan.h
--- a/vectorwave_amd/csrc/vw_plan.h
+++ b/vectorwave_amd/csrc/vw_plan.h
@@ -50,6 +50,7 @@
   int bi = 3;
   int inv_waves = 6;
   int mra_fused = 1;
+  int pair_fuse = 1;
   int bi_listed = 1;
 };
 
@@ -169,4 +170,7 @@
 template <typename T> void plan_forward(const Tuning& tu, const FwdCall<T>& c, FwdPlan<T>* p);
 template <typename T> void plan_inverse(const Tuning& tu, const InvCall<T>& c, InvPlan<T>* p);
 
+template <typename T>
+bool pair_fusable(const FwdCall<T>& fc, const FwdPlan<T>& fp, const InvCall<T>& ic, const InvPlan<T>& ip);
+
 }
diff --git a/vectorwave_amd/engine.py b/vectorwave_amd/engine.py
--- a/vectorwave_amd/engine.py
+++ b/vectorwave_amd/engine.py
@@ -197,6 +197,28 @@
                   detail_mask & 0xFFFFFFFF, 1 if approx_zero else 0, self._flags(flags, dev), self._ptr(y, dev)))
         return y
 
+    def roundtrip(self, x, lo, hi, rlo, rhi, wavelet_id: int, boundary: int, levels: int, flags: int):
+        xa, dev, xp, _ = self._prep(x, np.float64)
+        one = xa.ndim == 1
+        B, N = (1, xa.shape[0]) if one else xa.shape
+        det = self._empty(xa, dev, (levels, N) if one else (levels, B, N))
+        app = self._empty(xa, dev, xa.shape)
+        y = self._empty(xa, dev, xa.shape)
+        L = _one_length(lo, hi, "roundtrip")
+        if _one_length(rlo, rhi, "roundtrip") != L:
+            raise InvalidArgumentException("roundtrip takes one filter length for both pairs")
+        _check(self.lib.vw_modwt_roundtrip_f64(self.ctx, xp, B, N, N, nat.taps_array(lo), nat.taps_array(hi),
+                                               nat.taps_array(rlo), nat.taps_array(rhi), L, wavelet_id, boundary,
+                                               levels, self._flags(flags, dev), self._ptr(det, dev),
+                                               self._ptr(app, dev), self._ptr(y, dev)))
+        return det, app, y
+
+    def roundtrip_occupancy(self, N: int, L: int, levels: int, flags: int = 0) -> int:
+        from ctypes import c_int
+        n = c_int()
+        _check(self.lib.vw_roundtrip_occupancy(self.ctx, int(N), int(L), int(levels), int(flags), byref(n)))
+        return n.value
+
     def forward1(self, x, lo, hi, boundary: int, flags: int):
         xa, dev, xp, f32 = self._prep(x, np.float64)
         one = xa.ndim == 1
@@ -402,6 +424,12 @@
     def launch(self, count: int = 1) -> None:
         _check(self.engine.lib.vw_graph_launch(self.handle, int(count)))
 
+    def stats(self) -> Tuple[int, int]:
+        from ctypes import c_int
+        k, f = c_int(), c_int()
+        _check(self.engine.lib.vw_graph_stats(self.handle, byref(k), byref(f)))
+        return k.value, f.value
+
     def close(self) -> None:
         if self.handle:
             _check(self.engine.lib.vw_graph_destroy(self.handle))
```

After: 52770 (median of 6 runs). +8.8%, better.
